# SabaPivot/ProjectionTrainer

Hardware: AMD Instinct MI355X
Metric: Stage-1 images/sec/node (SigLIP-L-384 + Gemma3-1B, 576+128 tok) (higher is better)
Workload: dtype bf16; 1 GPU; cfg2: SigLIP-ViT-L/16-384 frozen fwd + MLP projector fwd/bwd + Gemma3-1B frozen fwd/bwd, 575 vis + 128 text tokens; global_batch=32, per_gpu_batch=32, seq_len=703, parallelism=dp1

## Files before the change

### include/ptk.h

```cpp
#ifndef PTK_H
#define PTK_H

#include <stddef.h>
#include <stdint.h>

#ifdef __cplusplus
extern "C" {
#endif

#define PTK_ABI_VERSION 8

int ptk_abi_version(void);
const char* ptk_last_error(void);


typedef struct {
  int g;
  int skip;
  int64_t gs;
  int64_t off;
} ptk_rowmap;

enum { PTK_ACT_NONE = 0, PTK_ACT_GELU_TANH = 1, PTK_ACT_GELU_ERF = 2, PTK_ACT_GEGLU = 3,
       PTK_ACT_GELU_ERF_BWD = 4, PTK_ACT_GEGLU_BWD = 5 };
enum { PTK_OUT_BF16 = 0, PTK_OUT_F32 = 1, PTK_OUT_F32_BF16ROUND = 2 };

typedef struct {
  const void* A;
  const void* B;
  void* C;
  int M, N, K;
  int64_t lda, ldb, ldc;
  int batch;
  int batch_inner;
  int64_t sA0, sA1, sB0, sB1, sC0, sC1;
  float alpha;
  int act;
  int out;
  const float* bias;
  const float* rowadd;
  int rowadd_period;
  int64_t ld_rowadd;
  const float* resid;
  int64_t ld_resid;
  void* aux;
  void* aux2;
  int64_t ld_aux;
  const void* aux_in;
  const void* aux_in2;
  int64_t ld_aux_in;
  ptk_rowmap amap;
  ptk_rowmap cmap;
  const void* resid16;
  int64_t ld_resid16;
  int bf16_linear;
  void* tail_ws;
  const void* B_kt;
  int A_kt, C_kt, aux_kt, aux_in_kt;
} ptk_gemm_desc;
int ptk_gemm_ktiled_counts(int64_t* out2, int reset);
int ptk_gemm_ktiled_pair(const ptk_gemm_desc* producer, const ptk_gemm_desc* consumer, int ncu, int64_t part_floats,
                         int train);
int ptk_a_ktiled_reload(void);
int ptk_gemm(const ptk_gemm_desc* d, void* stream);
int64_t ptk_kstep_tile_offset(int64_t row, int64_t k, int64_t K);
int ptk_pack_kstep_tiles_bf16(const void* src, void* dst, int N, int K, void* stream);
#define PTK_GEMM_TAIL_COUNTER_BYTES 16384
size_t ptk_gemm_tail_scratch_bytes(void);
int ptk_gemm_tail_split(const ptk_gemm_desc* d);
int ptk_gemm_plan(const ptk_gemm_desc* d, int ncu, int* path, int* tile_rows, int* tail_split);
int ptk_gemm_split_plan(const ptk_gemm_desc* d, int ncu, int64_t part_floats, int* slices, int* kc, int* rem,
                        int* tail_ws);

int ptk_layernorm(const float* x, const float* w, const float* b, void* y, int rows, int cols, float eps,
                  void* stream);
int ptk_rmsnorm(const float* x, const float* w, void* y, float* rstd, int rows, int cols, float eps,
                void* stream);
int ptk_rmsnorm_bwd(const float* x, const float* w, const float* rstd, const float* dn, const float* dacc,
                    float* dx, int rows, int cols, void* stream);
int ptk_qknorm_rope_fwd(const void* qkv, const float* q_norm_w, const float* k_norm_w, const float* cos_t,
                        const float* sin_t, int batch, int seq, int heads, int kv_heads, int head_dim, float eps,
                        void* Q, void* K, void* V, float* rstd_q, float* rstd_k, void* stream);
int ptk_qknorm_rope_bwd(const void* qkv, const float* q_norm_w, const float* k_norm_w, const float* cos_t,
                        const float* sin_t, int batch, int seq, int heads, int kv_heads, int head_dim,
                        const float* rstd_q, const float* rstd_k, const void* dQ, const void* dK, const void* dV,
                        void* dqkv, void* stream);
int ptk_softmax(const float* S, void* P, int nz, int rows, int cols, int64_t ld, int rows_per_batch, int qdiv,
                int zdiv, int causal, int window, const int32_t* key_valid, int key_len, void* stream);
int ptk_cross_entropy(void* logits, int64_t ld, int rows, int vocab, const int64_t* targets, float* row_loss,
                      const float* gscale, void* stream);
int ptk_transpose_bf16(const void* in, int64_t ld_in, void* out, int64_t ld_out, int nz, int64_t s_in,
                       int64_t s_out, int rows, int cols, int rows_pad, void* stream);
int ptk_transpose_rows_bf16(const void* in, int64_t ld_in, int map_g, int64_t map_gs, int64_t map_off, int rows,
                            int cols, void* out, int64_t ld_out, int rows_pad, void* stream);
int ptk_weight_grad_bf16(const void* dy, int64_t lddy, int y_map_g, int64_t y_map_gs, int64_t y_map_off, int Ny,
                         const void* x, int64_t ldx, int x_map_g, int64_t x_map_gs, int64_t x_map_off, int Nx, int rows,
                         void* grad, void* ta, void* tb, float* part, int64_t part_floats, int mode, void* stream);
int ptk_cast_f32_bf16(const float* in, void* out, int64_t n, void* stream);
int ptk_fill_normal_bf16(void* out, int64_t n, uint64_t seed, float std, float mean, void* stream);
int ptk_gemm_timer_enable(int on);
int ptk_gemm_force_small_tiles(int mode);
int ptk_gemm_timer_read(int act_class, double* total_ms, int* count);
#define PTK_GEMM_NPATHS 9
int ptk_gemm_path_counts(int64_t* counts, int reset);

int ptk_stage_timers_enable(int on);
int ptk_stage_begin(const char* name, void* stream);
int ptk_stage_end(void* stream);
int64_t ptk_stage_timers_read(char* buf, size_t cap, int reset);

typedef struct {
  const void* Q; const void* K; const void* V; void* O; float* lse;
  int rows, nkeys, head_dim;
  int64_t ldq, ldk, ldo;
  int batch, batch_inner, zdiv;
  int64_t sQ0, sQ1, sK0, sK1, sO0, sO1;
  ptk_rowmap qmap, omap;
  int qdiv, causal, window;
  const int32_t* key_valid;
  float scale;
} ptk_flash_desc;
int ptk_flash_attn_fwd(const ptk_flash_desc* d, void* stream);

typedef struct {
  const void* Q; const void* K; const void* V; const void* O; const void* dO;
  const float* lse; float* delta;
  void* dQ; void* dK; void* dV;
  int rows, nkeys, head_dim;
  int batch, batch_inner, zdiv;
  int64_t ldo, sO0, sO1;
  ptk_rowmap omap;
  int qdiv, causal, window;
// ... 223 lines not shown
```

### projectiontrainer_amd/_lib.py

```python
from __future__ import annotations

import ctypes as C
import os

_HERE = os.path.dirname(os.path.abspath(__file__))
LIB_PATH = os.path.join(_HERE, "libptk.so")
if os.environ.get("PTK_LIB"):
    LIB_PATH = os.path.join(os.path.dirname(_HERE), os.environ["PTK_LIB"])

c_void_p, c_int, c_int64, c_float, c_size_t, c_uint64 = C.c_void_p, C.c_int, C.c_int64, C.c_float, C.c_size_t, C.c_uint64
c_float_p = C.POINTER(C.c_float)

ACT_NONE, ACT_GELU_TANH, ACT_GELU_ERF, ACT_GEGLU, ACT_GELU_ERF_BWD, ACT_GEGLU_BWD = range(6)
OUT_BF16, OUT_F32, OUT_F32_BF16ROUND = range(3)


class RowMap(C.Structure):
    _fields_ = [("g", c_int), ("skip", c_int), ("gs", c_int64), ("off", c_int64)]


class GemmDesc(C.Structure):
    _fields_ = [("A", c_void_p), ("B", c_void_p), ("C", c_void_p),
                ("M", c_int), ("N", c_int), ("K", c_int),
                ("lda", c_int64), ("ldb", c_int64), ("ldc", c_int64),
# ... 95 lines not shown


class Gemma3LayerGradsC(C.Structure):
    _fields_ = [(n, c_void_p) for n in ("wqkv", "wo", "wgu", "wd", "ln_in", "ln_post_attn", "ln_pre_ff",
                                        "ln_post_ff", "q_norm", "k_norm")]


class Gemma3GradsC(C.Structure):
    _fields_ = [("embed", c_void_p), ("final_norm", c_void_p), ("layers", C.POINTER(Gemma3LayerGradsC))]


class ImageDesc(C.Structure):
    _fields_ = [("src_off", c_int64), ("h", C.c_int32), ("w", C.c_int32), ("c", C.c_int32),
                ("kh", C.c_int32), ("kv", C.c_int32), ("pad_", C.c_int32),
                ("coef_off", c_int64), ("tmp_off", c_int64)]


ABI_VERSION = 8

SIGNATURES = {
    "ptk_abi_version": (c_int, []),
    "ptk_last_error": (C.c_char_p, []),
    "ptk_gemm": (c_int, [C.POINTER(GemmDesc), c_void_p]),
    "ptk_gemm_tail_scratch_bytes": (c_size_t, []),
    "ptk_gemm_tail_split": (c_int, [C.POINTER(GemmDesc)]),
    "ptk_gemm_plan": (c_int, [C.POINTER(GemmDesc), c_int] + [C.POINTER(c_int)] * 3),
    "ptk_gemm_split_plan": (c_int, [C.POINTER(GemmDesc), c_int, c_int64] + [C.POINTER(c_int)] * 4),
    "ptk_layernorm": (c_int, [c_void_p, c_void_p, c_void_p, c_void_p, c_int, c_int, c_float, c_void_p]),
    "ptk_rmsnorm": (c_int, [c_void_p, c_void_p, c_void_p, c_void_p, c_int, c_int, c_float, c_void_p]),
    "ptk_rmsnorm_bwd": (c_int, [c_void_p] * 6 + [c_int, c_int, c_void_p]),
    "ptk_qknorm_rope_fwd": (c_int, [c_void_p] * 5 + [c_int] * 5 + [c_float] + [c_void_p] * 6),
    "ptk_qknorm_rope_bwd": (c_int, [c_void_p] * 5 + [c_int] * 5 + [c_void_p] * 7),
    "ptk_softmax": (c_int, [c_void_p, c_void_p, c_int, c_int, c_int, c_int64, c_int, c_int, c_int, c_int,
                            c_int, c_void_p, c_int, c_void_p]),
    "ptk_cross_entropy": (c_int, [c_void_p, c_int64, c_int, c_int, c_void_p, c_void_p, c_void_p, c_void_p]),
    "ptk_transpose_bf16": (c_int, [c_void_p, c_int64, c_void_p, c_int64, c_int, c_int64, c_int64, c_int,
                                   c_int, c_int, c_void_p]),
    "ptk_transpose_rows_bf16": (c_int, [c_void_p, c_int64, c_int, c_int64, c_int64, c_int, c_int, c_void_p, c_int64,
                                        c_int, c_void_p]),
    "ptk_weight_grad_bf16": (c_int, [c_void_p, c_int64, c_int, c_int64, c_int64, c_int,
                                     c_void_p, c_int64, c_int, c_int64, c_int64, c_int, c_int,
                                     c_void_p, c_void_p, c_void_p, c_void_p, c_int64, c_int, c_void_p]),
    "ptk_cast_f32_bf16": (c_int, [c_void_p, c_void_p, c_int64, c_void_p]),
    "ptk_kstep_tile_offset": (c_int64, [c_int64, c_int64, c_int64]),
    "ptk_pack_kstep_tiles_bf16": (c_int, [c_void_p, c_void_p, c_int, c_int, c_void_p]),
    "ptk_fill_normal_bf16": (c_int, [c_void_p, c_int64, c_uint64, c_float, c_float, c_void_p]),
    "ptk_gemm_timer_enable": (c_int, [c_int]),
    "ptk_gemm_force_small_tiles": (c_int, [c_int]),
    "ptk_gemm_timer_read": (c_int, [c_int, C.POINTER(C.c_double), C.POINTER(c_int)]),
    "ptk_gemm_path_counts": (c_int, [c_void_p, c_int]),
    "ptk_gemm_ktiled_counts": (c_int, [c_void_p, c_int]),
    "ptk_gemm_ktiled_pair": (c_int, [C.POINTER(GemmDesc), C.POINTER(GemmDesc), c_int, c_int64, c_int]),
    "ptk_a_ktiled_reload": (c_int, []),
    "ptk_stage_timers_enable": (c_int, [c_int]),
    "ptk_stage_begin": (c_int, [C.c_char_p, c_void_p]),
    "ptk_stage_end": (c_int, [c_void_p]),
    "ptk_stage_timers_read": (c_int64, [C.c_char_p, c_size_t, c_int]),
    "ptk_flash_attn_fwd": (c_int, [C.POINTER(FlashDesc), c_void_p]),
    "ptk_flash_attn_bwd": (c_int, [C.POINTER(FlashBwdDesc), c_void_p]),
    "ptk_flash_bwd_workspace_bytes": (c_size_t, [C.POINTER(FlashBwdDesc)]),
    "ptk_siglip_workspace_bytes": (c_size_t, [C.POINTER(SiglipConfigC), c_int]),
    "ptk_siglip_fwd": (c_int, [C.POINTER(SiglipConfigC), C.POINTER(SiglipWeightsC), c_int, c_void_p, c_void_p,
                               c_void_p, c_size_t, c_void_p]),
    "ptk_projector_fwd": (c_int, [C.POINTER(ProjectorC), c_int, c_void_p, c_void_p, c_void_p, c_void_p, RowMap,
                                  c_int64, c_int, c_void_p]),
    "ptk_projector_workspace_bytes": (c_size_t, [C.POINTER(ProjectorC), c_int]),
    "ptk_projector_bwd": (c_int, [C.POINTER(ProjectorC), c_int] + [c_void_p] * 8 + [c_void_p, c_size_t, c_void_p]),
    "ptk_gather_vision_grad": (c_int, [c_void_p, c_int, c_int, c_int, c_int, c_void_p, c_void_p]),
    "ptk_gemma3_workspace_bytes": (c_size_t, [C.POINTER(Gemma3ConfigC), c_int, c_int, c_int]),
    "ptk_gemma3_loss_fwd_bwd": (c_int, [C.POINTER(Gemma3ConfigC), C.POINTER(Gemma3WeightsC),
                                        C.POINTER(Gemma3BatchC), c_void_p, c_size_t, c_void_p]),
    "ptk_gemma3_loss_fwd": (c_int, [C.POINTER(Gemma3ConfigC), C.POINTER(Gemma3WeightsC),
                                    C.POINTER(Gemma3BatchC), c_void_p, c_size_t, c_void_p]),
    "ptk_gemma3_train_workspace_bytes": (c_size_t, [C.POINTER(Gemma3ConfigC), c_int, c_int, c_int]),
    "ptk_gemma3_train_fwd_bwd": (c_int, [C.POINTER(Gemma3ConfigC), C.POINTER(Gemma3WeightsC),
                                         C.POINTER(Gemma3BatchC), C.POINTER(Gemma3GradsC), c_void_p, c_size_t,
                                         c_void_p]),
    "ptk_gemma3_generate_workspace_bytes": (c_size_t, [C.POINTER(Gemma3ConfigC), c_int, c_int, c_int]),
    "ptk_gemma3_generate": (c_int, [C.POINTER(Gemma3ConfigC), C.POINTER(Gemma3WeightsC), C.POINTER(Gemma3GenerateC),
                                    c_void_p, c_void_p, c_void_p, c_void_p, c_void_p, c_size_t, c_void_p]),
    "ptk_gemma3_decode_workspace_bytes": (c_size_t, [C.POINTER(Gemma3ConfigC), C.POINTER(Gemma3DecodeC)]),
    "ptk_gemma3_decode_prefill": (c_int, [C.POINTER(Gemma3ConfigC), C.POINTER(Gemma3WeightsC),
                                          C.POINTER(Gemma3DecodeC), c_void_p, c_void_p, c_int64, c_void_p, c_void_p,
                                          c_size_t, c_void_p]),
    "ptk_gemma3_decode_step": (c_int, [C.POINTER(Gemma3ConfigC), C.POINTER(Gemma3WeightsC), C.POINTER(Gemma3DecodeC),
                                       c_int, c_void_p, c_void_p, c_void_p, c_void_p, c_size_t, c_void_p]),
    "ptk_beam_candidates_workspace_bytes": (c_size_t, [c_int, c_int, c_int]),
    "ptk_beam_candidates": (c_int, [c_void_p, c_int64, c_void_p, c_int, c_int, c_int, c_int, c_int, c_float, c_float,
                                    c_int, c_uint64, c_int, c_int, c_void_p, c_void_p, c_void_p, c_void_p, c_size_t,
                                    c_void_p]),
    "ptk_sample_next_token_workspace_bytes": (c_size_t, [c_int]),
    "ptk_sample_next_token": (c_int, [c_void_p, c_int64, c_int, c_int, c_int, c_int, c_float, c_float, c_uint64, c_int,
                                      c_int64, c_int64, c_void_p, c_void_p, c_int64, c_int, c_float, c_void_p,
                                      c_void_p, c_size_t, c_void_p]),
    "ptk_beam_candidates_penalized_workspace_bytes": (c_size_t, [c_int, c_int, c_int]),
    "ptk_beam_candidates_penalized": (c_int, [c_void_p, c_int64, c_void_p, c_int, c_int, c_int, c_int, c_int, c_float,
                                              c_float, c_int, c_uint64, c_int, c_int, c_void_p, c_int64, c_int,
                                              c_float, c_void_p, c_void_p, c_void_p, c_void_p, c_size_t, c_void_p]),
    "ptk_gemma3_generate_penalized_workspace_bytes": (c_size_t, [C.POINTER(Gemma3ConfigC), c_int, c_int, c_int]),
    "ptk_gemma3_generate_penalized": (c_int, [C.POINTER(Gemma3ConfigC), C.POINTER(Gemma3WeightsC),
                                              C.POINTER(Gemma3GenerateC), c_void_p, c_void_p, c_void_p, c_void_p,
                                              c_float, c_void_p, c_size_t, c_void_p]),
    "ptk_gemm_skinny_part_bytes": (c_size_t, [c_int, c_int, c_int]),
    "ptk_gemm_skinny": (c_int, [c_void_p, c_int64, c_void_p, c_int64, c_void_p, c_int64, c_int, c_int, c_int, c_int,
                                c_void_p, c_size_t, c_void_p]),
    "ptk_embed_grad_workspace_bytes": (c_size_t, [c_int, c_int]),
# ... 18 lines not shown
                                    [c_void_p, c_size_t, c_void_p, c_void_p, c_void_p]),
    "ptk_clip_adamw": (c_int, [c_void_p, c_void_p, c_void_p, c_void_p, c_int64, c_float, c_float, c_float,
                               c_float, c_float, c_float, c_float, c_int, c_void_p, c_void_p, c_void_p]),
}

_lib = None


class PtkError(RuntimeError):
    pass


def lib():
    global _lib
    if _lib is None:
        if not os.path.exists(LIB_PATH):
            raise PtkError(f"libptk.so not found at {LIB_PATH}: run `python -c 'import __graft_entry__ as g; g.build()'`")
        L = C.CDLL(LIB_PATH)
        for name, (res, args) in SIGNATURES.items():
            if os.environ.get("PTK_LIB") and not hasattr(L, name):
                continue
            f = getattr(L, name)
            f.restype, f.argtypes = res, args
        if L.ptk_abi_version() != ABI_VERSION:
            raise PtkError("libptk ABI version mismatch")
        _lib = L
    return _lib


def check(rc: int, what: str = ""):
    if rc != 0:
        raise PtkError(f"{what}: {lib().ptk_last_error().decode()}")


def ptr(t) -> int | None:
    return None if t is None else t.data_ptr()


GEMM_PATHS = ("nt128", "big", "big2", "w4", "nt128b", "p8sk", "p8", "tn", "unused8")


def gemm_path_counts(reset=False):
    buf = (C.c_int64 * (8 * len(GEMM_PATHS)))()
    check(lib().ptk_gemm_path_counts(buf, int(reset)), "gemm_path_counts")
    return {(GEMM_PATHS[i // 8], i % 8): int(v) for i, v in enumerate(buf) if v}


def gemm_ktiled_counts(reset=False):
    buf = (C.c_int64 * 2)()
    check(lib().ptk_gemm_ktiled_counts(buf, int(reset)), "gemm_ktiled_counts")
    return int(buf[0]), int(buf[1])


_stages_on = os.environ.get("PTK_STAGE_TIMERS", "0") not in ("", "0")


def stage_timers_enable(on=True):
    global _stages_on
    _stages_on = bool(on)
    check(lib().ptk_stage_timers_enable(int(bool(on))), "stage_timers_enable")


class stage:

    def __init__(self, name, device=None):
        self.name, self.device, self.on = name, device, False

    def __enter__(self):
        self.on = _stages_on
        if self.on:
            self.st = stream_ptr(self.device)
            check(lib().ptk_stage_begin(self.name.encode(), self.st), "stage_begin")
        return self

    def __exit__(self, *exc):
        if self.on:
            check(lib().ptk_stage_end(self.st), "stage_end")
        return False


def stage_timers_read(reset=False):
    n = lib().ptk_stage_timers_read(None, 0, 0)
    if n < 0:
        check(-1, "stage_timers_read")
    buf = C.create_string_buffer(int(n) + 64)
    n = lib().ptk_stage_timers_read(buf, len(buf), int(reset))
    if n < 0:
        check(-1, "stage_timers_read")
    out = {}
    for line in buf.value.decode().splitlines():
        name, ms, cnt = line.split("\t")
        out[name] = (float(ms), int(cnt))
    return out


def stream_ptr(device=None) -> int:
    import torch
    return torch.cuda.current_stream(device).cuda_stream
```

### projectiontrainer_amd/csrc/capi.cpp

```cpp
#include <stdarg.h>
#include <stdio.h>

#include "../../include/ptk.h"
#include "ptk_internal.h"

namespace ptk {

static thread_local char g_err[512] = "";

int set_error(const char* fmt, ...) {
  va_list ap;
  va_start(ap, fmt);
  vsnprintf(g_err, sizeof(g_err), fmt, ap);
  va_end(ap);
  return -1;
}

RowMap to_map(ptk_rowmap m) { return RowMap{m.g, m.skip, (long)m.gs, (long)m.off}; }

GemmArgs to_args(const ptk_gemm_desc* d) {
  GemmArgs a;
  a.A = (const bf16_t*)d->A; a.B = (const bf16_t*)d->B; a.C = d->C;
  a.M = d->M; a.N = d->N; a.K = d->K;
  a.lda = d->lda; a.ldb = d->ldb; a.ldc = d->ldc;
// ... 34 lines not shown

int ptk_abi_version(void) { return PTK_ABI_VERSION; }
const char* ptk_last_error(void) { return g_err; }

int ptk_gemm(const ptk_gemm_desc* d, void* stream) {
  if (!d) return set_error("ptk_gemm: null desc");
  if (d->act == PTK_ACT_GEGLU && (d->N % 32)) return set_error("ptk_gemm: GEGLU needs N %% 32 == 0");
  return launch_gemm(to_args(d), d->act, d->out, d->batch > 0 ? d->batch : 1, ST);
}

size_t ptk_gemm_tail_scratch_bytes(void) { return p8_tail_scratch_bytes(); }
int ptk_gemm_tail_split(const ptk_gemm_desc* d) {
  if (!d) return set_error("ptk_gemm_tail_split: null desc");
  return p8_tail_plan(to_args(d), d->act, d->out, gemm_plan_env()).gsplit;
}
static GemmPlanEnv test_plan_env(int ncu) {
  GemmPlanEnv e = gemm_plan_env();
  e.ncu = ncu;
  e.tail_scope = nullptr;
  return e;
}
int ptk_gemm_plan(const ptk_gemm_desc* d, int ncu, int* path, int* tile_rows, int* tail_split) {
  if (!d || ncu <= 0) return set_error("ptk_gemm_plan: null desc or ncu <= 0");
  const GemmPlan p = gemm_plan(to_args(d), d->act, d->out, d->batch > 0 ? d->batch : 1, test_plan_env(ncu));
  if (path) *path = p.path;
  if (tile_rows) *tile_rows = p.tm;
  if (tail_split) *tail_split = p.tail.gsplit;
  return 0;
}
int ptk_gemm_split_plan(const ptk_gemm_desc* d, int ncu, int64_t part_floats, int* slices, int* kc, int* rem,
                        int* tail_ws) {
  if (!d || ncu <= 0) return set_error("ptk_gemm_split_plan: null desc or ncu <= 0");
  const GemmSplitPlan s = gemm_split_plan(to_args(d), d->out, (long)part_floats, test_plan_env(ncu));
  if (slices) *slices = s.slices;
  if (kc) *kc = s.kc;
  if (rem) *rem = s.rem;
  if (tail_ws) *tail_ws = s.tail_ws ? 1 : 0;
  return 0;
}

size_t ptk_gemm_skinny_part_bytes(int M, int N, int K) { return skinny_part_bytes(M, N, K); }
int ptk_gemm_skinny(const void* A, int64_t lda, const void* B, int64_t ldb, void* C, int64_t ldc, int M, int N, int K,
                    int act, void* part, size_t part_bytes, void* stream) {
  if (!A || !B || !C) return set_error("ptk_gemm_skinny: NULL operand");
  return launch_gemm_skinny((const bf16_t*)A, (long)lda, (const bf16_t*)B, (long)ldb, (bf16_t*)C, (long)ldc, M, N, K,
                            act, (float*)part, part_bytes, (hipStream_t)stream);
}

int ptk_layernorm(const float* x, const float* w, const float* b, void* y, int rows, int cols, float eps,
                  void* stream) {
  return launch_layernorm(x, w, b, (bf16_t*)y, rows, cols, eps, ST);
}

int ptk_rmsnorm(const float* x, const float* w, void* y, float* rstd, int rows, int cols, float eps, void* stream) {
  return launch_rmsnorm_fwd(x, cols, RowMap{0, 0, 0, 0}, w, (bf16_t*)y, rstd, rows, cols, eps, ST);
}

int ptk_rmsnorm_bwd(const float* x, const float* w, const float* rstd, const float* dn, const float* dacc, float* dx,
                    int rows, int cols, void* stream) {
  return launch_rmsnorm_bwd_f32(x, w, rstd, dn, dacc, dx, rows, cols, ST);
}

int ptk_qknorm_rope_fwd(const void* qkv, const float* q_norm_w, const float* k_norm_w, const float* cos_t,
                        const float* sin_t, int batch, int seq, int heads, int kv_heads, int head_dim, float eps,
                        void* Q, void* K, void* V, float* rstd_q, float* rstd_k, void* stream) {
  const AttnShape sh{batch, seq, heads, kv_heads, head_dim};
  return launch_qknorm_rope_fwd((const bf16_t*)qkv, q_norm_w, k_norm_w, cos_t, sin_t, sh, eps, (bf16_t*)Q,
                                (bf16_t*)K, (bf16_t*)V, rstd_q, rstd_k, ST);
}
int ptk_qknorm_rope_bwd(const void* qkv, const float* q_norm_w, const float* k_norm_w, const float* cos_t,
                        const float* sin_t, int batch, int seq, int heads, int kv_heads, int head_dim,
                        const float* rstd_q, const float* rstd_k, const void* dQ, const void* dK, const void* dV,
                        void* dqkv, void* stream) {
  const AttnShape sh{batch, seq, heads, kv_heads, head_dim};
  return launch_qknorm_rope_bwd((const bf16_t*)qkv, q_norm_w, k_norm_w, cos_t, sin_t, sh, rstd_q, rstd_k,
                                (const bf16_t*)dQ, (const bf16_t*)dK, (const bf16_t*)dV, (bf16_t*)dqkv, ST);
}
int ptk_softmax(const float* S, void* P, int nz, int rows, int cols, int64_t ld, int rows_per_batch, int qdiv,
                int zdiv, int causal, int window, const int32_t* key_valid, int key_len, void* stream) {
  MaskSpec m{rows_per_batch > 0 ? rows_per_batch : rows, qdiv > 0 ? qdiv : 1, zdiv > 0 ? zdiv : 1, causal, window,
             key_valid, key_len};
  return launch_softmax_fwd(S, (bf16_t*)P, nz, rows, cols, ld, m, ST);
}

int ptk_cross_entropy(void* logits, int64_t ld, int rows, int vocab, const int64_t* targets, float* row_loss,
                      const float* gscale, void* stream) {
  return launch_ce_fwd_bwd((bf16_t*)logits, ld, rows, vocab, targets, row_loss, gscale, ST);
}

int ptk_transpose_bf16(const void* in, int64_t ld_in, void* out, int64_t ld_out, int nz, int64_t s_in, int64_t s_out,
                       int rows, int cols, int rows_pad, void* stream) {
  return launch_transpose((const bf16_t*)in, ld_in, s_in, 0, 1, (bf16_t*)out, ld_out, s_out, 0, nz, rows, cols,
                          rows_pad, ST);
}

int ptk_transpose_rows_bf16(const void* in, int64_t ld_in, int map_g, int64_t map_gs, int64_t map_off, int rows,
                            int cols, void* out, int64_t ld_out, int rows_pad, void* stream) {
  const RowMap m{map_g, 0, map_gs, map_off};
  return launch_transpose_rows((const bf16_t*)in, ld_in, m, rows, cols, (bf16_t*)out, ld_out, rows_pad, ST);
}

int64_t ptk_kstep_tile_offset(int64_t row, int64_t k, int64_t K) { return kstep_tile_offset(row, k, K); }
int ptk_pack_kstep_tiles_bf16(const void* src, void* dst, int N, int K, void* stream) {
  return launch_pack_kstep_tiles((const bf16_t*)src, (bf16_t*)dst, N, K, ST);
}
int ptk_cast_f32_bf16(const float* in, void* out, int64_t n, void* stream) {
  return launch_cast_f32_bf16(in, (bf16_t*)out, n, ST);
}

int ptk_gemm_force_small_tiles(int mode) {
  if (mode != 0 && mode != 1 && mode != 2 && mode != 4 && mode != 8 && mode != 32 && mode != 512 && mode != 1024 &&
      mode != 4096)
    return set_error("gemm tile mode %d not in {0, 1, 2, 4, 8, 32, 512, 1024, 4096}", mode);
  force_small_tiles(mode);
  return 0;
}
int ptk_gemm_timer_enable(int on) {
  timer_enable(on);
  return 0;
}
int ptk_gemm_timer_read(int act_class, double* total_ms, int* count) { return timer_read(act_class, total_ms, count); }
int ptk_gemm_path_counts(int64_t* counts, int reset) { return path_counts(counts, reset); }
int ptk_gemm_ktiled_counts(int64_t* out2, int reset) { return ktiled_counts(out2, reset); }
int ptk_gemm_ktiled_pair(const ptk_gemm_desc* producer, const ptk_gemm_desc* consumer, int ncu, int64_t part_floats,
                         int train) {
  if (!producer || !consumer || ncu <= 0 || producer->batch > 1 || consumer->batch > 1) return 0;
  return !train && gemm_ktiled_pair(to_args(producer), producer->act, to_args(consumer), (long)part_floats,
                                    test_plan_env(ncu), a_ktiled_mode() != 0, true) ? 1 : 0;
}

int ptk_fill_normal_bf16(void* out, int64_t n, uint64_t seed, float std, float mean, void* stream) {
  return launch_fill_normal_bf16((bf16_t*)out, n, seed, std, mean, ST);
}

int ptk_flash_attn_fwd(const ptk_flash_desc* d, void* stream) {
  if (!d) return set_error("flash: null desc");
  FlashArgs a;
  a.Q = (const bf16_t*)d->Q; a.K = (const bf16_t*)d->K; a.V = (const bf16_t*)d->V; a.O = (bf16_t*)d->O;
  a.lse = d->lse; a.rows = d->rows; a.nkeys = d->nkeys; a.D = d->head_dim;
  a.ldq = d->ldq; a.ldk = d->ldk; a.ldo = d->ldo;
  a.zin = d->batch_inner > 0 ? d->batch_inner : 1; a.zdiv = d->zdiv > 0 ? d->zdiv : 1;
  a.sQ0 = d->sQ0; a.sQ1 = d->sQ1; a.sK0 = d->sK0; a.sK1 = d->sK1; a.sO0 = d->sO0; a.sO1 = d->sO1;
  a.qmap = to_map(d->qmap); a.omap = to_map(d->omap);
  a.qdiv = d->qdiv > 0 ? d->qdiv : 1; a.causal = d->causal; a.window = d->window;
  a.key_valid = d->key_valid; a.scale = d->scale;
  return launch_attn_fwd(a, d->batch > 0 ? d->batch : 1, ST);
}

static FlashBwdArgs to_bwd_args(const ptk_flash_bwd_desc* d) {
  FlashBwdArgs a;
  a.Q = (const bf16_t*)d->Q; a.K = (const bf16_t*)d->K; a.V = (const bf16_t*)d->V; a.O = (const bf16_t*)d->O;
  a.dO = (const bf16_t*)d->dO; a.lse = d->lse; a.delta = d->delta;
  a.dQ = (bf16_t*)d->dQ; a.dK = (bf16_t*)d->dK; a.dV = (bf16_t*)d->dV;
  a.rows = d->rows; a.nkeys = d->nkeys; a.D = d->head_dim;
  a.zin = d->batch_inner > 0 ? d->batch_inner : 1; a.zdiv = d->zdiv > 0 ? d->zdiv : 1;
  a.ldo = d->ldo; a.sO0 = d->sO0; a.sO1 = d->sO1; a.omap = to_map(d->omap);
  a.qdiv = d->qdiv > 0 ? d->qdiv : 1; a.causal = d->causal; a.window = d->window;
  a.key_valid = d->key_valid; a.scale = d->scale;
  a.dkv_part = (float*)d->workspace;
  a.dkv_part_bytes = d->workspace && d->workspace_bytes > 0 ? (size_t)d->workspace_bytes : 0;
  return a;
}

size_t ptk_flash_bwd_workspace_bytes(const ptk_flash_bwd_desc* d) {
  if (!d) return 0;
  return attn_bwd_workspace_bytes(to_bwd_args(d), d->batch > 0 ? d->batch : 1);
}

int ptk_flash_attn_bwd(const ptk_flash_bwd_desc* d, void* stream) {
  if (!d) return set_error("flash_bwd: null desc");
  return launch_attn_bwd(to_bwd_args(d), d->batch > 0 ? d->batch : 1, ST);
}

int ptk_projector_fwd(const ptk_projector* p, int rows, const void* x, void* a, void* h, float* out,
                      ptk_rowmap out_map, int64_t ld_out, int round_bf16, void* stream) {
  const int Dv = p->vision_dim, I = p->inter_dim, Dl = p->llm_dim;
  TailScratchScope tail(p->tail_ws, ST);
  if (tail.status) return -1;
  StageScope stage("projector.fwd", ST);
  GemmArgs g1;
  g1.A = (const bf16_t*)x; g1.B = (const bf16_t*)p->w1; g1.C = h;
  g1.M = rows; g1.N = I; g1.K = Dv; g1.lda = Dv; g1.ldb = Dv; g1.ldc = I;
// ... 101 lines not shown
```

### projectiontrainer_amd/csrc/gemm.hip

```cpp
#include <stdlib.h>

#include "common.h"
#include "ptk_internal.h"
#include "gemm_epi.h"

#include <algorithm>
#include <vector>

namespace ptk {

constexpr int BM = 128, BN = 128, BK = 64, GROUP_M = 8;
constexpr int STAGE_BYTES = (BM + BN) * BK * 2;
static_assert(4 * 64 * 68 * 4 >= 2 * STAGE_BYTES, "epilogue staging must cover the pipeline buffers");

typedef const __attribute__((address_space(1))) void* gptr_t;
typedef __attribute__((address_space(3))) void* lptr_t;

#ifdef PTK_NO_SRC_SWZ
#define PTK_SRC_SWZ(c, r) (c)
#else
#define PTK_SRC_SWZ(c, r) ((c) ^ (((r) >> 1) & 7))
#endif

#ifndef PTK_GLDS_AUX
// ... 594 lines not shown
  for (int i = 0; i < 8; ++i)
#pragma unroll
    for (int j = 0; j < 4; ++j) acc[i][j] = (f32x4_t){0.f, 0.f, 0.f, 0.f};
  big2_kloop(p, smem, bm, bn, 0, p.K / BK, acc, threadIdx.x);
  big_epilogue<ACT, OUT>(p, smem, bm, bn, acc, threadIdx.x);
}

static bool g_timing = false;
static int g_timing_mask = 0;
static int g_force_tiles = 0;
void force_small_tiles(int mode) { g_force_tiles = mode; }
static std::vector<hipEvent_t> g_ev[8];
static size_t g_ev_used[8];

void timer_enable(int on) {
  g_timing = on != 0;
  g_timing_mask = on == 1 ? 0xff : (on & 0xff);
  if (g_timing)
    for (int c = 0; c < 8; ++c) g_ev_used[c] = 0;
}
static hipEvent_t next_event(int cls) {
  auto& v = g_ev[cls];
  if (g_ev_used[cls] == v.size()) {
    hipEvent_t e;
    if (hipEventCreate(&e) != hipSuccess) return nullptr;
    v.push_back(e);
  }
  return v[g_ev_used[cls]++];
}
int timer_read(int cls, double* total_ms, int* count) {
  *total_ms = 0;
  *count = 0;
  if (cls < 0 || cls >= 8) return set_error("timer: class out of range");
  for (size_t i = 0; i + 1 < g_ev_used[cls]; i += 2) {
    float ms = 0;
    if (hipEventSynchronize(g_ev[cls][i + 1]) != hipSuccess) return set_error("timer: sync failed");
    if (hipEventElapsedTime(&ms, g_ev[cls][i], g_ev[cls][i + 1]) != hipSuccess) return set_error("timer: elapsed");
    *total_ms += ms;
    *count += 1;
  }
  return 0;
}

static long g_path_count[GEMM_NPATH][8];
int path_counts(int64_t* out, int reset) {
  for (int p = 0; p < GEMM_NPATH; ++p)
    for (int c = 0; c < 8; ++c) {
      if (out) out[p * 8 + c] = g_path_count[p][c];
      if (reset) g_path_count[p][c] = 0;
    }
  return 0;
}

static long g_kt_count[2];
int ktiled_counts(int64_t* out2, int reset) {
  for (int i = 0; i < 2; ++i) {
    if (out2) out2[i] = g_kt_count[i];
    if (reset) g_kt_count[i] = 0;
  }
  return 0;
}

struct GemmLaunchScope {
  hipStream_t st;
  hipEvent_t e0 = nullptr, e1 = nullptr;
  GemmLaunchScope(int path, int act, hipStream_t s) : st(s) {
    ++g_path_count[path][act & 7];
    if (g_timing && ((g_timing_mask >> act) & 1)) { e0 = next_event(act); e1 = next_event(act); }
    if (e0) (void)hipEventRecord(e0, st);
  }
  ~GemmLaunchScope() { if (e1) (void)hipEventRecord(e1, st); }
};

GemmPlanEnv gemm_plan_env() {
  GemmPlanEnv e;
  e.ncu = device_cus();
  e.force_tiles = g_force_tiles;
  e.p8_all = PTK_AB("PTK_P8", 0) == 1;
  e.tm_short = PTK_AB("PTK_TM224", 1) != 0;
  e.lean_epi = lean_epilogue_enabled();
  e.streamk = streamk_enabled();
  e.tail_scope = tail_scope();
  return e;
}

int launch_gemm(const GemmArgs& a, int act, int out, int batch, hipStream_t st, const GemmPlan* planned) {
  if (a.M <= 0 || a.N <= 0 || batch <= 0) return 0;
  if (a.K <= 0 || a.K % BK) return set_error("gemm: K=%d must be a positive multiple of 64", a.K);
  if ((a.lda % 8) || (a.ldb % 8)) return set_error("gemm: lda/ldb must be multiples of 8 (16-B rows)");
  if (((uintptr_t)a.A | (uintptr_t)a.B) & 15) return set_error("gemm: A/B must be 16-B aligned");
  if (a.zin <= 0) return set_error("gemm: zin must be >= 1");
  const long ntile = (long)((a.M + BM - 1) / BM) * ((a.N + BN - 1) / BN);
  if (ntile > 0x7fffffffL) return set_error("gemm: too many tiles");
  if (!gemm_act_out(act, out, [](auto, auto) {})) return set_error("gemm: unsupported (act=%d, out=%d)", act, out);
  const GemmPlan plan = planned ? *planned : gemm_plan(a, act, out, batch, gemm_plan_env());
  if (a.a_kt && !a_ktiled_ok(a, plan, act, out, batch, lean_epilogue_enabled()))
    return set_error("gemm: this launch cannot read a k-step-tiled A");
  if (!c_ktiled_ok(a, plan, act, out, batch, lean_epilogue_enabled()))
    return set_error("gemm: this launch cannot write k-step-tiled outputs");
  GemmLaunchScope scope(plan.path, act, st);
  g_kt_count[0] += a.a_kt != 0;
  g_kt_count[1] += a.c_kt != 0;
  const dim3 grid_big((unsigned)((long)((a.M + BIG - 1) / BIG) * ((a.N + BIG - 1) / BIG)), 1, 1);
  switch (plan.path) {
    case GEMM_PATH_P8:
    case GEMM_PATH_P8SK:
    case GEMM_PATH_W4: {
      GemmArgs b = a;
      if (!b_ktiled_ok(a, plan, act, batch)) b.B_kt = nullptr;
      if (plan.path == GEMM_PATH_W4) return launch_gemm_w4(b, act, out, st, 0);
      return launch_gemm_p8(b, act, out, st, plan.tail, plan.tm);
    }
    case GEMM_PATH_BIG2:
      gemm_act_out(act, out, [&](auto A, auto O) {
        hipLaunchKernelGGL((gemm_big2_kernel<A(), O()>), grid_big, dim3(512), 0, st, a);
      });
      break;
    case GEMM_PATH_BIG:
      gemm_act_out(act, out, [&](auto A, auto O) {
        hipLaunchKernelGGL((gemm_big_kernel<A(), O()>), grid_big, dim3(512), 0, st, a);
      });
      break;
    default:
      gemm_act_out(act, out, [&](auto A, auto O) {
        hipLaunchKernelGGL((gemm_nt_kernel<A(), O()>), dim3((unsigned)ntile, 1, (unsigned)batch), dim3(256), 0, st, a);
      });
      break;
  }
  return hipGetLastError() == hipSuccess ? 0 : set_error("gemm launch failed");
}

int gemm_p8_kslices(const GemmArgs& a, int slices, hipStream_t st) {
  if (a.M <= 0 || a.N <= 0) return 0;
  GemmLaunchScope scope(GEMM_PATH_P8, ACT_NONE, st);
  return launch_gemm_p8_kslices(a, slices, st);
}

int gemm_tn(const GemmArgs& a, int out, int slices, void* slab, hipStream_t st, long k_rows) {
  if (a.M <= 0 || a.N <= 0) return 0;
  GemmLaunchScope scope(GEMM_PATH_TN, ACT_NONE, st);
  return launch_gemm_tn(a, out, slices, slab, st, k_rows);
}

}

#ifdef PTK_STAMPS
extern "C" int ptk_debug_epi_mode(int m) {
  return hipMemcpyToSymbol(HIP_SYMBOL(ptk::g_epi_mode), &m, sizeof(int), 0, hipMemcpyHostToDevice) == hipSuccess ? 0 : -1;
}
extern "C" int ptk_debug_stamps_read(void* host, size_t bytes) {
  return hipMemcpyFromSymbol(host, HIP_SYMBOL(ptk::g_stamps), bytes, 0, hipMemcpyDeviceToHost) == hipSuccess ? 0 : -1;
}
#endif
```

### projectiontrainer_amd/csrc/gemm_plan.cpp

```cpp
#include <algorithm>

#include "ptk_internal.h"

namespace ptk {

bool w4_supported(const GemmArgs& a, int act, int out) {
  if (a.N % 8 || a.K % W4_KT) return false;
  if (a.alpha != 1.f) return false;
  if (a.row_stats) return false;
  if (a.resid16 && (out != OUT_BF16 || a.ld_resid16 % 8)) return false;
  if ((a.ldc % 8) || (a.resid && a.ld_resid % 4) || (a.rowadd && a.ld_rowadd % 4)) return false;
  if ((a.aux || a.aux2) && a.ld_aux % 8) return false;
  if ((a.aux_in || a.aux_in2) && a.ld_aux_in % 8) return false;
  if (((uintptr_t)a.C | (uintptr_t)a.bias | (uintptr_t)a.resid | (uintptr_t)a.resid16 | (uintptr_t)a.rowadd | (uintptr_t)a.aux |
       (uintptr_t)a.aux2 | (uintptr_t)a.aux_in | (uintptr_t)a.aux_in2) & 15)
    return false;
  if (act == ACT_GEGLU && (a.N % 32)) return false;
  if (act == ACT_GEGLU_BWD && (!a.aux_in || !a.aux_in2 || (a.N % 16) || (a.ldc % 8))) return false;
  if (act == ACT_GELU_ERF_BWD && !a.aux_in) return false;
  if (out != OUT_BF16 && (act != ACT_NONE)) return false;
  if (a.amap.g != 0) return false;
  const double abytes = (double)(a.M + a.amap.off) * a.lda * 2, bbytes = (double)a.N * a.ldb * 2;
  return abytes < 2147483000.0 && bbytes < 2147483000.0;
}
// ... 133 lines not shown
         (act == ACT_NONE && out == OUT_BF16 && a.N >= 1536 && a.K <= 2048 && fill >= 0.65 &&
          lean_epilogue_candidate(a, e.lean_epi));
}

bool big_shape(const GemmArgs& a) {
  return a.M >= 1024 && a.N >= 512 && (a.K >= 6144 || (a.N >= 6144 && a.K >= 1152));
}
bool staggered_big(const GemmArgs& a, const GemmPlanEnv& e) {
  return e.force_tiles == 4 || (e.force_tiles == 0 && big_shape(a) && a.K >= 4096);
}
bool big(const GemmArgs& a, const GemmPlanEnv& e) {
  return e.force_tiles != 1 && (e.force_tiles == 2 || big_shape(a));
}

}

GemmPlan gemm_plan(const GemmArgs& a, int act, int out, int batch, const GemmPlanEnv& e) {
  GemmPlan p;
  if (batch != 1) {
    p.path = GEMM_PATH_NTB;
    return p;
  }
  if (p8_supported(a, act, out)) {
    const P8Tail tl = tail(a, act, out, e);
    const int tm = tl.units ? 256 : short_tile(a, act, out, e);
    const bool single = single_round(a, act, out, e);
    if (e.force_tiles == 32 || single || tl.units || tm != 256 || p8_over_w4(a, act, out, e)) {
      p.path = tl.units ? GEMM_PATH_P8SK : GEMM_PATH_P8;
      p.tm = tm;
      p.tail = tl;
      p.single_round = single;
      return p;
    }
  }
  if ((e.force_tiles == 8 || w4_shape(a, act, out, e)) && w4_supported(a, act, out)) p.path = GEMM_PATH_W4;
  else if (staggered_big(a, e)) p.path = GEMM_PATH_BIG2;
  else if (big(a, e)) p.path = GEMM_PATH_BIG;
  return p;
}

long kstep_tile_offset(long row, long k, long K) {
  const long rr = row & 15, chunk = (k >> 3) & 3;
  const long unit = 4 * rr + (chunk ^ ((rr >> 1) & 2));
  return ((row >> 4) * (K / 32) + (k >> 5)) * 1024 + unit * 16 + (k & 7) * 2;
}

bool b_ktiled_ok(const GemmArgs& a, const GemmPlan& plan, int act, int batch) {
  if (!a.B_kt || batch != 1 || !bkt_act(act)) return false;
  if (plan.path != GEMM_PATH_W4 && plan.path != GEMM_PATH_P8 && plan.path != GEMM_PATH_P8SK) return false;
  return a.ldb == a.K && a.K % 32 == 0 && a.N % 16 == 0 && !((uintptr_t)a.B_kt & 15);
}

bool a_ktiled_ok(const GemmArgs& a, const GemmPlan& plan, int act, int out, int batch, bool lean_epi) {
  if (batch != 1 || act != ACT_NONE || out != OUT_BF16 || plan.path != GEMM_PATH_P8 || plan.tail.units) return false;
  if (a.M % 16 || a.K % 32 || a.lda != a.K || a.amap.g != 0 || a.amap.off < 0 || a.amap.off % 16) return false;
  (void)lean_epi;
  return b_ktiled_ok(a, plan, act, batch);
}

bool c_ktiled_ok(const GemmArgs& a, const GemmPlan& plan, int act, int out, int batch, bool lean_epi) {
  if (!a.c_kt) return !a.aux_kt && !a.aux_in_kt;
  if (batch != 1 || out != OUT_BF16 || plan.path != GEMM_PATH_W4 || a.M % 16 || !b_ktiled_ok(a, plan, act, batch))
    return false;
  if (a.cmap.g != 0 || a.cmap.off < 0 || a.cmap.off % 16 || ((uintptr_t)a.C & 15)) return false;
  if (act == ACT_GEGLU) {
    if (a.N % 64 || a.ldc != a.N / 2 || a.aux_in_kt) return false;
    return !a.aux_kt || (a.aux && a.aux2 && a.ld_aux == a.N / 2 && !(((uintptr_t)a.aux | (uintptr_t)a.aux2) & 15));
  }
  uint32_t cb = 0;
  if (act != ACT_GEGLU_BWD || a.aux_kt || !lean_epilogue_ok(a, act, out, cb, lean_epi)) return false;
  return a.ldc == 2L * a.N && (!a.aux_in_kt || a.ld_aux_in == a.N);
}

bool gemm_ktiled_pair(const GemmArgs& prod, int pact, const GemmArgs& cons, long part_floats, const GemmPlanEnv& env,
                      bool enabled, bool factors) {
  if (!enabled || (pact != ACT_GEGLU && pact != ACT_GEGLU_BWD)) return false;
  GemmArgs p = prod, c = cons;
  p.c_kt = 1;
  if (factors) (pact == ACT_GEGLU ? p.aux_kt : p.aux_in_kt) = 1;
  c.a_kt = 1;
  if (!c_ktiled_ok(p, gemm_plan(prod, pact, OUT_BF16, 1, env), pact, OUT_BF16, 1, env.lean_epi)) return false;
  if (cons.A != (const bf16_t*)prod.C || cons.M != prod.M || cons.K != (pact == ACT_GEGLU ? prod.N / 2 : 2 * prod.N) ||
      cons.amap.off != prod.cmap.off)
    return false;
  const GemmSplitPlan sp = gemm_split_plan(cons, OUT_BF16, part_floats, env);
  if (sp.kc != 0 || sp.tail_ws) return false;
  const GemmPlan cp = env.force_tiles == 0 ? sp.direct : gemm_plan(cons, ACT_NONE, OUT_BF16, 1, env);
  return a_ktiled_ok(c, cp, ACT_NONE, OUT_BF16, 1, env.lean_epi);
}

GemmSplitPlan gemm_split_plan(const GemmArgs& a, int out, long part_floats, const GemmPlanEnv& env) {
  GemmSplitPlan sp;
  GemmPlanEnv e = env;
  e.force_tiles = 0;
  sp.direct = gemm_plan(a, ACT_NONE, out, 1, e);
  const GemmPlan& direct = sp.direct;
  if (direct.path == GEMM_PATH_P8SK) return sp;
  if (e.streamk && a.K >= 4096 && (size_t)part_floats * sizeof(float) >= P8_CNT_BYTES + p8_slab_bytes(e.ncu)) {
    GemmArgs b = a;
    b.tail_ws = reinterpret_cast<void*>((uintptr_t)256);
    const GemmPlan lent = gemm_plan(b, ACT_NONE, out, 1, e);
    if (lent.path == GEMM_PATH_P8SK) {
      sp.tail_ws = true;
      sp.direct = lent;
      return sp;
    }
  }
  if (direct.single_round) return sp;
  const long nbig = tiles256(a);
  int S = 1, kmin = 1024;
  if (a.K >= 4096 && nbig <= 64) S = 4;
  else if (a.K >= 4096 && nbig <= 300) S = 2;
  const long n128 = (long)((a.M + 127) / 128) * ((a.N + 127) / 128), cus = e.ncu;
  if (n128 * 2 <= cus) {
    kmin = 256;
    while (n128 * S * 2 <= 2 * cus && a.K / (S * 2) >= kmin) S *= 2;
  }
  while (S > 1 && ((long)S * a.M * a.N > part_floats || a.K / S < kmin || a.N % 4 || a.ldc % 4)) S /= 2;
  const bool plain = !a.rowadd && !a.resid && !a.aux && !a.aux_in && a.amap.g == 0 && a.amap.off == 0 &&
                     a.cmap.g == 0 && a.cmap.off == 0 && a.bias == nullptr && a.alpha == 1.f;
  if (S == 1 || !plain) return sp;
  sp.kc = (a.K / S + 63) / 64 * 64;
  sp.slices = a.K / sp.kc;
  sp.rem = a.K - sp.slices * sp.kc;
  return sp;
}

bool tn_supported(const GemmArgs& a, int out, int slices, bool lean_epi) {
  if (slices < 1 || a.K % (W4_KT * slices) || a.K / slices < 2 * W4_KT) return false;
  if (a.N % 64 || a.lda % 8 || a.ldb % 8 || a.lda < a.M || a.ldb < a.N) return false;
  if (((uintptr_t)a.A | (uintptr_t)a.B | (uintptr_t)a.C) & 15) return false;
  if (a.amap.g || a.amap.off || a.bias || a.rowadd || a.resid || a.aux || a.aux_in || a.row_stats || a.alpha != 1.f)
    return false;
  const double ab = (double)a.K * a.lda * 2, bb = (double)a.K * a.ldb * 2;
  if (ab >= 4293918720.0 || bb >= 4293918720.0) return false;
  if (out == OUT_BF16) {
    uint32_t cb = 0;
    return slices == 1 && lean_epilogue_candidate(a, lean_epi) && lean_epilogue_ok(a, ACT_NONE, OUT_BF16, cb, lean_epi);
  }
  if (out != OUT_F32 || a.ldc % 4 || a.ldc < a.N || a.cmap.g || a.cmap.off || a.resid16 || a.bf16_linear) return false;
  return (double)slices * a.M * a.ldc * 4 < 2147483000.0;
// ... 34 lines not shown
```

### projectiontrainer_amd/csrc/gemm_w4.hip

```cpp
#include "common.h"
#include "ptk_internal.h"
#include "gemm_epi.h"
#include "gemm_persist.h"

#include <algorithm>
#include <cstdlib>
#include <type_traits>

#ifndef PTK_W4_RDS
#define PTK_W4_RDS 0
#endif
#ifndef PTK_W4_DMS
#define PTK_W4_DMS 0
#endif
#ifndef PTK_P8_PRIO
#define PTK_P8_PRIO 1
#endif
#ifndef PTK_P8_MPRIO
#define PTK_P8_MPRIO 0
#endif

namespace ptk {

template <int ACT, int OUT, bool LEAN = false, bool BKT = false, int KTO = 0>
__global__ void __launch_bounds__(256, 1) gemm_w4_kernel(GemmArgs p, uint32_t a_bytes, uint32_t b_bytes,
                                                         uint32_t c_bytes) {
  __shared__ __attribute__((aligned(16))) char smem[W4_NSLOT * W4_SLOT];
  const int lane = threadIdx.x & 63;
  const int wave = __builtin_amdgcn_readfirstlane(threadIdx.x >> 6);
  const int wr = wave >> 1, wc = wave & 1;
  const int nbm = (p.M + W4 - 1) / W4, nbn = (p.N + W4 - 1) / W4;
  const int ntile = nbm * nbn;
  const int G = gridDim.x;
  int loc;
  {
    const int b = blockIdx.x, q = G >> 3, rr = G & 7, x = b & 7;
    loc = (x < rr ? x * (q + 1) : rr * (q + 1) + (x - rr) * q) + (b >> 3);
  }
  if (loc >= ntile) return;
  const int nt = p.K / W4_KT;
  const int nks = 2 * nt;
  const int total_ks = ((ntile - loc + G - 1) / G) * nks;

  constexpr bool bkt = BKT;
  constexpr uint32_t bks = BKT ? 1024u : (uint32_t)(W4_KS * 2);
  const u32x4_t rsa = w4_rsrc(p.A, a_bytes), rsb = w4_rsrc(bkt ? p.B_kt : p.B, b_bytes);

  uint32_t offa[4], offb[4];
#pragma unroll
  for (int j = 0; j < 4; ++j) {
    const int lr = wave * 64 + 16 * j + (lane >> 2);
    const int lc = (lane & 3) ^ ((lane >> 3) & 2);
    offa[j] = (uint32_t)lr * (uint32_t)p.lda * 2u + lc * 16;
    offb[j] = bkt ? (uint32_t)(wave * 4 + j) * (uint32_t)p.K * 32u + lane * 16
                  : (uint32_t)lr * (uint32_t)p.ldb * 2u + lc * 16;
  }
  const uint32_t lds_base = __builtin_amdgcn_readfirstlane(lds_addr(smem));
  const uint32_t lds_dma = lds_base + wave * 64 * 64;
  int dt = loc, dks = 0, dcount = 0;
  uint32_t dsa = 0, dsb = 0;
  auto dma_tile = [&](int t) {
    int bm, bn;
    w4_tile_coords(t, nbm, nbn, bm, bn);
    dsa = __builtin_amdgcn_readfirstlane((uint32_t)(bm * W4 + (int)p.amap.off) * (uint32_t)p.lda * 2u);
    dsb = __builtin_amdgcn_readfirstlane((uint32_t)(bn * W4) * (uint32_t)p.ldb * 2u);
  };
  auto dma_advance = [&]() {
    if (++dcount < total_ks) {
      if (++dks == nks) {
        dks = 0;
        dt += G;
        dma_tile(dt);
      }
    }
  };
  auto slot_next = [](uint32_t s) { s += W4_SLOT; return s == W4_NSLOT * W4_SLOT ? 0u : s; };

  const int frag_off = (lane & 15) * 64 + (((lane >> 4) ^ ((lane >> 1) & 2)) << 4);
  const uint32_t frag_a = lds_addr(smem) + wr * 128 * 64 + frag_off;
  const uint32_t frag_b = lds_addr(smem) + W4_SOPB + wc * 128 * 64 + frag_off;
  bf16x8_t fa0[8], fb0[8], fa1[8], fb1[8];
  f32x4_t acc[8][8];

#define W4_GROUP(FA, FB, Q, FIRST)                                                  \
  do {                                                                              \
    _Pragma("unroll") for (int jj = 0; jj < 4; ++jj) {                              \
      if (FIRST) W4_MFMA0(acc[(Q) >> 1][4 * ((Q) & 1) + jj], FB[4 * ((Q) & 1) + jj], FA[(Q) >> 1]); \
      else W4_MFMA(acc[(Q) >> 1][4 * ((Q) & 1) + jj], FB[4 * ((Q) & 1) + jj], FA[(Q) >> 1]);       \
    }                                                                               \
  } while (0)
#define W4_READ(FA, FB, BA, BB, Q)                                                  \
  do {                                                                              \
    if ((Q) < 8) W4_DSREAD(FA[(Q) & 7], BA, ((Q) & 7) * 1024);                      \
    else W4_DSREAD(FB[(Q) & 7], BB, ((Q) & 7) * 1024);                              \
  } while (0)
#define W4_PIN(FA, FB)                                                                              \
  do {                                                                                              \
    asm volatile("s_waitcnt lgkmcnt(0)" ::: "memory");                                              \
    asm volatile("" : "+v"(FA[0]), "+v"(FA[1]), "+v"(FA[2]), "+v"(FA[3]), "+v"(FA[4]), "+v"(FA[5]),  \
                 "+v"(FA[6]), "+v"(FA[7]));                                                         \
    asm volatile("" : "+v"(FB[0]), "+v"(FB[1]), "+v"(FB[2]), "+v"(FB[3]), "+v"(FB[4]), "+v"(FB[5]),  \
                 "+v"(FB[6]), "+v"(FB[7]));                                                         \
  } while (0)

  auto kstep = [&](auto first_c, const bf16x8_t (&FA)[8], const bf16x8_t (&FB)[8], bf16x8_t (&NA)[8],
                   bf16x8_t (&NB)[8], uint32_t rs, uint32_t ws) {
    constexpr bool first = decltype(first_c)::value;
    const uint32_t ba = frag_a + rs, bb = frag_b + rs;
    const uint32_t da = lds_dma + ws, db = da + W4_SOPB;
    const uint32_t sa = dsa + dks * (W4_KS * 2), sb = dsb + dks * bks;
#pragma unroll
    for (int q = 0; q < 16; ++q) {
#if PTK_W4_RDS == 1
      if (q < 8) {
        W4_READ(NA, NB, ba, bb, 2 * q);
        W4_READ(NA, NB, ba, bb, 2 * q + 1);
      }
#else
      if (q < 8) {
        W4_READ(NA, NB, ba, bb, q);
      } else if (q < 12) {
        W4_READ(NA, NB, ba, bb, 8 + 2 * (q - 8));
        W4_READ(NA, NB, ba, bb, 9 + 2 * (q - 8));
      }
#endif
#if PTK_W4_DMS == 1
      if (q >= 8) {
        const int pc = q - 8;
#elif PTK_W4_DMS == 2
      if (q < 8) {
        const int pc = q;
#elif PTK_W4_DMS == 3
      if (q & 1) {
        const int pc = q >> 1;
#else
      if (!(q & 1)) {
        const int pc = q >> 1;
#endif
        if (pc & 1) W4_DMA(rsb, offb[pc >> 1], sb, db + (pc >> 1) * 1024);
        else W4_DMA(rsa, offa[pc >> 1], sa, da + (pc >> 1) * 1024);
      }
      W4_GROUP(FA, FB, q, first);
    }
  };

  dma_tile(dt);
#pragma unroll
  for (int b = 0; b < 4; ++b) {
    const uint32_t da = lds_dma + b * W4_SLOT, db = da + W4_SOPB;
    const uint32_t sa = dsa + dks * (W4_KS * 2), sb = dsb + dks * bks;
#pragma unroll
    for (int j = 0; j < 4; ++j) {
      W4_DMA(rsa, offa[j], sa, da + j * 1024);
      W4_DMA(rsb, offb[j], sb, db + j * 1024);
    }
    dma_advance();
  }
  asm volatile("s_waitcnt vmcnt(8)" ::: "memory");
  __builtin_amdgcn_s_barrier();
#pragma unroll
  for (int q = 0; q < 16; ++q) W4_READ(fa0, fb0, frag_a, frag_b, q);
  W4_PIN(fa0, fb0);
  __builtin_amdgcn_s_barrier();

  uint32_t rs = W4_SLOT, ws = 4 * W4_SLOT;
  int t = loc, kt = 0;
#ifdef PTK_P8_STAMPS
  unsigned int stv_[4] = {0u, 0u, 0u, 0u};
  const int em_ = g_p8_epi_mode;
#endif
  for (int g = 0; g < total_ks; g += 2) {
    if (kt == 0) P8_STAMP(0, (t - loc) / G);
    if (kt == 0) kstep(std::true_type{}, fa0, fb0, fa1, fb1, rs, ws);
    else kstep(std::false_type{}, fa0, fb0, fa1, fb1, rs, ws);
    W4_PIN(fa1, fb1);
    dma_advance();
    rs = slot_next(rs);
    ws = slot_next(ws);
    kstep(std::false_type{}, fa1, fb1, fa0, fb0, rs, ws);
    W4_PIN(fa0, fb0);
    dma_advance();
    rs = slot_next(rs);
    ws = slot_next(ws);
    asm volatile("s_waitcnt vmcnt(8)" ::: "memory");
    __builtin_amdgcn_s_barrier();
    if (kt == 0) P8_STAMP(1, (t - loc) / G);
    if (kt == nt - 1) {
      P8_STAMP(2, (t - loc) / G);
      asm volatile("s_nop 7\n\ts_nop 7" ::: "memory");
      int bm, bn;
      w4_tile_coords(t, nbm, nbn, bm, bn);
#ifdef PTK_P8_STAMPS
      if (em_ != 1)
#endif
      {
        const long row0 = (long)bm * W4 + wr * 128, col0 = (long)bn * W4 + wc * 128;
        if constexpr (LEAN && ACT == ACT_GEGLU_BWD)
          w4_epilogue_lean_glu<ACT, 8, KTO>(kernarg_args(), acc, row0, col0, lane, c_bytes);
        else if constexpr (LEAN) w4_epilogue_lean<ACT, 8>(kernarg_args(), acc, row0, col0, lane, c_bytes);
        else w4_epilogue<ACT, OUT, 8, 8, KTO>(kernarg_args(), acc, row0, col0, lane);
      }
      P8_STAMP(3, (t - loc) / G);
      t += G;
      kt = 0;
    } else {
      ++kt;
    }
  }
  asm volatile("s_waitcnt vmcnt(0)" ::: "memory");
#ifdef PTK_P8_STAMPS
  if (wave == 0 && blockIdx.x < 1024)
#pragma unroll
    for (int k = 0; k < 4; ++k) g_p8_stamps[blockIdx.x][k][lane] = stv_[k];
#endif
#undef W4_GROUP
#undef W4_READ
#undef W4_PIN
}

bool lean_epilogue_enabled() { return PTK_AB("PTK_LEAN_EPI", 1) != 0; }

template <int ACT, int OUT, bool LEAN>
static void w4_launch(const GemmArgs& a, long grid, hipStream_t st, uint32_t ab, uint32_t bb, uint32_t cb) {
  if constexpr ((ACT == ACT_GEGLU && !LEAN) || (ACT == ACT_GEGLU_BWD && LEAN)) {
    if (a.c_kt && a.B_kt) {
      if (a.aux_kt || a.aux_in_kt)
        hipLaunchKernelGGL((gemm_w4_kernel<ACT, OUT, LEAN, true, 3>), dim3((unsigned)grid), dim3(256), 0, st, a, ab, bb, cb);
      else
        hipLaunchKernelGGL((gemm_w4_kernel<ACT, OUT, LEAN, true, 1>), dim3((unsigned)grid), dim3(256), 0, st, a, ab, bb, cb);
      return;
    }
  }
  if constexpr (bkt_act(ACT)) {
    if (a.B_kt) {
      hipLaunchKernelGGL((gemm_w4_kernel<ACT, OUT, LEAN, true>), dim3((unsigned)grid), dim3(256), 0, st, a, ab, bb, cb);
      return;
    }
  }
  hipLaunchKernelGGL((gemm_w4_kernel<ACT, OUT, LEAN, false>), dim3((unsigned)grid), dim3(256), 0, st, a, ab, bb, cb);
}

int launch_gemm_w4(const GemmArgs& a, int act, int out, hipStream_t st, int max_grid) {
  const long ntile = (long)((a.M + W4 - 1) / W4) * ((a.N + W4 - 1) / W4);
  long grid = std::min<long>(ntile, max_grid > 0 ? max_grid : device_cus());
#ifdef PTK_P8_STAMPS
  if (const char* e = getenv("PTK_GEMM_GRID")) grid = std::min<long>(grid, atol(e));
#endif
  const long arows = a.M + a.amap.off;
  const uint32_t ab = (uint32_t)std::min<double>((double)arows * a.lda * 2, 2147483000.0);
  const uint32_t bb = (uint32_t)std::min<double>((double)a.N * a.ldb * 2, 2147483000.0);
  uint32_t cb = 0;
  const bool lean = lean_epilogue_ok(a, act, out, cb, lean_epilogue_enabled());
  if (a.c_kt || a.aux_kt || a.aux_in_kt) {
    if (!a.c_kt || !a.B_kt || !((act == ACT_GEGLU && !a.aux_in_kt) || (act == ACT_GEGLU_BWD && lean && !a.aux_kt)))
      return set_error("gemm_w4: no k-step-tiled-output variant for this launch");
  }
  if (lean) {
#define PTK_W4L_CASE(ACT_) \
    if (act == ACT_)       \
      w4_launch<ACT_, OUT_BF16, true>(a, grid, st, ab, bb, cb);
    PTK_W4L_CASE(ACT_NONE)
    PTK_W4L_CASE(ACT_GELU_TANH)
    PTK_W4L_CASE(ACT_GEGLU_BWD)
#undef PTK_W4L_CASE
    return hipGetLastError() == hipSuccess ? 0 : set_error("gemm_w4 launch failed");
  }
  if (!gemm_act_out(act, out, [&](auto A, auto O) {
        w4_launch<A(), O(), false>(a, grid, st, ab, bb, 0u);
      }))
    return set_error("gemm_w4: unsupported (act=%d, out=%d)", act, out);
  return hipGetLastError() == hipSuccess ? 0 : set_error("gemm_w4 launch failed");
}


namespace {
constexpr int P8_PIECES = 4;

}



#ifdef PTK_P8_CREAD
#define P8_DSREAD(DST, ADDR, OFF) \
  (DST) = *reinterpret_cast<const __attribute__((address_space(3))) bf16x8_t*>((uintptr_t)((ADDR) + (OFF)))
#define P8_LGKM(N) do { } while (0)
#define P8_BARRIER() do { __builtin_amdgcn_s_barrier(); asm volatile("" ::: "memory"); } while (0)
#else
#define P8_BARRIER() __builtin_amdgcn_s_barrier()
#define P8_DSREAD(DST, ADDR, OFF) W4_DSREAD(DST, ADDR, OFF)
#define P8_LGKM(N) asm volatile("s_waitcnt lgkmcnt(" #N ")" ::: "memory")
#endif
template <int ACT, int OUT, bool SK, bool LEAN = false, int TM = 256, bool BKT = false, bool AKT = false>
__global__ void __launch_bounds__(512, 1) gemm_p8_kernel(GemmArgs p, uint32_t a_bytes, uint32_t b_bytes, P8Tail tl,
                                                         uint32_t c_bytes) {
  static_assert(TM == 256 || ((TM == 224 || TM == 192 || TM == 160) && !SK), "shorter tiles: whole tiles only");
  static_assert(!AKT || !SK, "a tiled A: whole tiles only");
  constexpr int RB = TM / 32;
  __shared__ __attribute__((aligned(16))) char smem[W4_NSLOT * W4_SLOT];
  const int lane = threadIdx.x & 63;
  const int wave = __builtin_amdgcn_readfirstlane(threadIdx.x >> 6);
  const int hf = wave >> 2, wq = wave & 3, wr = wq >> 1, wc = wq & 1;
  const bool a_dma = TM == 256 || wave < RB;
  const int nbm = (p.M + TM - 1) / TM, nbn = (p.N + W4 - 1) / W4;
  const int ntile = nbm * nbn;
  const int G = gridDim.x;
// ... 325 lines not shown
  if (out == OUT_BF16) hipLaunchKernelGGL((p8_fixup_kernel<ACT_NONE, OUT_BF16>), grid, dim3(512), 0, st, a, tl, nu);
  else if (out == OUT_F32) hipLaunchKernelGGL((p8_fixup_kernel<ACT_NONE, OUT_F32>), grid, dim3(512), 0, st, a, tl, nu);
  else hipLaunchKernelGGL((p8_fixup_kernel<ACT_NONE, OUT_F32_BFR>), grid, dim3(512), 0, st, a, tl, nu);
  return hipGetLastError() == hipSuccess ? 0 : set_error("p8 fixup launch failed");
}

size_t p8_tail_scratch_bytes() { return P8_CNT_BYTES + p8_slab_bytes(device_cus()); }

static bool streamk_models() { return PTK_AB("PTK_STREAMK", 1) != 0; }
bool streamk_enabled() { return streamk_models(); }
static thread_local void* g_tail_scope = nullptr;
void* tail_scope() { return g_tail_scope; }
TailScratchScope::TailScratchScope(void* ws, hipStream_t st) : prev(g_tail_scope) {
  if (!streamk_models()) ws = nullptr;
  g_tail_scope = ws;
  (void)st;
}
TailScratchScope::~TailScratchScope() { g_tail_scope = prev; }

size_t p8_tail_scratch_bytes_models() { return streamk_models() ? p8_tail_scratch_bytes() : 0; }

int launch_gemm_p8_kslices(const GemmArgs& a, int slices, hipStream_t st) {
  if (a.a_kt || a.c_kt) return set_error("gemm_p8_kslices: K slices take no k-step-tiled activation");
  if (slices < 1 || a.M % W4 || a.K < 128 || a.K % W4_KT || a.cmap.g || a.cmap.off || a.amap.g || a.amap.off ||
      a.bias || a.rowadd || a.resid || a.resid16 || a.aux || a.row_stats)
    return set_error("gemm_p8_kslices: unsupported operands");
  if ((double)a.M * a.lda * 2 + (double)slices * a.K * 2 >= 4293918720.0 ||
      (double)a.N * a.ldb * 2 + (double)slices * a.K * 2 >= 4293918720.0)
    return set_error("gemm_p8_kslices: operands past 4 GiB");
  GemmArgs g = a;
  g.M = a.M * slices;
  g.B_kt = nullptr;
  P8Tail tl;
  tl.zslices = slices;
  const long ntile = (long)(g.M / W4) * ((g.N + W4 - 1) / W4);
  const long grid = std::min<long>(ntile, device_cus());
  const uint32_t ab = (uint32_t)std::min<double>((double)a.M * a.lda * 2, 4294967040.0);
  const uint32_t bb = (uint32_t)std::min<double>((double)a.N * a.ldb * 2, 4294967040.0);
  hipLaunchKernelGGL((gemm_p8_kernel<ACT_NONE, OUT_F32, false>), dim3((unsigned)grid), dim3(512), 0, st, g, ab, bb, tl,
                     0u);
  return hipGetLastError() == hipSuccess ? 0 : set_error("gemm_p8_kslices launch failed");
}

template <int ACT, int OUT, bool SK, bool LEAN, int TM>
static void p8_launch(const GemmArgs& a, long grid, hipStream_t st, uint32_t ab, uint32_t bb, const P8Tail& tl,
                      uint32_t cb) {
  if constexpr (ACT == ACT_NONE && OUT == OUT_BF16 && !SK) {
    if (a.a_kt && a.B_kt) {
      hipLaunchKernelGGL((gemm_p8_kernel<ACT, OUT, SK, LEAN, TM, true, true>), dim3((unsigned)grid), dim3(512), 0, st, a,
                         ab, bb, tl, cb);
      return;
    }
  }
  if constexpr (bkt_act(ACT)) {
    if (a.B_kt) {
      hipLaunchKernelGGL((gemm_p8_kernel<ACT, OUT, SK, LEAN, TM, true>), dim3((unsigned)grid), dim3(512), 0, st, a, ab,
                         bb, tl, cb);
      return;
    }
  }
  hipLaunchKernelGGL((gemm_p8_kernel<ACT, OUT, SK, LEAN, TM, false>), dim3((unsigned)grid), dim3(512), 0, st, a, ab, bb,
                     tl, cb);
}

template <int TM>
static int launch_p8_short(const GemmArgs& a, int act, int out, hipStream_t st, long grid, bool lean_epi) {
  const uint32_t ab = (uint32_t)std::min<double>((double)(a.M + a.amap.off) * a.lda * 2, 2147483000.0);
  const uint32_t bb = (uint32_t)std::min<double>((double)a.N * a.ldb * 2, 2147483000.0);
  const P8Tail tl{};
  uint32_t cb = 0;
  if (lean_epilogue_ok(a, act, out, cb, lean_epi)) {
    if (act == ACT_NONE)
      p8_launch<ACT_NONE, OUT_BF16, false, true, TM>(a, grid, st, ab, bb, tl, cb);
    else
      p8_launch<ACT_GELU_TANH, OUT_BF16, false, true, TM>(a, grid, st, ab, bb, tl, cb);
  } else if (act == ACT_GELU_TANH) {
    p8_launch<ACT_GELU_TANH, OUT_BF16, false, false, TM>(a, grid, st, ab, bb, tl, 0u);
  } else if (out == OUT_BF16) {
    p8_launch<ACT_NONE, OUT_BF16, false, false, TM>(a, grid, st, ab, bb, tl, 0u);
  } else if (out == OUT_F32) {
    p8_launch<ACT_NONE, OUT_F32, false, false, TM>(a, grid, st, ab, bb, tl, 0u);
  } else {
    p8_launch<ACT_NONE, OUT_F32_BFR, false, false, TM>(a, grid, st, ab, bb, tl, 0u);
  }
  return hipGetLastError() == hipSuccess ? 0 : set_error("gemm_p8 launch failed");
}

int launch_gemm_p8(const GemmArgs& a, int act, int out, hipStream_t st, const P8Tail& tl, int tm) {
  const long ncu = device_cus();
  const bool lean_epi = lean_epilogue_enabled();
  if (a.a_kt) {
    if (act != ACT_NONE || out != OUT_BF16 || tl.units || !a.B_kt)
      return set_error("gemm_p8: no k-step-tiled-A variant for this launch");
  }
  if (tm != 256 && !tl.units) {
    if (!(act == ACT_NONE || (act == ACT_GELU_TANH && out == OUT_BF16)))
      return set_error("gemm_p8: %d-row tiles take the plain / GELU-tanh epilogues only", tm);
    if (tm != 224 && tm != 192 && tm != 160) return set_error("gemm_p8: tile height %d (256, 224, 192, 160)", tm);
    const long ntm = (long)((a.M + tm - 1) / tm) * ((a.N + W4 - 1) / W4);
    const long grid = std::min<long>(ntm, ncu);
    if (tm == 224) return launch_p8_short<224>(a, act, out, st, grid, lean_epi);
    if (tm == 192) return launch_p8_short<192>(a, act, out, st, grid, lean_epi);
    return launch_p8_short<160>(a, act, out, st, grid, lean_epi);
  }
  const long ntile = (long)((a.M + W4 - 1) / W4) * ((a.N + W4 - 1) / W4);
  long grid = tl.units ? ncu : std::min<long>(ntile, ncu);
#ifdef PTK_P8_STAMPS
  if (const char* e = getenv("PTK_GEMM_GRID")) grid = std::min<long>(grid, atol(e));
#endif
  const long arows = a.M + a.amap.off;
  const uint32_t ab = (uint32_t)std::min<double>((double)arows * a.lda * 2, 2147483000.0);
  const uint32_t bb = (uint32_t)std::min<double>((double)a.N * a.ldb * 2, 2147483000.0);
  uint32_t cb = 0;
  if (tl.units) {
    if (act != ACT_NONE) return set_error("gemm_p8: the stream-K tail takes ACT_NONE only (act=%d)", act);
    if (lean_epilogue_ok(a, act, out, cb, lean_epi)) {
      p8_launch<ACT_NONE, OUT_BF16, true, true, 256>(a, grid, st, ab, bb, tl, cb);
    } else if (!gemm_act_out(act, out, [&](auto A, auto O) {
                 if constexpr (A() == ACT_NONE)
                   p8_launch<ACT_NONE, O(), true, false, 256>(a, grid, st, ab, bb, tl, 0u);
               })) {
      return set_error("gemm_p8: unsupported (act=%d, out=%d)", act, out);
    }
    if (hipGetLastError() != hipSuccess) return set_error("gemm_p8 launch failed");
    return launch_p8_fixup(a, act, out, tl, st);
  }
  if (lean_epilogue_ok(a, act, out, cb, lean_epi)) {
#define PTK_P8L_CASE(ACT_)                                                                                   \
    if (act == ACT_)                                                                                         \
      p8_launch<ACT_, OUT_BF16, false, true, 256>(a, grid, st, ab, bb, tl, cb);
    PTK_P8L_CASE(ACT_NONE)
    PTK_P8L_CASE(ACT_GELU_TANH)
    PTK_P8L_CASE(ACT_GEGLU_BWD)
#undef PTK_P8L_CASE
    return hipGetLastError() == hipSuccess ? 0 : set_error("gemm_p8 launch failed");
  }
  if (!gemm_act_out(act, out, [&](auto A, auto O) {
        p8_launch<A(), O(), false, false, 256>(a, grid, st, ab, bb, tl, 0u);
      }))
    return set_error("gemm_p8: unsupported (act=%d, out=%d)", act, out);
  return hipGetLastError() == hipSuccess ? 0 : set_error("gemm_p8 launch failed");
}

}
```

### projectiontrainer_amd/csrc/models.cpp

```cpp
#include <cstdlib>
#include <algorithm>
#include <math.h>
#include <string.h>

#include <vector>

#include "../../include/ptk.h"
#include "ptk_internal.h"

using namespace ptk;

namespace {

struct Bump {
  char* base;
  size_t off = 0;
  explicit Bump(void* b) : base((char*)b) {}
  template <class T>
  T* take(size_t n) {
    off = (off + 255) & ~(size_t)255;
    T* p = base ? reinterpret_cast<T*>(base + off) : nullptr;
    off += n * sizeof(T);
    return p;
  }
};

float bfround_host(float f) {
  uint32_t u;
  memcpy(&u, &f, 4);
  u += 0x7fffu + ((u >> 16) & 1u);
  u &= 0xffff0000u;
  memcpy(&f, &u, 4);
  return f;
}

constexpr int LM_SPLITK = 8;
constexpr int LM_KSLICES = 16;

#define CK(x) \
  do {        \
    if ((x)) return -1; \
  } while (0)
#define CKH(x)                                                                       \
  do {                                                                               \
    hipError_t e_ = (x);                                                             \
    if (e_ != hipSuccess) return set_error("%s: %s", #x, hipGetErrorString(e_));    \
  } while (0)

static bool geglu_split() {
  const int v = PTK_AB("PTK_GEGLU_SPLIT", 0) == 1;
  return v != 0;
}
static bool norm_wg_fused() { return PTK_AB("PTK_NORM_WG", 1) != 0; }

static int residual_norm_bwd_grads(const float* x2, const float* w_pre, const float* rstd_pre, const bf16_t* dn,
                                   float* dR, const bf16_t* t, const float* w_post, const float* rstd_t, bf16_t* dt,
                                   int M, int H, bf16_t* g_pre, bf16_t* g_post, float* wpart, hipStream_t st) {
  const RowMap ident{0, 0, 0, 0};
  if (g_pre && norm_wg_fused()) {
    const int nb = residual_norm_bwd_wg_blocks(M);
    float* pq = wpart + rms_wgrad_finish_floats(nb, H);
    CK(launch_residual_norm_bwd_wg(x2, w_pre, rstd_pre, dn, dR, t, w_post, rstd_t, dt, M, H, wpart, pq, st));
    CK(launch_rms_wgrad_finish(wpart, nb, H, g_pre, st));
    return launch_rms_wgrad_finish(pq, nb, H, g_post, st);
  }
  if (g_pre) CK(launch_rms_wgrad_bdy(x2, H, ident, rstd_pre, dn, H, M, H, g_pre, wpart, st));
  CK(launch_residual_norm_bwd_bdn(x2, w_pre, rstd_pre, dn, dR, t, w_post, rstd_t, dt, M, H, st));
  if (g_pre) CK(launch_rms_wgrad_bx(t, H, ident, rstd_t, dR, H, 1, M, H, g_post, wpart, st));
  return 0;
}
static bool dkv_reduce_split() {
  static const int v = [] { const char* e = getenv("PTK_DKV_REDUCE_SPLIT"); return e && e[0] == '1' ? 1 : 0; }();
  return v != 0;
}

static bool lm_stats_only() {
#ifdef PTK_DIAG
  static const int v = [] { const char* e = getenv("PTK_LM_STATS_ONLY"); return e && e[0] == '1' ? 1 : 0; }();
  return v != 0;
#else
  return false;
#endif
}

static bool ce_two_pass() {
  static const int v = [] { const char* e = getenv("PTK_CE_TWO_PASS"); return e && e[0] == '1' ? 1 : 0; }();
  return v != 0;
}

static int g_a_ktiled = -1;
}
namespace ptk {
int a_ktiled_mode() {
  if (g_a_ktiled < 0) {
    const char* e = getenv("PTK_A_KTILED");
    g_a_ktiled = e && e[0] == '0' ? 0 : (e && e[0] == '2' ? 2 : 1);
  }
  return g_a_ktiled;
}
}
extern "C" int ptk_a_ktiled_reload(void) {
  g_a_ktiled = -1;
  return a_ktiled_mode();
}
namespace {

GemmArgs gemm(const void* A, long lda, const void* B, long ldb, void* C, long ldc, int M, int N, int K,
              const void* B_kt = nullptr) {
  GemmArgs g;
  g.B_kt = (const bf16_t*)B_kt;
  g.A = (const bf16_t*)A; g.B = (const bf16_t*)B; g.C = C;
  g.lda = lda; g.ldb = ldb; g.ldc = ldc;
  g.M = M; g.N = N; g.K = K;
  return g;
}

struct SiglipWs {
  bf16_t *patches, *h, *a, *qkv, *o, *mlp;
  void* tail;
};

SiglipWs siglip_layout(Bump& bp, const ptk_siglip_config* c, int B) {
  const long D = c->hidden, I = c->intermediate, P = c->patch_size, Nn = (c->image_size / P) * (c->image_size / P);
  const long Np = (Nn + 63) / 64 * 64, M = B * Nn, H = c->heads, hd = D / H, Kp = (long)c->channels * P * P;
  SiglipWs w;
  w.patches = bp.take<bf16_t>(M * Kp);
  w.h = bp.take<bf16_t>(M * D);
  w.a = bp.take<bf16_t>(M * D);
  w.qkv = bp.take<bf16_t>(M * 3 * D);
  w.o = bp.take<bf16_t>(M * D);
  w.mlp = bp.take<bf16_t>(M * I);
  w.tail = bp.take<char>(p8_tail_scratch_bytes_models());
  return w;
}

struct GemmaLayerSave {
  float *x2, *rstd_in, *rstd_ao, *rstd_pre, *rstd_dn, *rstd_q, *rstd_k;
  bf16_t *qkv, *Q, *K, *V, *O, *ao, *glu_a, *glu_b, *dn;
  float* lse;
  bf16_t *xn_in = nullptr, *xn_ff = nullptr, *h = nullptr;
};
struct GemmaWs {
  std::vector<float*> x;
  std::vector<GemmaLayerSave> L;
  bf16_t *P, *xn, *O, *h, *Vt, *Kt, *Qt, *dqkv, *dgu, *dao, *dO, *dS, *dST, *PT, *dOT, *dQ, *dK, *dV, *xf, *logits;
  bf16_t* dtmp;
  float *S, *rstd_f, *row_loss, *dxf, *dxf_part, *count, *gscale, *delta;
  float* ce_stats = nullptr;
  float* dkv_part;
  size_t dkv_part_bytes;
  int32_t* key_valid;
  bf16_t *TA = nullptr, *TB = nullptr, *TL = nullptr, *TX = nullptr;
  float* wpart = nullptr;
  void* eg_keys = nullptr;
  float* skpart = nullptr;
  long sk_floats = 0;
// ... 168 lines not shown
  g.bf16_linear = 1;
  g.resid16 = (const bf16_t*)grad;
  g.ld_resid16 = Nx;
  return gemm_split(g, OUT_BF16, skpart, sk_floats, st);
}

}

extern "C" {

int ptk_weight_grad_bf16(const void* dy, int64_t lddy, int y_map_g, int64_t y_map_gs, int64_t y_map_off, int Ny,
                         const void* x, int64_t ldx, int x_map_g, int64_t x_map_gs, int64_t x_map_off, int Nx, int rows,
                         void* grad, void* ta, void* tb, float* part, int64_t part_floats, int mode, void* stream) {
  if (mode < 0 || mode > 2) return set_error("weight_grad: mode %d (0 auto, 1 transposes, 2 TN)", mode);
  if (Ny <= 0 || Nx <= 0 || rows <= 0) return 0;
  const RowMap ym{y_map_g, 0, y_map_gs, y_map_off}, xm{x_map_g, 0, x_map_gs, x_map_off};
  const bool tn_ok = mode != 1 && ym.g == 0 && ym.off == 0 && xm.g == 0 && xm.off == 0;
  if (!tn_ok && (!ta || !tb)) return set_error("weight_grad: the transpose path needs ta / tb scratch");
  return weight_grad((const bf16_t*)dy, lddy, ym, Ny, (const bf16_t*)x, ldx, xm, Nx, rows, (bf16_t*)ta, (bf16_t*)tb,
                     grad, part, part_floats, (hipStream_t)stream, mode == 0 ? -1 : (mode == 1 ? 0 : 2));
}

size_t ptk_siglip_workspace_bytes(const ptk_siglip_config* c, int batch) {
  Bump bp(nullptr);
  siglip_layout(bp, c, batch);
  return bp.off + 256;
}

int ptk_siglip_fwd(const ptk_siglip_config* c, const ptk_siglip_weights* wt, int B, const void* pixels, void* out,
                   void* ws, size_t ws_bytes, void* stream) {
  hipStream_t st = (hipStream_t)stream;
  if (ws_bytes < ptk_siglip_workspace_bytes(c, B)) return set_error("siglip_fwd: workspace too small");
  if (c->hidden % c->heads) return set_error("siglip_fwd: hidden %% heads");
  const int D = c->hidden, I = c->intermediate, P = c->patch_size, Hh = c->heads, hd = D / Hh;
  const int Nn = (c->image_size / P) * (c->image_size / P), Np = (Nn + 63) / 64 * 64, M = B * Nn;
  const int Kp = c->channels * P * P;
  if (Kp % 64 || hd % 64) return set_error("siglip_fwd: patch dim %d and head dim %d must be multiples of 64", Kp, hd);
  Bump bp(ws);
  SiglipWs w = siglip_layout(bp, c, B);
  TailScratchScope tail(w.tail, st);
  CK(tail.status);
  StageScope stage_all("siglip.fwd", st);
  StageSeq sq(st);
  sq.next("siglip.embed");

  CK(launch_im2col((const bf16_t*)pixels, w.patches, B, c->channels, c->image_size, c->image_size, P, st));
  {
    GemmArgs g = gemm(w.patches, Kp, wt->patch_w, Kp, w.h, D, M, D, Kp);
    g.bias = wt->patch_b;
    g.bf16_linear = 1;
    g.rowadd = wt->pos; g.rowadd_period = Nn; g.ld_rowadd = D;
    CK(launch_gemm(g, ACT_NONE, OUT_BF16, 1, st));
  }
  for (int l = 0; l < c->layers; ++l) {
    const ptk_siglip_layer& L = wt->layers[l];
    sq.next("siglip.attn");
    CK(launch_layernorm_bf16(w.h, L.ln1_w, L.ln1_b, w.a, M, D, c->eps, st));
    {
      GemmArgs g = gemm(w.a, D, L.wqkv, D, w.qkv, 3 * D, M, 3 * D, D, L.wqkv_kt);
      g.bias = L.bqkv;
      CK(launch_gemm(g, ACT_NONE, OUT_BF16, 1, st));
    }
    {
      FlashArgs fa;
      fa.Q = w.qkv; fa.K = w.qkv + D; fa.V = w.qkv + 2 * D; fa.O = w.o;
      fa.rows = Nn; fa.nkeys = Nn; fa.D = hd;
      fa.ldq = fa.ldk = 3 * D; fa.ldo = D;
      fa.zin = Hh; fa.zdiv = Hh;
      fa.sQ0 = fa.sK0 = (long)Nn * 3 * D; fa.sQ1 = fa.sK1 = hd;
      fa.sO0 = (long)Nn * D; fa.sO1 = hd;
      fa.scale = 1.0f / sqrtf((float)hd);
      StageScope sf("siglip.flash", st);
      CK(launch_attn_fwd(fa, B * Hh, st));
    }
    {
      GemmArgs g = gemm(w.o, D, L.wo, D, w.h, D, M, D, D, L.wo_kt);
      g.bias = L.bo; g.bf16_linear = 1; g.resid16 = w.h; g.ld_resid16 = D;
      CK(launch_gemm(g, ACT_NONE, OUT_BF16, 1, st));
    }
    sq.next("siglip.mlp");
    CK(launch_layernorm_bf16(w.h, L.ln2_w, L.ln2_b, w.a, M, D, c->eps, st));
    {
      GemmArgs g = gemm(w.a, D, L.w1, D, w.mlp, I, M, I, D, L.w1_kt);
      g.bias = L.b1;
      CK(launch_gemm(g, ACT_GELU_TANH, OUT_BF16, 1, st));
    }
    {
      GemmArgs g = gemm(w.mlp, I, L.w2, I, w.h, D, M, D, I, L.w2_kt);
      g.bias = L.b2; g.bf16_linear = 1; g.resid16 = w.h; g.ld_resid16 = D;
      CK(launch_gemm(g, ACT_NONE, OUT_BF16, 1, st));
    }
  }
  sq.next("siglip.post_norm");
  CK(launch_layernorm_bf16(w.h, wt->post_w, wt->post_b, (bf16_t*)out, M, D, c->eps, st));
  return 0;
}

size_t ptk_gemma3_workspace_bytes(const ptk_gemma3_config* c, int batch, int text_len, int seq_pad) {
  Bump bp(nullptr);
  gemma_layout(bp, c, batch, text_len, seq_pad);
  return bp.off + 256;
}

size_t ptk_gemma3_train_workspace_bytes(const ptk_gemma3_config* c, int batch, int text_len, int seq_pad) {
  Bump bp(nullptr);
  gemma_layout(bp, c, batch, text_len, seq_pad, true);
  return bp.off + 256;
}

}

namespace {

int gemma_run(const ptk_gemma3_config* c, const ptk_gemma3_weights* wt, const ptk_gemma3_batch* bt,
              const ptk_gemma3_grads* gr, void* ws, size_t ws_bytes, hipStream_t st, bool fwd_only = false) {
  const bool train = gr != nullptr;
  const int B = bt->batch, T = bt->text_len, Nv = bt->num_vision, Sp = bt->seq_pad, S = Nv + T;
  const int lo = bt->label_offset;
  if (Sp % 64 || S > Sp) return set_error("gemma3: seq_pad %d must be a multiple of 64 and >= %d", Sp, S);
  if (Sp > wt->rope_max_pos) return set_error("gemma3: seq_pad %d exceeds rope table (%d)", Sp, wt->rope_max_pos);
  if (c->heads % c->kv_heads) return set_error("gemma3: heads %% kv_heads");
  if (Nv < 1) return set_error("gemma3: num_vision must be >= 1");
  if (lo < 0 || lo >= T) return set_error("gemma3: label_offset %d outside [0, text_len %d)", lo, T);
  const size_t need = train ? ptk_gemma3_train_workspace_bytes(c, B, T, Sp) : ptk_gemma3_workspace_bytes(c, B, T, Sp);
  if (ws_bytes < need) return set_error("gemma3: workspace too small");
  if (c->vocab % 64 || c->vocab < 64 * LM_SPLITK) return set_error("gemma3: vocab must be a multiple of 64 and >= %d", 64 * LM_SPLITK);
  if (train && (!gr->layers || !gr->embed || !gr->final_norm)) return set_error("gemma3 train: grads missing");
  const int H = c->hidden, I = c->inter, D = c->head_dim, Hq = c->heads, Hkv = c->kv_heads, G = Hq / Hkv;
  const int M = B * Sp, Dq = Hq * D, Dqkv = (Hq + 2 * Hkv) * D, Tl = T - lo, R = B * Tl, V = c->vocab;
  const int Z = B * Hkv, SG = Sp * G, nl = c->layers;
  const float eps = c->eps, scale = 1.0f / sqrtf(c->query_pre_attn_scalar);
  Bump bp(ws);
  GemmaWs w = gemma_layout(bp, c, B, T, Sp, train);
  TailScratchScope tail(w.tail, st);
  CK(tail.status);
  AttnShape ash{B, Sp, Hq, Hkv, D};
  const RowMap ident{0, 0, 0, 0};
  const int Rp = (R + 63) / 64 * 64;
  StageSeq sq(st);
  sq.next("gemma.embed");

  const float escale = bfround_host(sqrtf((float)H));
  CK(launch_build_llm_inputs((const bf16_t*)wt->embed, bt->token_ids, B, T, Nv, S, Sp, H, escale, c->pad_token_id,
                             bt->x, w.key_valid, st));
  w.x[0] = bt->x;
  CK(launch_rmsnorm_fwd(w.x[0], H, ident, wt->layers[0].ln_in, train ? w.L[0].xn_in : w.xn, w.L[0].rstd_in, M, H,
                        eps, st));

  const RowMap lossmap{Tl, 0, Sp, Nv - 1 + lo};

  auto mlp_fwd = [&](int l, GemmArgs& g, GemmArgs& d) {
    const ptk_gemma3_layer& L = wt->layers[l];
    g = gemm(train ? w.L[l].xn_ff : w.xn, H, L.wgu, H, train ? w.L[l].h : w.h, I, M, 2 * I, H, L.wgu_kt);
    g.aux = w.L[l].glu_a; g.aux2 = w.L[l].glu_b; g.ld_aux = I;
    d = gemm(g.C, I, L.wd, I, w.L[l].dn, H, M, H, I, L.wd_kt);
  };
  auto mlp_bwd = [&](int l, GemmArgs& g, GemmArgs& d) {
    const ptk_gemma3_layer& L = wt->layers[l];
    g = gemm(w.dao, H, L.wd_t, H, w.dgu, 2 * I, M, I, H, L.wd_t_kt);
    g.aux_in = w.L[l].glu_a; g.aux_in2 = w.L[l].glu_b; g.ld_aux_in = I;
    d = gemm(w.dgu, 2 * I, L.wgu_t, 2 * I, w.dtmp, H, M, H, 2 * I, L.wgu_t_kt);
  };
  bool h_kt = false, dgu_kt = false, fac_kt = false;
  if (!train && nl > 1 && !geglu_split() && a_ktiled_mode()) {
    const GemmPlanEnv env = gemm_plan_env();
    h_kt = true;
    dgu_kt = !fwd_only;
    fac_kt = dgu_kt && a_ktiled_mode() != 2;
    for (int l = 0; l + 1 < nl; ++l) {
      GemmArgs gf, df, gb, db;
      mlp_fwd(l, gf, df);
      mlp_bwd(l, gb, db);
      h_kt = h_kt && gemm_ktiled_pair(gf, ACT_GEGLU, df, w.sk_floats, env, true, false);
      dgu_kt = dgu_kt && gemm_ktiled_pair(gb, ACT_GEGLU_BWD, db, w.sk_floats, env, true, false);
      fac_kt = fac_kt && gemm_ktiled_pair(gf, ACT_GEGLU, df, w.sk_floats, env, true, true) &&
               gemm_ktiled_pair(gb, ACT_GEGLU_BWD, db, w.sk_floats, env, true, true);
    }
  }

  for (int l = 0; l < nl; ++l) {
    const ptk_gemma3_layer& L = wt->layers[l];
    GemmaLayerSave& sv = w.L[l];
    const bool sliding = (l + 1) % c->sliding_pattern != 0;
    const float* cs = sliding ? wt->rope_cos_local : wt->rope_cos_global;
    const float* sn = sliding ? wt->rope_sin_local : wt->rope_sin_global;
    bf16_t* xin = train ? sv.xn_in : w.xn;
    bf16_t* xff = train ? sv.xn_ff : w.xn;
    bf16_t* hh = train ? sv.h : w.h;
    sq.next("gemma.fwd.attn");
    CK(gemm_split(gemm(xin, H, L.wqkv, H, sv.qkv, Dqkv, M, Dqkv, H, L.wqkv_kt), OUT_BF16, w.skpart, w.sk_floats, st));
    CK(launch_qknorm_rope_fwd(sv.qkv, L.q_norm, L.k_norm, cs, sn, ash, eps, sv.Q, sv.K, sv.V, sv.rstd_q, sv.rstd_k,
                              st));
    {
      FlashArgs fa;
      fa.Q = sv.Q; fa.K = sv.K; fa.V = sv.V; fa.O = sv.O; fa.lse = sv.lse;
      fa.rows = SG; fa.nkeys = Sp; fa.D = D;
      fa.ldq = D; fa.ldk = D; fa.ldo = D;
      fa.zin = Hkv; fa.zdiv = Hkv;
      fa.sQ0 = (long)Hkv * SG * D; fa.sQ1 = (long)SG * D;
      fa.sK0 = (long)Hkv * Sp * D; fa.sK1 = (long)Sp * D;
      fa.sO0 = (long)Sp * Hq * D; fa.sO1 = (long)G * D;
      fa.omap = RowMap{G, 0, Hq, 0};
      fa.qdiv = G; fa.causal = 1; fa.window = sliding ? c->sliding_window : 0;
      fa.key_valid = w.key_valid;
      fa.scale = scale;
      StageScope sf("gemma.fwd.flash", st);
      CK(launch_attn_fwd(fa, Z, st));
    }
    CK(gemm_split(gemm(sv.O, Dq, L.wo, Dq, sv.ao, H, M, H, Dq, L.wo_kt), OUT_BF16, w.skpart, w.sk_floats, st));
    CK(launch_residual_norm_fwd(sv.ao, w.x[l], L.ln_post_attn, L.ln_pre_ff, sv.x2, xff, sv.rstd_ao, sv.rstd_pre, M,
                                H, eps, st));
    sq.next("gemma.fwd.mlp");
    if (l + 1 < nl) {
      GemmArgs g, d;
      mlp_fwd(l, g, d);
      g.c_kt = d.a_kt = h_kt;
      g.aux_kt = fac_kt;
      CK(launch_gemm(g, ACT_GEGLU, OUT_BF16, 1, st));
      CK(gemm_split(d, OUT_BF16, w.skpart, w.sk_floats, st));
    } else {
      GemmArgs g = gemm(xff, H, L.wgu, H, hh, I, R, 2 * I, H, L.wgu_kt);
      g.amap = lossmap;
      g.aux = sv.glu_a; g.aux2 = sv.glu_b; g.ld_aux = I;
      CK(launch_gemm(g, ACT_GEGLU, OUT_BF16, 1, st));
      CK(launch_zero(sv.dn, (size_t)M * H * sizeof(bf16_t), st));
      GemmArgs g2 = gemm(hh, I, L.wd, I, sv.dn, H, R, H, I, L.wd_kt);
      g2.cmap = lossmap;
      CK(launch_gemm(g2, ACT_NONE, OUT_BF16, 1, st));
    }
    const float* wnext = (l + 1 < nl) ? wt->layers[l + 1].ln_in : nullptr;
    float* rnext = (l + 1 < nl) ? w.L[l + 1].rstd_in : nullptr;
    bf16_t* xnext = (train && l + 1 < nl) ? w.L[l + 1].xn_in : w.xn;
    CK(launch_residual_norm_fwd(sv.dn, sv.x2, L.ln_post_ff, wnext, w.x[l + 1], xnext, sv.rstd_dn, rnext, M, H, eps,
                                st));
  }

  sq.next("gemma.lm_head_ce");
  CK(launch_rmsnorm_fwd(w.x[nl], H, lossmap, wt->final_norm, w.xf, w.rstd_f, R, H, eps, st));
  {
    GemmArgs g = gemm(w.xf, H, wt->embed, H, w.logits, V, R, V, H);
    if (w.ce_stats && !ce_two_pass()) {
      g.row_stats = w.ce_stats;
      g.ld_stats = (V / 64) * 2;
      g.stats_only = lm_stats_only() ? 1 : 0;
    }
    CK(launch_gemm(g, ACT_NONE, OUT_BF16, 1, st));
    CK(launch_count_valid(bt->labels, R, bt->loss_scale, w.gscale, w.count, st));
    if (g.row_stats)
      CK(launch_ce_stats_fwd_bwd(w.logits, V, R, V, w.ce_stats, g.ld_stats, bt->labels, w.row_loss, w.gscale, st));
    else
      CK(launch_ce_fwd_bwd(w.logits, V, R, V, bt->labels, w.row_loss, w.gscale, st));
  }
  CK(launch_loss_reduce(w.row_loss, R, w.count, bt->loss, st));
  if (fwd_only) return 0;
  sq.next("gemma.lm_head_bwd");
  if (train) CK(weight_grad(w.logits, V, ident, V, w.xf, H, ident, H, R, w.TL, w.TX, gr->embed, w.skpart, w.sk_floats, st));
  const bool ks_fits = (double)R * V * 2 + (double)LM_KSLICES * (V / LM_KSLICES) * 2 < 4293918720.0;
  if (R % 256 == 0 && V % (64 * LM_KSLICES) == 0 && ks_fits) {
    GemmArgs g = gemm(w.logits, V, wt->embed_t, V, w.dxf_part, H, R, H, V / LM_KSLICES);
    CK(gemm_p8_kslices(g, LM_KSLICES, st));
    CK(launch_sum_partials(w.dxf_part, LM_KSLICES, (long)R * H, w.dxf, st));
  } else {
    const int kc = V / (64 * LM_SPLITK) * 64, rem = V - LM_SPLITK * kc;
    GemmArgs g = gemm(w.logits, V, wt->embed_t, V, w.dxf_part, H, R, H, kc);
    g.sA0 = kc; g.sB0 = kc; g.sC0 = (long)R * H;
    CK(launch_gemm(g, ACT_NONE, OUT_F32, LM_SPLITK, st));
    if (rem) {
      const long o = (long)LM_SPLITK * kc;
      CK(launch_gemm(gemm(w.logits + o, V, (const bf16_t*)wt->embed_t + o, V, w.dxf_part + (long)LM_SPLITK * R * H, H, R, H, rem),
                     ACT_NONE, OUT_F32, 1, st));
    }
    CK(launch_sum_partials(w.dxf_part, LM_SPLITK + (rem ? 1 : 0), (long)R * H, w.dxf, st));
  }
  float* dR = bt->dx;
  CK(launch_zero(dR, (size_t)M * H * 4, st));
  CK(launch_rmsnorm_bwd_scatter(w.x[nl], lossmap, wt->final_norm, w.rstd_f, w.dxf, dR, R, H, st));
  if (train)
    CK(launch_rms_wgrad(w.x[nl], H, lossmap, w.rstd_f, w.dxf, H, 1, R, H, (bf16_t*)gr->final_norm, w.wpart, st));

  for (int l = nl - 1; l >= 0; --l) {
    const ptk_gemma3_layer& L = wt->layers[l];
    const ptk_gemma3_layer_grads* GL = train ? &gr->layers[l] : nullptr;
    GemmaLayerSave& sv = w.L[l];
    const bool sliding = (l + 1) % c->sliding_pattern != 0;
    const float* cs = sliding ? wt->rope_cos_local : wt->rope_cos_global;
    const float* sn = sliding ? wt->rope_sin_local : wt->rope_sin_global;
    const bool last = l == nl - 1;
    sq.next("gemma.bwd.mlp");
    if (last) {
      CK(launch_post_norm_bwd(dR, sv.dn, L.ln_post_ff, sv.rstd_dn, w.dao, M, H, st));
      if (train)
        CK(launch_rms_wgrad_bx(sv.dn, H, ident, sv.rstd_dn, dR, H, 1, M, H, (bf16_t*)GL->ln_post_ff, w.wpart, st));
    }
    if (train)
      CK(last ? weight_grad(w.dao, H, lossmap, H, sv.h, I, ident, I, R, w.TA, w.TB, GL->wd, w.skpart, w.sk_floats, st)
              : weight_grad(w.dao, H, ident, H, sv.h, I, ident, I, M, w.TA, w.TB, GL->wd, w.skpart, w.sk_floats, st));
    if (!last) {
      if (geglu_split()) {
        CK(launch_gemm(gemm(w.dao, H, L.wd_t, H, w.h, I, M, I, H, L.wd_t_kt), ACT_NONE, OUT_BF16, 1, st));
        CK(launch_geglu_bwd(w.h, sv.glu_a, sv.glu_b, w.dgu, M, I, st));
      } else {
        GemmArgs g, d;
        mlp_bwd(l, g, d);
        g.c_kt = dgu_kt;
        g.aux_in_kt = fac_kt;
        CK(launch_gemm(g, ACT_GEGLU_BWD, OUT_BF16, 1, st));
      }
      if (train) CK(weight_grad(w.dgu, 2 * I, ident, 2 * I, sv.xn_ff, H, ident, H, M, w.TA, w.TB, GL->wgu, w.skpart, w.sk_floats, st));
      {
        GemmArgs g, d;
        mlp_bwd(l, g, d);
        d.a_kt = dgu_kt;
        CK(gemm_split(d, OUT_BF16, w.skpart, w.sk_floats, st));
      }
    } else {
      GemmArgs g = gemm(w.dao, H, L.wd_t, H, w.h, I, R, I, H, L.wd_t_kt);
      g.amap = lossmap;
      CK(launch_gemm(g, ACT_NONE, OUT_BF16, 1, st));
      CK(launch_geglu_bwd(w.h, sv.glu_a, sv.glu_b, w.dgu, R, I, st));
      if (train) CK(weight_grad(w.dgu, 2 * I, ident, 2 * I, sv.xn_ff, H, lossmap, H, R, w.TA, w.TB, GL->wgu, w.skpart, w.sk_floats, st));
      CK(launch_zero(w.dtmp, (size_t)M * H * sizeof(bf16_t), st));
      GemmArgs g2 = gemm(w.dgu, 2 * I, L.wgu_t, 2 * I, w.dtmp, H, R, H, 2 * I, L.wgu_t_kt);
      g2.cmap = lossmap;
      CK(launch_gemm(g2, ACT_NONE, OUT_BF16, 1, st));
    }
    sq.next("gemma.bwd.attn");
    CK(residual_norm_bwd_grads(sv.x2, L.ln_pre_ff, sv.rstd_pre, w.dtmp, dR, sv.ao, L.ln_post_attn, sv.rstd_ao, w.dao,
                               M, H, train ? (bf16_t*)GL->ln_pre_ff : nullptr,
                               train ? (bf16_t*)GL->ln_post_attn : nullptr, w.wpart, st));
    if (train)
      CK(weight_grad(w.dao, H, ident, H, sv.O, Dq, ident, Dq, M, w.TA, w.TB, GL->wo, w.skpart, w.sk_floats, st));
    {
      GemmArgs g = gemm(w.dao, H, L.wo_t, H, w.dO, (long)G * D, M, G * D, H, L.wo_t_kt);
      g.sB0 = (long)G * D * H; g.sC0 = (long)Sp * G * D;
      g.cmap = RowMap{Sp, 0, (long)Hkv * Sp, 0};
      CK(launch_gemm(g, ACT_NONE, OUT_BF16, Hkv, st));
    }
    FlashBwdArgs dkv_plan;
    dkv_plan.dkv_deferred = 0;
    {
      FlashBwdArgs fb;
      fb.Q = sv.Q; fb.K = sv.K; fb.V = sv.V; fb.O = sv.O; fb.dO = w.dO; fb.lse = sv.lse; fb.delta = w.delta;
      fb.dQ = w.dQ; fb.dK = w.dK; fb.dV = w.dV;
      fb.rows = SG; fb.nkeys = Sp; fb.D = D;
      fb.zin = Hkv; fb.zdiv = Hkv;
      fb.ldo = D; fb.sO0 = (long)Sp * Hq * D; fb.sO1 = (long)G * D;
      fb.omap = RowMap{G, 0, Hq, 0};
      fb.qdiv = G; fb.causal = 1; fb.window = sliding ? c->sliding_window : 0;
      fb.key_valid = w.key_valid;
      fb.scale = scale;
      fb.dkv_part = w.dkv_part; fb.dkv_part_bytes = w.dkv_part_bytes;
      StageScope sf("gemma.bwd.flash", st);
      CK(launch_attn_bwd(fb, Z, st, (dkv_reduce_split() || train) ? nullptr : &dkv_plan));
    }
    CK(launch_qknorm_rope_bwd(sv.qkv, L.q_norm, L.k_norm, cs, sn, ash, sv.rstd_q, sv.rstd_k, w.dQ, w.dK, w.dV, w.dqkv,
                              st, &dkv_plan));
    if (train) {
      CK(launch_qknorm_wgrad(sv.qkv, cs, sn, ash, sv.rstd_q, sv.rstd_k, w.dQ, w.dK, (bf16_t*)GL->q_norm,
                             (bf16_t*)GL->k_norm, w.wpart, st));
      CK(weight_grad(w.dqkv, Dqkv, ident, Dqkv, sv.xn_in, H, ident, H, M, w.TA, w.TB, GL->wqkv, w.skpart, w.sk_floats, st));
    }
    CK(gemm_split(gemm(w.dqkv, Dqkv, L.wqkv_t, Dqkv, w.dtmp, H, M, H, Dqkv, L.wqkv_t_kt), OUT_BF16, w.skpart, w.sk_floats, st));
    if (l > 0) {
      const ptk_gemma3_layer& Lp = wt->layers[l - 1];
      const GemmaLayerSave& sp = w.L[l - 1];
      CK(residual_norm_bwd_grads(w.x[l], L.ln_in, sv.rstd_in, w.dtmp, dR, sp.dn, Lp.ln_post_ff, sp.rstd_dn, w.dao,
                                 M, H, train ? (bf16_t*)GL->ln_in : nullptr,
                                 train ? (bf16_t*)gr->layers[l - 1].ln_post_ff : nullptr, w.wpart, st));
    } else {
      if (train)
        CK(launch_rms_wgrad_bdy(w.x[l], H, ident, sv.rstd_in, w.dtmp, H, M, H, (bf16_t*)GL->ln_in, w.wpart, st));
      CK(launch_rmsnorm_bwd_bdn(w.x[l], L.ln_in, sv.rstd_in, w.dtmp, dR, dR, M, H, st));
    }
  }
  if (train) sq.next("gemma.embed_grad");
  if (train) CK(launch_embed_grad(bt->token_ids, B, T, Nv, Sp, H, escale, dR, (bf16_t*)gr->embed, w.eg_keys, st));
  return 0;
}

}

namespace {

struct GenPass {
  float *xa, *xb, *x2, *rs1, *rs2, *rq, *rk;
  bf16_t *xn, *qkv, *Q, *K, *V, *O, *ao, *h, *dn;
  int32_t* kv;
  float* skp = nullptr;
  size_t skp_bytes = 0;
};
size_t gen_skinny_bytes(const ptk_gemma3_config* c, long rows) {
  if (rows > 256) return 0;
  rows = std::min<long>(rows, 64);
  const int H = c->hidden, I = c->inter, D = c->head_dim, Dq = c->heads * D, Dqkv = (c->heads + 2 * c->kv_heads) * D;
  const int M = (int)rows;
  const int shapes[5][2] = {{Dqkv, H}, {H, Dq}, {2 * I, H}, {H, I}, {c->vocab, H}};
  size_t b = 0;
  for (const auto& nk : shapes) b = std::max(b, skinny_part_bytes(M, nk[0], nk[1]));
  return b;
}
int gen_gemm(const GenPass& g, const bf16_t* A, long lda, const void* B, long ldb, bf16_t* C, long ldc, int M, int N,
             int K, int act, hipStream_t st) {
  if (g.skp_bytes > 0 && skinny_supported(std::min(M, 64), N, K, lda, ldb, ldc, act)) {
    for (int r0 = 0; r0 < M; r0 += 64)
      CK(launch_gemm_skinny(A + (long)r0 * lda, lda, (const bf16_t*)B, ldb, C + (long)r0 * ldc, ldc, std::min(64, M - r0),
                            N, K, act, g.skp, g.skp_bytes, st));
    return 0;
  }
  return launch_gemm(gemm(A, lda, B, ldb, C, ldc, M, N, K), act, OUT_BF16, 1, st);
}
struct GenWs {
  GenPass pre, dec;
  std::vector<bf16_t*> kc, vc;
  bf16_t *xf, *logits;
  float* rstd_f;
  int32_t* finished;
  int64_t *next, *feed;
  void* tail;
};
GenPass gen_pass(Bump& bp, const ptk_gemma3_config* c, long M) {
  const long H = c->hidden, I = c->inter, D = c->head_dim, Hq = c->heads, Hkv = c->kv_heads;
// ... 495 lines not shown
```

### projectiontrainer_amd/csrc/norm.hip

```cpp
#include "common.h"
#include "ptk_internal.h"

namespace ptk {

constexpr int MAXV = 12;

PTK_DEV float4 ld4(const float* p) { return *reinterpret_cast<const float4*>(p); }
PTK_DEV void st4(float* p, float4 v) { *reinterpret_cast<float4*>(p) = v; }
PTK_DEV float4 ld4bf(const bf16_t* p) {
  u16x4_t u = *reinterpret_cast<const u16x4_t*>(p);
  return make_float4(bf2f(u[0]), bf2f(u[1]), bf2f(u[2]), bf2f(u[3]));
}
PTK_DEV void st4bf(bf16_t* p, float4 v) {
  u16x4_t u;
  u[0] = f2bf(v.x); u[1] = f2bf(v.y); u[2] = f2bf(v.z); u[3] = f2bf(v.w);
  *reinterpret_cast<u16x4_t*>(p) = u;
}
PTK_DEV float dot4(float4 a, float4 b) { return a.x * b.x + a.y * b.y + a.z * b.z + a.w * b.w; }
PTK_DEV float4 bfr4(float4 v) { return make_float4(bfround(v.x), bfround(v.y), bfround(v.z), bfround(v.w)); }
PTK_DEV float4 onep(float4 w) { return make_float4(1.f + w.x, 1.f + w.y, 1.f + w.z, 1.f + w.w); }
PTK_DEV float4 mul4(float4 a, float4 b) { return make_float4(a.x * b.x, a.y * b.y, a.z * b.z, a.w * b.w); }
PTK_DEV float4 add4(float4 a, float4 b) { return make_float4(a.x + b.x, a.y + b.y, a.z + b.z, a.w + b.w); }
PTK_DEV float4 scl4(float4 a, float s) { return make_float4(a.x * s, a.y * s, a.z * s, a.w * s); }

#define ROW_SETUP                                          \
  const int lane = threadIdx.x & 63;                       \
  const long row = (long)blockIdx.x * 4 + (threadIdx.x >> 6); \
  if (row >= rows) return;

#define FOR_V for (int v = 0; v < NV; ++v) if (v < NV - 1 || lane * 4 + v * 256 < cols)
#define COL (lane * 4 + v * 256)

PTK_DEV float4 ldx4(const float* p) { return ld4(p); }
PTK_DEV float4 ldx4(const bf16_t* p) { return ld4bf(p); }

template <typename T, int NV>
PTK_DEV void layernorm_body(const T* __restrict__ x, const float* __restrict__ w, const float* __restrict__ b,
                            bf16_t* __restrict__ y, long rows, int cols, float eps) {
  ROW_SETUP
  float4 r[NV];
  float s = 0.f;
#pragma unroll
  FOR_V { r[v] = ldx4(x + row * cols + COL); s += r[v].x + r[v].y + r[v].z + r[v].w; }
  const float mean = warp_sum(s) / cols;
  float q = 0.f;
#pragma unroll
  FOR_V {
    float4 d = make_float4(r[v].x - mean, r[v].y - mean, r[v].z - mean, r[v].w - mean);
    r[v] = d;
    q += dot4(d, d);
  }
  const float rstd = rsqrtf(warp_sum(q) / cols + eps);
#pragma unroll
  FOR_V { st4bf(y + row * cols + COL, add4(mul4(scl4(r[v], rstd), ld4(w + COL)), ld4(b + COL))); }
}

template <int NV>
__global__ void __launch_bounds__(256) layernorm_f32(const float* __restrict__ x, const float* __restrict__ w,
                                                     const float* __restrict__ b, bf16_t* __restrict__ y, long rows,
                                                     int cols, float eps) {
  layernorm_body<float, NV>(x, w, b, y, rows, cols, eps);
}
template <int NV>
__global__ void __launch_bounds__(256) layernorm_b16(const bf16_t* __restrict__ x, const float* __restrict__ w,
                                                     const float* __restrict__ b, bf16_t* __restrict__ y, long rows,
                                                     int cols, float eps) {
  layernorm_body<bf16_t, NV>(x, w, b, y, rows, cols, eps);
}

template <int NV>
__global__ void __launch_bounds__(256) rmsnorm_fwd_kernel(const float* __restrict__ x, long ldx, RowMap xmap,
                                                          const float* __restrict__ w, bf16_t* __restrict__ y,
                                                          float* __restrict__ rstd_out, long rows, int cols,
                                                          float eps) {
  ROW_SETUP
  const float* xr = x + map_row(xmap, row) * ldx;
  float4 r[NV];
  float q = 0.f;
#pragma unroll
  FOR_V { r[v] = ld4(xr + COL); q += dot4(r[v], r[v]); }
  const float rs = rsqrtf(warp_sum(q) / cols + eps);
  if (lane == 0 && rstd_out) rstd_out[row] = rs;
#pragma unroll
  FOR_V { st4bf(y + row * cols + COL, mul4(scl4(r[v], rs), onep(ld4(w + COL)))); }
}

template <int NV>
__global__ void __launch_bounds__(256) residual_norm_fwd_kernel(
    const bf16_t* __restrict__ t, const float* __restrict__ xi, const float* __restrict__ w_post,
    const float* __restrict__ w_next, float* __restrict__ xo, bf16_t* __restrict__ n,
    float* __restrict__ rstd_t, float* __restrict__ rstd_x, long rows, int cols, float eps) {
  ROW_SETUP
  float4 r[NV];
  float q = 0.f;
#pragma unroll
  FOR_V { r[v] = ld4bf(t + row * cols + COL); q += dot4(r[v], r[v]); }
  const float rs = rsqrtf(warp_sum(q) / cols + eps);
  if (lane == 0) rstd_t[row] = rs;
  float q2 = 0.f;
#pragma unroll
  FOR_V {
    float4 yv = bfr4(mul4(scl4(r[v], rs), onep(ld4(w_post + COL))));
    float4 xv = add4(ld4(xi + row * cols + COL), yv);
    st4(xo + row * cols + COL, xv);
    r[v] = xv;
    q2 += dot4(xv, xv);
  }
  if (!w_next) return;
  const float rs2 = rsqrtf(warp_sum(q2) / cols + eps);
  if (lane == 0) rstd_x[row] = rs2;
#pragma unroll
  FOR_V { st4bf(n + row * cols + COL, mul4(scl4(r[v], rs2), onep(ld4(w_next + COL)))); }
}

#define RMS_BWD_BODY(XV, DNV, RS, OUTEXPR)                                   \
  {                                                                           \
    float sdot = 0.f;                                                         \
    _Pragma("unroll") FOR_V { sdot += dot4(mul4(DNV[v], onep(ld4(w + COL))), XV[v]); } \
    sdot = warp_sum(sdot);                                                    \
    const float c3 = RS * RS * RS * sdot / cols;                              \
    _Pragma("unroll") FOR_V {                                                 \
      float4 dxv = add4(scl4(mul4(DNV[v], onep(ld4(w + COL))), RS), scl4(XV[v], -c3)); \
      OUTEXPR;                                                                \
    }                                                                         \
  }

template <typename TD, int NV>
PTK_DEV void rmsnorm_bwd_body(const float* __restrict__ x, const float* __restrict__ w, const float* __restrict__ rstd,
                              const TD* __restrict__ dn, const float* dacc, float* dx, long rows, int cols) {
  ROW_SETUP
  float4 xv[NV], dv[NV];
#pragma unroll
  FOR_V { xv[v] = ld4(x + row * cols + COL); dv[v] = ldx4(dn + row * cols + COL); }
  const float rs = rstd[row];
  RMS_BWD_BODY(xv, dv, rs, {
    float4 o = dacc ? add4(ld4(dacc + row * cols + COL), dxv) : dxv;
    st4(dx + row * cols + COL, o);
  })
}
template <int NV>
__global__ void __launch_bounds__(256) rmsnorm_bwd_f32_kernel(const float* __restrict__ x, const float* __restrict__ w,
                                                              const float* __restrict__ rstd, const float* __restrict__ dn,
                                                              const float* dacc, float* dx, long rows, int cols) {
  rmsnorm_bwd_body<float, NV>(x, w, rstd, dn, dacc, dx, rows, cols);
}
template <int NV>
__global__ void __launch_bounds__(256) rmsnorm_bwd_bdn_kernel(const float* __restrict__ x, const float* __restrict__ w,
                                                              const float* __restrict__ rstd, const bf16_t* __restrict__ dn,
                                                              const float* dacc, float* dx, long rows, int cols) {
  rmsnorm_bwd_body<bf16_t, NV>(x, w, rstd, dn, dacc, dx, rows, cols);
}

template <int NV>
__global__ void __launch_bounds__(256) rmsnorm_bwd_scatter_kernel(const float* __restrict__ x, RowMap xmap,
                                                                  const float* __restrict__ w,
                                                                  const float* __restrict__ rstd,
                                                                  const float* __restrict__ dn, float* dR,
                                                                  long rows, int cols) {
  ROW_SETUP
  const long xr = map_row(xmap, row);
  float4 xv[NV], dv[NV];
#pragma unroll
  FOR_V { xv[v] = ld4(x + xr * cols + COL); dv[v] = ld4(dn + row * cols + COL); }
  const float rs = rstd[row];
  RMS_BWD_BODY(xv, dv, rs, { st4(dR + xr * cols + COL, add4(ld4(dR + xr * cols + COL), dxv)); })
}

template <int NV>
PTK_DEV void post_norm_bwd_row(const float* dR, const bf16_t* t, const float* w, float rs, bf16_t* dt, int lane,
                               int cols) {
  float4 xv[NV], dv[NV];
#pragma unroll
  FOR_V { xv[v] = ld4bf(t + COL); dv[v] = bfr4(ld4(dR + COL)); }
  RMS_BWD_BODY(xv, dv, rs, { st4bf(dt + COL, dxv); })
}

template <typename TD, int NV>
PTK_DEV void residual_norm_bwd_body(
    const float* __restrict__ x2, const float* __restrict__ w_pre, const float* __restrict__ rstd_pre,
    const TD* __restrict__ dn, float* __restrict__ dR, const bf16_t* __restrict__ t,
    const float* __restrict__ w_post, const float* __restrict__ rstd_t, bf16_t* __restrict__ dt, long rows,
    int cols) {
  ROW_SETUP
  float4 nd[NV];
  {
    const float* w = w_pre;
    float4 xv[NV], dv[NV];
#pragma unroll
    FOR_V { xv[v] = ld4(x2 + row * cols + COL); dv[v] = ldx4(dn + row * cols + COL); }
    const float rs = rstd_pre[row];
    RMS_BWD_BODY(xv, dv, rs, {
      nd[v] = add4(ld4(dR + row * cols + COL), dxv);
      st4(dR + row * cols + COL, nd[v]);
    })
  }
  {
    const float* w = w_post;
    const float rs = rstd_t[row];
    float4 xv[NV], dv[NV];
#pragma unroll
    FOR_V { xv[v] = ld4bf(t + row * cols + COL); dv[v] = bfr4(nd[v]); }
    RMS_BWD_BODY(xv, dv, rs, { st4bf(dt + row * cols + COL, dxv); })
  }
}
template <int NV>
__global__ void __launch_bounds__(256) residual_norm_bwd_kernel(
    const float* __restrict__ x2, const float* __restrict__ w_pre, const float* __restrict__ rstd_pre,
    const float* __restrict__ dn, float* __restrict__ dR, const bf16_t* __restrict__ t,
    const float* __restrict__ w_post, const float* __restrict__ rstd_t, bf16_t* __restrict__ dt, long rows,
    int cols) {
  residual_norm_bwd_body<float, NV>(x2, w_pre, rstd_pre, dn, dR, t, w_post, rstd_t, dt, rows, cols);
}
template <int NV>
__global__ void __launch_bounds__(256) residual_norm_bwd_bdn_kernel(
    const float* __restrict__ x2, const float* __restrict__ w_pre, const float* __restrict__ rstd_pre,
    const bf16_t* __restrict__ dn, float* __restrict__ dR, const bf16_t* __restrict__ t,
    const float* __restrict__ w_post, const float* __restrict__ rstd_t, bf16_t* __restrict__ dt, long rows,
    int cols) {
  residual_norm_bwd_body<bf16_t, NV>(x2, w_pre, rstd_pre, dn, dR, t, w_post, rstd_t, dt, rows, cols);
}

#ifndef PTK_NWG_WAVES
#define PTK_NWG_WAVES 4
#endif
constexpr int NWG = PTK_NWG_WAVES;
template <int NV>
__global__ void __launch_bounds__(64 * NWG) residual_norm_bwd_wg_kernel(
    const float* __restrict__ x2, const float* __restrict__ w_pre, const float* __restrict__ rstd_pre,
    const bf16_t* __restrict__ dn, float* __restrict__ dR, const bf16_t* __restrict__ t,
    const float* __restrict__ w_post, const float* __restrict__ rstd_t, bf16_t* __restrict__ dt, long rows,
    int cols, float* __restrict__ part_pre, float* __restrict__ part_post) {
  __shared__ float4 red[NWG][NV][64];
  const int lane = threadIdx.x & 63, wv = threadIdx.x >> 6;
  const long row = (long)blockIdx.x * NWG + wv;
  const bool ok = row < rows;
#define NWG_SUM(PART)                                                                    \
  __syncthreads();                                                                       \
  if (wv == 0) {                                                                         \
    float* part = PART + (long)blockIdx.x * cols;                                        \
    _Pragma("unroll") FOR_V {                                                            \
      float4 a = red[0][v][lane];                                                        \
      _Pragma("unroll") for (int g = 1; g < NWG; ++g) a = add4(a, red[g][v][lane]);      \
      st4(part + COL, a);                                                                \
    }                                                                                    \
  }                                                                                      \
  __syncthreads();
  float4 nd[NV];
  if (ok) {
    const float* w = w_pre;
    float4 xv[NV], dv[NV];
#pragma unroll
    FOR_V { xv[v] = ld4(x2 + row * cols + COL); dv[v] = ld4bf(dn + row * cols + COL); }
    const float rs = rstd_pre[row];
#pragma unroll
    FOR_V { red[wv][v][lane] = scl4(mul4(dv[v], xv[v]), rs); }
    RMS_BWD_BODY(xv, dv, rs, {
      nd[v] = add4(ld4(dR + row * cols + COL), dxv);
      st4(dR + row * cols + COL, nd[v]);
    })
  } else {
#pragma unroll
    for (int v = 0; v < NV; ++v) red[wv][v][lane] = make_float4(0.f, 0.f, 0.f, 0.f);
  }
  NWG_SUM(part_pre)
  if (ok) {
    const float* w = w_post;
    const float rs = rstd_t[row];
    float4 xv[NV], dv[NV];
#pragma unroll
    FOR_V { xv[v] = ld4bf(t + row * cols + COL); dv[v] = bfr4(nd[v]); }
#pragma unroll
    FOR_V { red[wv][v][lane] = scl4(mul4(dv[v], xv[v]), rs); }
    RMS_BWD_BODY(xv, dv, rs, { st4bf(dt + row * cols + COL, dxv); })
  } else {
#pragma unroll
    for (int v = 0; v < NV; ++v) red[wv][v][lane] = make_float4(0.f, 0.f, 0.f, 0.f);
  }
  NWG_SUM(part_post)
#undef NWG_SUM
}

template <int NV>
__global__ void __launch_bounds__(256) post_norm_bwd_kernel(const float* __restrict__ dR, const bf16_t* __restrict__ t,
                                                            const float* __restrict__ w, const float* __restrict__ rstd_t,
                                                            bf16_t* __restrict__ dt, long rows, int cols) {
  ROW_SETUP
  post_norm_bwd_row<NV>(dR + row * cols, t + row * cols, w, rstd_t[row], dt + row * cols, lane, cols);
}

#define NORM_DISPATCH(KERNEL, ...)                                                                  \
  do {                                                                                              \
    switch ((cols + 255) / 256) {                                                                   \
      case 1: hipLaunchKernelGGL(KERNEL<1>, NORM_GRID, __VA_ARGS__); break;                         \
      case 2: hipLaunchKernelGGL(KERNEL<2>, NORM_GRID, __VA_ARGS__); break;                         \
      case 3: hipLaunchKernelGGL(KERNEL<3>, NORM_GRID, __VA_ARGS__); break;                         \
      case 4: hipLaunchKernelGGL(KERNEL<4>, NORM_GRID, __VA_ARGS__); break;                         \
      case 5: hipLaunchKernelGGL(KERNEL<5>, NORM_GRID, __VA_ARGS__); break;                         \
      case 6: hipLaunchKernelGGL(KERNEL<6>, NORM_GRID, __VA_ARGS__); break;                         \
      case 7: hipLaunchKernelGGL(KERNEL<7>, NORM_GRID, __VA_ARGS__); break;                         \
      case 8: hipLaunchKernelGGL(KERNEL<8>, NORM_GRID, __VA_ARGS__); break;                         \
      case 9: hipLaunchKernelGGL(KERNEL<9>, NORM_GRID, __VA_ARGS__); break;                         \
      case 10: hipLaunchKernelGGL(KERNEL<10>, NORM_GRID, __VA_ARGS__); break;                       \
      case 11: hipLaunchKernelGGL(KERNEL<11>, NORM_GRID, __VA_ARGS__); break;                       \
      default: hipLaunchKernelGGL(KERNEL<MAXV>, NORM_GRID, __VA_ARGS__); break;                     \
    }                                                                                               \
  } while (0)

static int check_cols(int cols) {
  if (cols <= 0 || cols % 4 || cols > 256 * MAXV) return set_error("norm: cols=%d unsupported", cols);
  return 0;
}
#define NORM_GRID dim3((unsigned)((rows + 3) / 4)), dim3(256), 0, st
#define RET_LAUNCH(name) return hipGetLastError() == hipSuccess ? 0 : set_error(name " launch failed")

int launch_layernorm(const float* x, const float* w, const float* b, bf16_t* y, int rows, int cols, float eps,
                     hipStream_t st) {
  if (check_cols(cols)) return -1;
  if (rows <= 0) return 0;
  NORM_DISPATCH(layernorm_f32, x, w, b, y, (long)rows, cols, eps);
  RET_LAUNCH("layernorm");
}
int launch_layernorm_bf16(const bf16_t* x, const float* w, const float* b, bf16_t* y, int rows, int cols, float eps,
                          hipStream_t st) {
  if (check_cols(cols)) return -1;
  if (rows <= 0) return 0;
  NORM_DISPATCH(layernorm_b16, x, w, b, y, (long)rows, cols, eps);
  RET_LAUNCH("layernorm_bf16");
}
int launch_rmsnorm_fwd(const float* x, long ldx, RowMap xmap, const float* w, bf16_t* y, float* rstd, int rows,
                       int cols, float eps, hipStream_t st) {
  if (check_cols(cols)) return -1;
  if (rows <= 0) return 0;
  NORM_DISPATCH(rmsnorm_fwd_kernel, x, ldx, xmap, w, y, rstd, (long)rows, cols, eps);
  RET_LAUNCH("rmsnorm_fwd");
}
int launch_residual_norm_fwd(const bf16_t* t, const float* xi, const float* w_post, const float* w_next, float* xo,
                             bf16_t* n, float* rstd_t, float* rstd_x, int rows, int cols, float eps,
                             hipStream_t st) {
  if (check_cols(cols)) return -1;
  if (rows <= 0) return 0;
  NORM_DISPATCH(residual_norm_fwd_kernel, t, xi, w_post, w_next, xo, n, rstd_t, rstd_x,
                     (long)rows, cols, eps);
  RET_LAUNCH("residual_norm_fwd");
}
int launch_rmsnorm_bwd_f32(const float* x, const float* w, const float* rstd, const float* dn, const float* dacc,
                           float* dx, int rows, int cols, hipStream_t st) {
  if (check_cols(cols)) return -1;
  if (rows <= 0) return 0;
  NORM_DISPATCH(rmsnorm_bwd_f32_kernel, x, w, rstd, dn, dacc, dx, (long)rows, cols);
  RET_LAUNCH("rmsnorm_bwd");
}
int launch_rmsnorm_bwd_bdn(const float* x, const float* w, const float* rstd, const bf16_t* dn, const float* dacc,
                           float* dx, int rows, int cols, hipStream_t st) {
  if (check_cols(cols)) return -1;
  if (rows <= 0) return 0;
  NORM_DISPATCH(rmsnorm_bwd_bdn_kernel, x, w, rstd, dn, dacc, dx, (long)rows, cols);
  RET_LAUNCH("rmsnorm_bwd_bdn");
}
int launch_residual_norm_bwd_bdn(const float* x2, const float* w_pre, const float* rstd_pre, const bf16_t* dn,
                                 float* dR, const bf16_t* t, const float* w_post, const float* rstd_t, bf16_t* dt,
                                 int rows, int cols, hipStream_t st) {
  if (check_cols(cols)) return -1;
  if (rows <= 0) return 0;
  NORM_DISPATCH(residual_norm_bwd_bdn_kernel, x2, w_pre, rstd_pre, dn, dR, t, w_post, rstd_t, dt, (long)rows, cols);
  RET_LAUNCH("residual_norm_bwd_bdn");
}
int residual_norm_bwd_wg_blocks(int rows) { return (rows + NWG - 1) / NWG; }
int launch_residual_norm_bwd_wg(const float* x2, const float* w_pre, const float* rstd_pre, const bf16_t* dn,
                                float* dR, const bf16_t* t, const float* w_post, const float* rstd_t, bf16_t* dt,
                                int rows, int cols, float* part_pre, float* part_post, hipStream_t st) {
  if (check_cols(cols)) return -1;
  if (rows <= 0) return 0;
#undef NORM_GRID
#define NORM_GRID dim3((unsigned)residual_norm_bwd_wg_blocks(rows)), dim3(64 * NWG), 0, st
  NORM_DISPATCH(residual_norm_bwd_wg_kernel, x2, w_pre, rstd_pre, dn, dR, t, w_post, rstd_t, dt, (long)rows, cols,
                part_pre, part_post);
#undef NORM_GRID
#define NORM_GRID dim3((unsigned)((rows + 3) / 4)), dim3(256), 0, st
  RET_LAUNCH("residual_norm_bwd_wg");
}
int launch_rmsnorm_bwd_scatter(const float* x, RowMap xmap, const float* w, const float* rstd, const float* dn,
                               float* dR, int rows, int cols, hipStream_t st) {
  if (check_cols(cols)) return -1;
  if (rows <= 0) return 0;
  NORM_DISPATCH(rmsnorm_bwd_scatter_kernel, x, xmap, w, rstd, dn, dR, (long)rows, cols);
  RET_LAUNCH("rmsnorm_bwd_scatter");
}
int launch_residual_norm_bwd(const float* x2, const float* w_pre, const float* rstd_pre, const float* dn, float* dR,
                             const bf16_t* t, const float* w_post, const float* rstd_t, bf16_t* dt, int rows,
                             int cols, hipStream_t st) {
  if (check_cols(cols)) return -1;
  if (rows <= 0) return 0;
  NORM_DISPATCH(residual_norm_bwd_kernel, x2, w_pre, rstd_pre, dn, dR, t, w_post, rstd_t, dt,
                     (long)rows, cols);
  RET_LAUNCH("residual_norm_bwd");
}
int launch_post_norm_bwd(const float* dR, const bf16_t* t, const float* w, const float* rstd_t, bf16_t* dt,
                         int rows, int cols, hipStream_t st) {
  if (check_cols(cols)) return -1;
  if (rows <= 0) return 0;
  NORM_DISPATCH(post_norm_bwd_kernel, dR, t, w, rstd_t, dt, (long)rows, cols);
  RET_LAUNCH("post_norm_bwd");
}

}
```

### projectiontrainer_amd/csrc/ptk_internal.h

```cpp
#pragma once
#include <hip/hip_runtime.h>
#include <stddef.h>
#include <stdint.h>

#include <type_traits>

#include "common.h"

namespace ptk {

int set_error(const char* fmt, ...);

#ifdef PTK_AB_ENV
}
#include <cstdlib>
namespace ptk {
inline int ab_env(const char* name, int dflt) { const char* e = getenv(name); return e && *e ? atoi(e) : dflt; }
#define PTK_AB(NAME, DFLT) ([] { static const int v_ = ::ptk::ab_env(NAME, DFLT); return v_; }())
#else
#define PTK_AB(NAME, DFLT) (DFLT)
#endif

enum Act { ACT_NONE = 0, ACT_GELU_TANH = 1, ACT_GELU_ERF = 2, ACT_GEGLU = 3,
           ACT_GELU_ERF_BWD = 4, ACT_GEGLU_BWD = 5 };
enum Out { OUT_BF16 = 0, OUT_F32 = 1, OUT_F32_BFR = 2 };

struct GemmArgs {
  const bf16_t* A = nullptr;
  const bf16_t* B = nullptr;
  void* C = nullptr;
  int M = 0, N = 0, K = 0;
  long lda = 0, ldb = 0, ldc = 0;
  int zin = 1;
  long sA0 = 0, sA1 = 0, sB0 = 0, sB1 = 0, sC0 = 0, sC1 = 0;
  float alpha = 1.f;
  const float* bias = nullptr;
  const float* rowadd = nullptr;
  int rowadd_period = 1;
  long ld_rowadd = 0;
  const float* resid = nullptr;
  long ld_resid = 0;
  const bf16_t* resid16 = nullptr;
  long ld_resid16 = 0;
  int bf16_linear = 0;
  bf16_t* aux = nullptr;
  bf16_t* aux2 = nullptr;
  long ld_aux = 0;
  const bf16_t* aux_in = nullptr;
  const bf16_t* aux_in2 = nullptr;
  long ld_aux_in = 0;
  RowMap amap{0, 0, 0, 0};
  RowMap cmap{0, 0, 0, 0};
  float* row_stats = nullptr;
  long ld_stats = 0;
  int stats_only = 0;
  void* tail_ws = nullptr;
  const bf16_t* B_kt = nullptr;
  int a_kt = 0, c_kt = 0, aux_kt = 0, aux_in_kt = 0;
};

enum GemmPath { GEMM_PATH_NT = 0, GEMM_PATH_BIG = 1, GEMM_PATH_BIG2 = 2, GEMM_PATH_W4 = 3, GEMM_PATH_NTB = 4,
                GEMM_PATH_P8SK = 5, GEMM_PATH_P8 = 6, GEMM_PATH_TN = 7, GEMM_NPATH = 9 };
int path_counts(int64_t* out, int reset);
int ktiled_counts(int64_t* out2, int reset);
int device_cus();

template <class F>
inline bool gemm_act_out(int act, int out, F&& f) {
#define PTK_ACT_OUT(ACT_, OUT_)                                                          \
  if (act == ACT_ && out == OUT_) {                                                      \
    f(std::integral_constant<int, ACT_>{}, std::integral_constant<int, OUT_>{});         \
    return true;                                                                         \
  }
  PTK_ACT_OUT(ACT_NONE, OUT_BF16)
  PTK_ACT_OUT(ACT_NONE, OUT_F32)
  PTK_ACT_OUT(ACT_NONE, OUT_F32_BFR)
  PTK_ACT_OUT(ACT_GELU_TANH, OUT_BF16)
  PTK_ACT_OUT(ACT_GELU_ERF, OUT_BF16)
  PTK_ACT_OUT(ACT_GEGLU, OUT_BF16)
  PTK_ACT_OUT(ACT_GELU_ERF_BWD, OUT_BF16)
  PTK_ACT_OUT(ACT_GEGLU_BWD, OUT_BF16)
#undef PTK_ACT_OUT
  return false;
}

constexpr int W4 = 256;
constexpr int W4_KT = 64;
struct P8Tail {
  int dp_tiles = 0;
  int units = 0;
  int gsplit = 0;
  float* slab = nullptr;
  int zslices = 1;
};
constexpr size_t P8_WAVE_FLOATS = 128 * 64;
constexpr size_t P8_CNT_BYTES = 16384;
struct GemmPlanEnv {
  int ncu = 256;
  int force_tiles = 0;
  bool p8_all = false;
  bool tm_short = true;
  bool lean_epi = true;
  bool streamk = true;
  void* tail_scope = nullptr;
};
GemmPlanEnv gemm_plan_env();
struct GemmPlan {
  int path = GEMM_PATH_NT;
  int tm = 256;
  P8Tail tail;
  bool single_round = false;
};
GemmPlan gemm_plan(const GemmArgs& a, int act, int out, int batch, const GemmPlanEnv& env);
constexpr bool bkt_act(int act) { return act != ACT_GELU_ERF && act != ACT_GELU_ERF_BWD; }
long kstep_tile_offset(long row, long k, long K);
bool b_ktiled_ok(const GemmArgs& a, const GemmPlan& plan, int act, int batch);
bool a_ktiled_ok(const GemmArgs& a, const GemmPlan& plan, int act, int out, int batch, bool lean_epi);
bool c_ktiled_ok(const GemmArgs& a, const GemmPlan& plan, int act, int out, int batch, bool lean_epi);
bool gemm_ktiled_pair(const GemmArgs& prod, int pact, const GemmArgs& cons, long part_floats, const GemmPlanEnv& env,
                      bool enabled, bool factors);
int a_ktiled_mode();
int launch_gemm(const GemmArgs& a, int act, int out, int batch, hipStream_t st, const GemmPlan* planned = nullptr);
struct GemmSplitPlan {
  int slices = 1, kc = 0, rem = 0;
  bool tail_ws = false;
  GemmPlan direct;
};
GemmSplitPlan gemm_split_plan(const GemmArgs& a, int out, long part_floats, const GemmPlanEnv& env);
bool w4_supported(const GemmArgs& a, int act, int out);
int launch_gemm_w4(const GemmArgs& a, int act, int out, hipStream_t st, int max_grid);
double w4_round_fill(long M, long N, int ncu);
bool p8_supported(const GemmArgs& a, int act, int out);
int launch_gemm_p8(const GemmArgs& a, int act, int out, hipStream_t st, const P8Tail& tail, int tm = 256);
int p8_tile_height(const GemmArgs& a, int act, int out, int ncu);
int launch_gemm_p8_kslices(const GemmArgs& a, int slices, hipStream_t st);
int gemm_p8_kslices(const GemmArgs& a, int slices, hipStream_t st);
bool lean_epilogue_candidate(const GemmArgs& a, bool lean_epi);
bool lean_epilogue_ok(const GemmArgs& a, int act, int out, uint32_t& c_bytes, bool lean_epi);
bool lean_epilogue_enabled();
bool tn_supported(const GemmArgs& a, int out, int slices, bool lean_epi);
int tn_slices(const GemmArgs& a, long part_floats, const GemmPlanEnv& env);
P8Tail tn_tail_plan(const GemmArgs& a, void* slab, int ncu);
size_t tn_slab_bytes();
int launch_gemm_tn(const GemmArgs& a, int out, int slices, void* slab, hipStream_t st, long k_rows = -1);
int gemm_tn(const GemmArgs& a, int out, int slices, void* slab, hipStream_t st, long k_rows = -1);
int wgrad_tn_enabled();
size_t p8_tail_scratch_bytes();
size_t p8_tail_scratch_bytes_models();
size_t p8_slab_bytes(long G);
bool streamk_enabled();
P8Tail p8_tail_plan_ws(const GemmArgs& a, long ntile, long G, void* slab, long max_t0, long max_t1);
P8Tail p8_tail_plan(const GemmArgs& a, int act, int out, const GemmPlanEnv& env);
void* tail_scope();
struct TailScratchScope {
  void* prev;
  int status = 0;
  TailScratchScope(void* ws, hipStream_t st);
  ~TailScratchScope();
};
bool stage_timers_on();
void stage_begin(const char* name, hipStream_t st);
int stage_end(hipStream_t st);
struct StageScope {
  hipStream_t st;
  bool on;
  StageScope(const char* name, hipStream_t s) : st(s), on(stage_timers_on()) { if (on) stage_begin(name, s); }
  ~StageScope() { if (on) (void)stage_end(st); }
};
struct StageSeq {
  hipStream_t st;
  bool on, open = false;
  explicit StageSeq(hipStream_t s) : st(s), on(stage_timers_on()) {}
  void next(const char* name) {
    if (!on) return;
    if (open) (void)stage_end(st);
    stage_begin(name, st);
    open = true;
  }
  ~StageSeq() { if (on && open) (void)stage_end(st); }
};
void timer_enable(int on);
void force_small_tiles(int mode);
int timer_read(int cls, double* total_ms, int* count);

int launch_layernorm(const float* x, const float* w, const float* b, bf16_t* y, int rows, int cols,
                     float eps, hipStream_t st);
int launch_layernorm_bf16(const bf16_t* x, const float* w, const float* b, bf16_t* y, int rows, int cols,
                          float eps, hipStream_t st);
int launch_rmsnorm_fwd(const float* x, long ldx, RowMap xmap, const float* w, bf16_t* y, float* rstd,
                       int rows, int cols, float eps, hipStream_t st);
int launch_residual_norm_fwd(const bf16_t* t, const float* xi, const float* w_post, const float* w_next,
                             float* xo, bf16_t* n, float* rstd_t, float* rstd_x, int rows, int cols,
                             float eps, hipStream_t st);
int launch_rmsnorm_bwd_f32(const float* x, const float* w, const float* rstd, const float* dn,
                           const float* dacc, float* dx, int rows, int cols, hipStream_t st);
int launch_residual_norm_bwd(const float* x2, const float* w_pre, const float* rstd_pre, const float* dn,
                             float* dR, const bf16_t* t, const float* w_post, const float* rstd_t,
                             bf16_t* dt, int rows, int cols, hipStream_t st);
int launch_post_norm_bwd(const float* dR, const bf16_t* t, const float* w, const float* rstd_t, bf16_t* dt,
                         int rows, int cols, hipStream_t st);
int launch_rmsnorm_bwd_bdn(const float* x, const float* w, const float* rstd, const bf16_t* dn, const float* dacc,
                           float* dx, int rows, int cols, hipStream_t st);
int launch_residual_norm_bwd_bdn(const float* x2, const float* w_pre, const float* rstd_pre, const bf16_t* dn,
                                 float* dR, const bf16_t* t, const float* w_post, const float* rstd_t, bf16_t* dt,
                                 int rows, int cols, hipStream_t st);
int residual_norm_bwd_wg_blocks(int rows);
int launch_residual_norm_bwd_wg(const float* x2, const float* w_pre, const float* rstd_pre, const bf16_t* dn,
                                float* dR, const bf16_t* t, const float* w_post, const float* rstd_t, bf16_t* dt,
                                int rows, int cols, float* part_pre, float* part_post, hipStream_t st);
int launch_rmsnorm_bwd_scatter(const float* x, RowMap xmap, const float* w, const float* rstd,
                               const float* dn, float* dR, int rows, int cols, hipStream_t st);

struct AttnShape {
  int B, S, Hq, Hkv, D;
  const int32_t* pos = nullptr;
};
int launch_qknorm_rope_fwd(const bf16_t* qkv, const float* qw, const float* kw, const float* cos_t,
                           const float* sin_t, AttnShape s, float eps, bf16_t* Q, bf16_t* K, bf16_t* V,
                           float* rstd_q, float* rstd_k, hipStream_t st);
int launch_qknorm_rope_bwd(const bf16_t* qkv, const float* qw, const float* kw, const float* cos_t,
                           const float* sin_t, AttnShape s, const float* rstd_q, const float* rstd_k,
                           const bf16_t* dQ, const bf16_t* dK, const bf16_t* dV, bf16_t* dqkv,
                           hipStream_t st, const struct FlashBwdArgs* dkv = nullptr);
struct MaskSpec {
  int rows_per_batch;
  int qdiv;
  int zdiv;
  int causal;
  int window;
  const int32_t* key_valid;
  int key_len;
};
int launch_softmax_fwd(const float* S, bf16_t* P, int nz, int rows, int cols, long ld, MaskSpec m,
                       hipStream_t st);
int launch_softmax_bwd(const bf16_t* P, const float* dP, bf16_t* dS, int nrows, int cols, long ld,
                       float scale, hipStream_t st);

struct FlashArgs {
  const bf16_t* Q = nullptr;
  const bf16_t* K = nullptr;
  const bf16_t* V = nullptr;
  bf16_t* O = nullptr;
  float* lse = nullptr;
  int rows = 0, nkeys = 0, D = 0;
  long ldq = 0, ldk = 0, ldo = 0;
  int zin = 1, zdiv = 1;
  long sQ0 = 0, sQ1 = 0, sK0 = 0, sK1 = 0, sO0 = 0, sO1 = 0;
  RowMap qmap{0, 0, 0, 0}, omap{0, 0, 0, 0};
  int qdiv = 1, causal = 0, window = 0;
  const int32_t* key_valid = nullptr;
  float scale = 1.f;
  int variant = 0;
};
int launch_attn_fwd(const FlashArgs& a, int nz, hipStream_t st);
struct FlashBwdArgs {
  const bf16_t* Q = nullptr;
  const bf16_t* K = nullptr;
  const bf16_t* V = nullptr;
// ... 157 lines not shown
```

### projectiontrainer_amd/kernels.py

```python
from __future__ import annotations

import os

import torch

from . import _lib as L
from ._lib import check, ptr


def _require_cuda(*ts):
    for t in ts:
        if t is not None and not t.is_cuda:
            raise L.PtkError("libptk ops need HIP device tensors (no CPU fallback)")


def _bits(t):
    return ptr(t)


def gemm(A, B, *, C=None, out_dtype=torch.bfloat16, act=L.ACT_NONE, alpha=1.0, bias=None, rowadd=None,
         resid=None, aux=None, aux2=None, aux_in=None, aux_in2=None, M=None, N=None, K=None,
         lda=None, ldb=None, ldc=None, batch=1, batch_inner=1, strides=(0, 0, 0, 0, 0, 0),
         amap=(0, 0, 0, 0), cmap=(0, 0, 0, 0), out_mode=None, resid16=None, bf16_linear=False, tail_ws=None,
         B_kt=None, A_kt=False, C_kt=False, aux_kt=False, aux_in_kt=False):
    _require_cuda(A, B)
    M = A.shape[-2] if M is None else M
    K = A.shape[-1] if K is None else K
    N = B.shape[-2] if N is None else N
    n_out = N // 2 if act == L.ACT_GEGLU else (2 * N if act == L.ACT_GEGLU_BWD else N)
    if C is None:
        C = torch.empty((M, n_out), dtype=out_dtype, device=A.device)
    if out_mode is None:
        out_mode = L.OUT_BF16 if C.dtype == torch.bfloat16 else L.OUT_F32
    d = L.GemmDesc()
    d.A, d.B, d.C = ptr(A), ptr(B), ptr(C)
    d.M, d.N, d.K = M, N, K
    d.lda = A.stride(-2) if lda is None else lda
    d.ldb = B.stride(-2) if ldb is None else ldb
    d.ldc = C.stride(-2) if ldc is None else ldc
    d.batch, d.batch_inner = batch, batch_inner
    d.sA0, d.sA1, d.sB0, d.sB1, d.sC0, d.sC1 = strides
    d.alpha, d.act, d.out = alpha, act, out_mode
    d.bias = ptr(bias)
    if rowadd is not None:
        d.rowadd, d.rowadd_period, d.ld_rowadd = ptr(rowadd), rowadd.shape[0], rowadd.stride(0)
    if resid is not None:
        d.resid, d.ld_resid = ptr(resid), resid.stride(-2)
    if aux is not None:
        d.aux, d.ld_aux = ptr(aux), aux.stride(-2)
    d.aux2 = ptr(aux2)
    if aux_in is not None:
        d.aux_in, d.ld_aux_in = ptr(aux_in), aux_in.stride(-2)
    d.aux_in2 = ptr(aux_in2)
    d.amap = L.RowMap(*amap)
    d.cmap = L.RowMap(*cmap)
    if resid16 is not None:
        d.resid16, d.ld_resid16 = ptr(resid16), resid16.stride(-2)
    d.bf16_linear = int(bool(bf16_linear))
    d.tail_ws = ptr(tail_ws)
    d.B_kt = ptr(B_kt)
    d.A_kt, d.C_kt, d.aux_kt, d.aux_in_kt = int(bool(A_kt)), int(bool(C_kt)), int(bool(aux_kt)), int(bool(aux_in_kt))
    check(L.lib().ptk_gemm(d, L.stream_ptr(A.device)), "ptk_gemm")
    return C


def layernorm(x, w, b, eps):
    _require_cuda(x)
    y = torch.empty(x.shape, dtype=torch.bfloat16, device=x.device)
    rows, cols = x.numel() // x.shape[-1], x.shape[-1]
    check(L.lib().ptk_layernorm(ptr(x), ptr(w), ptr(b), ptr(y), rows, cols, eps, L.stream_ptr(x.device)), "layernorm")
    return y


def rmsnorm(x, w, eps):
    _require_cuda(x)
    rows, cols = x.numel() // x.shape[-1], x.shape[-1]
    y = torch.empty(x.shape, dtype=torch.bfloat16, device=x.device)
    rstd = torch.empty(rows, dtype=torch.float32, device=x.device)
    check(L.lib().ptk_rmsnorm(ptr(x), ptr(w), ptr(y), ptr(rstd), rows, cols, eps, L.stream_ptr(x.device)), "rmsnorm")
    return y, rstd


def rmsnorm_bwd(x, w, rstd, dn, dacc=None):
    rows, cols = x.numel() // x.shape[-1], x.shape[-1]
    dx = torch.empty_like(x)
    check(L.lib().ptk_rmsnorm_bwd(ptr(x), ptr(w), ptr(rstd), ptr(dn), ptr(dacc), ptr(dx), rows, cols,
                                  L.stream_ptr(x.device)), "rmsnorm_bwd")
    return dx


def qknorm_rope(qkv, q_w, k_w, cos_t, sin_t, *, batch, seq, heads, kv_heads, head_dim, eps):
    _require_cuda(qkv)
    dev, G = qkv.device, heads // kv_heads
    Q = torch.empty(batch, kv_heads, seq, G, head_dim, dtype=torch.bfloat16, device=dev)
    K = torch.empty(batch, kv_heads, seq, head_dim, dtype=torch.bfloat16, device=dev)
    V = torch.empty_like(K)
    rq = torch.empty(batch * seq, heads, dtype=torch.float32, device=dev)
    rk = torch.empty(batch * seq, kv_heads, dtype=torch.float32, device=dev)
    check(L.lib().ptk_qknorm_rope_fwd(ptr(qkv), ptr(q_w), ptr(k_w), ptr(cos_t), ptr(sin_t), batch, seq, heads, kv_heads,
                                      head_dim, eps, ptr(Q), ptr(K), ptr(V), ptr(rq), ptr(rk), L.stream_ptr(dev)),
          "qknorm_rope_fwd")
    return Q, K, V, rq, rk


def qknorm_rope_bwd(qkv, q_w, k_w, cos_t, sin_t, rq, rk, dQ, dK, dV, *, batch, seq, heads, kv_heads, head_dim):
    _require_cuda(qkv)
    dqkv = torch.empty_like(qkv)
    check(L.lib().ptk_qknorm_rope_bwd(ptr(qkv), ptr(q_w), ptr(k_w), ptr(cos_t), ptr(sin_t), batch, seq, heads,
                                      kv_heads, head_dim, ptr(rq), ptr(rk), ptr(dQ), ptr(dK), ptr(dV), ptr(dqkv),
                                      L.stream_ptr(qkv.device)), "qknorm_rope_bwd")
    return dqkv


def softmax(S, *, nz, rows, cols, rows_per_batch=0, qdiv=1, zdiv=1, causal=False, window=0, key_valid=None,
            key_len=None):
    P = torch.empty(S.shape, dtype=torch.bfloat16, device=S.device)
    check(L.lib().ptk_softmax(ptr(S), ptr(P), nz, rows, cols, S.stride(-2), rows_per_batch, qdiv, zdiv, int(causal),
                              window, ptr(key_valid), cols if key_len is None else key_len,
                              L.stream_ptr(S.device)), "softmax")
    return P


def cross_entropy_(logits, targets, gscale):
    R, V = logits.shape
# ... 147 lines not shown
```

Before: 337.4 images/sec.

## Let norm kernels write k-step-tiled rows consumed directly by following GEMMs

Result: no change. 340.4 images/sec (median of 6 runs) (+0.9%).

```diff
diff --git a/include/ptk.h b/include/ptk.h
--- a/include/ptk.h
+++ b/include/ptk.h
@@ -62,6 +62,11 @@
 int ptk_gemm_ktiled_pair(const ptk_gemm_desc* producer, const ptk_gemm_desc* consumer, int ncu, int64_t part_floats,
                          int train);
 int ptk_a_ktiled_reload(void);
+int ptk_gemm_row_ktiled_pair(const ptk_gemm_desc* consumer, int ncu, int64_t part_floats, int via_split, int kind,
+                             int train);
+int ptk_row_ktiled_reload(void);
+int64_t ptk_gemm_row_ktiled_count(int reset);
+int64_t ptk_row_ktile_lane_offset(int64_t row, int lane, int v, int cols);
 int ptk_gemm(const ptk_gemm_desc* d, void* stream);
 int64_t ptk_kstep_tile_offset(int64_t row, int64_t k, int64_t K);
 int ptk_pack_kstep_tiles_bf16(const void* src, void* dst, int N, int K, void* stream);
@@ -78,6 +83,13 @@
                 void* stream);
 int ptk_rmsnorm_bwd(const float* x, const float* w, const float* rstd, const float* dn, const float* dacc,
                     float* dx, int rows, int cols, void* stream);
+int ptk_residual_norm_fwd(const void* t, const float* xi, const float* w_post, const float* w_next, float* xo, void* n,
+                          float* rstd_t, float* rstd_x, int rows, int cols, float eps, int kt, void* stream);
+int ptk_residual_norm_bwd_bdn(const float* x2, const float* w_pre, const float* rstd_pre, const void* dn, float* dR,
+                              const void* t, const float* w_post, const float* rstd_t, void* dt, int rows, int cols,
+                              int kt, void* stream);
+int ptk_layernorm_bf16(const void* x, const float* w, const float* b, void* y, int rows, int cols, float eps, int kt,
+                       void* stream);
 int ptk_qknorm_rope_fwd(const void* qkv, const float* q_norm_w, const float* k_norm_w, const float* cos_t,
                         const float* sin_t, int batch, int seq, int heads, int kv_heads, int head_dim, float eps,
                         void* Q, void* K, void* V, float* rstd_q, float* rstd_k, void* stream);
diff --git a/projectiontrainer_amd/_lib.py b/projectiontrainer_amd/_lib.py
--- a/projectiontrainer_amd/_lib.py
+++ b/projectiontrainer_amd/_lib.py
@@ -171,6 +171,13 @@
     "ptk_gemm_ktiled_counts": (c_int, [c_void_p, c_int]),
     "ptk_gemm_ktiled_pair": (c_int, [C.POINTER(GemmDesc), C.POINTER(GemmDesc), c_int, c_int64, c_int]),
     "ptk_a_ktiled_reload": (c_int, []),
+    "ptk_gemm_row_ktiled_pair": (c_int, [C.POINTER(GemmDesc), c_int, c_int64, c_int, c_int, c_int]),
+    "ptk_row_ktiled_reload": (c_int, []),
+    "ptk_gemm_row_ktiled_count": (c_int64, [c_int]),
+    "ptk_row_ktile_lane_offset": (c_int64, [c_int64, c_int, c_int, c_int]),
+    "ptk_layernorm_bf16": (c_int, [c_void_p, c_void_p, c_void_p, c_void_p, c_int, c_int, c_float, c_int, c_void_p]),
+    "ptk_residual_norm_fwd": (c_int, [c_void_p] * 8 + [c_int, c_int, c_float, c_int, c_void_p]),
+    "ptk_residual_norm_bwd_bdn": (c_int, [c_void_p] * 9 + [c_int, c_int, c_int, c_void_p]),
     "ptk_stage_timers_enable": (c_int, [c_int]),
     "ptk_stage_begin": (c_int, [C.c_char_p, c_void_p]),
     "ptk_stage_end": (c_int, [c_void_p]),
@@ -295,6 +302,10 @@
     return int(buf[0]), int(buf[1])
 
 
+def gemm_row_ktiled_count(reset=False):
+    return int(lib().ptk_gemm_row_ktiled_count(int(reset)))
+
+
 _stages_on = os.environ.get("PTK_STAGE_TIMERS", "0") not in ("", "0")
 
 
diff --git a/projectiontrainer_amd/csrc/capi.cpp b/projectiontrainer_amd/csrc/capi.cpp
--- a/projectiontrainer_amd/csrc/capi.cpp
+++ b/projectiontrainer_amd/csrc/capi.cpp
@@ -110,6 +110,25 @@
   return launch_layernorm(x, w, b, (bf16_t*)y, rows, cols, eps, ST);
 }
 
+int ptk_layernorm_bf16(const void* x, const float* w, const float* b, void* y, int rows, int cols, float eps, int kt,
+                       void* stream) {
+  return launch_layernorm_bf16((const bf16_t*)x, w, b, (bf16_t*)y, rows, cols, eps, ST, kt);
+}
+int ptk_residual_norm_fwd(const void* t, const float* xi, const float* w_post, const float* w_next, float* xo, void* n,
+                          float* rstd_t, float* rstd_x, int rows, int cols, float eps, int kt, void* stream) {
+  return launch_residual_norm_fwd((const bf16_t*)t, xi, w_post, w_next, xo, (bf16_t*)n, rstd_t, rstd_x, rows, cols, eps,
+                                  ST, kt);
+}
+int ptk_residual_norm_bwd_bdn(const float* x2, const float* w_pre, const float* rstd_pre, const void* dn, float* dR,
+                              const void* t, const float* w_post, const float* rstd_t, void* dt, int rows, int cols,
+                              int kt, void* stream) {
+  return launch_residual_norm_bwd_bdn(x2, w_pre, rstd_pre, (const bf16_t*)dn, dR, (const bf16_t*)t, w_post, rstd_t,
+                                      (bf16_t*)dt, rows, cols, ST, kt);
+}
+int64_t ptk_row_ktile_lane_offset(int64_t row, int lane, int v, int cols) {
+  return row_ktile_lane_offset((long)row, lane, v, cols);
+}
+
 int ptk_rmsnorm(const float* x, const float* w, void* y, float* rstd, int rows, int cols, float eps, void* stream) {
   return launch_rmsnorm_fwd(x, cols, RowMap{0, 0, 0, 0}, w, (bf16_t*)y, rstd, rows, cols, eps, ST);
 }
@@ -186,6 +205,15 @@
   return !train && gemm_ktiled_pair(to_args(producer), producer->act, to_args(consumer), (long)part_floats,
                                     test_plan_env(ncu), a_ktiled_mode() != 0, true) ? 1 : 0;
 }
+
+int ptk_gemm_row_ktiled_pair(const ptk_gemm_desc* consumer, int ncu, int64_t part_floats, int via_split, int kind,
+                             int train) {
+  if (!consumer || ncu <= 0) return 0;
+  return !train && row_ktiled_pair(to_args(consumer), consumer->act, consumer->batch > 0 ? consumer->batch : 1,
+                                   via_split != 0, (long)part_floats, test_plan_env(ncu),
+                                   (row_ktiled_mode() & kind) != 0) ? 1 : 0;
+}
+int64_t ptk_gemm_row_ktiled_count(int reset) { return row_ktiled_count(reset); }
 
 int ptk_fill_normal_bf16(void* out, int64_t n, uint64_t seed, float std, float mean, void* stream) {
   return launch_fill_normal_bf16((bf16_t*)out, n, seed, std, mean, ST);
diff --git a/projectiontrainer_amd/csrc/gemm.hip b/projectiontrainer_amd/csrc/gemm.hip
--- a/projectiontrainer_amd/csrc/gemm.hip
+++ b/projectiontrainer_amd/csrc/gemm.hip
@@ -670,7 +670,12 @@
   return 0;
 }
 
-static long g_kt_count[2];
+static long g_kt_count[2], g_row_kt_count;
+int64_t row_ktiled_count(int reset) {
+  const int64_t v = g_row_kt_count;
+  if (reset) g_row_kt_count = 0;
+  return v;
+}
 int ktiled_counts(int64_t* out2, int reset) {
   for (int i = 0; i < 2; ++i) {
     if (out2) out2[i] = g_kt_count[i];
@@ -717,7 +722,8 @@
   if (!c_ktiled_ok(a, plan, act, out, batch, lean_epilogue_enabled()))
     return set_error("gemm: this launch cannot write k-step-tiled outputs");
   GemmLaunchScope scope(plan.path, act, st);
-  g_kt_count[0] += a.a_kt != 0;
+  g_kt_count[0] += a.a_kt != 0 && a.a_kt != A_KT_ROW;
+  g_row_kt_count += a.a_kt == A_KT_ROW;
   g_kt_count[1] += a.c_kt != 0;
   const dim3 grid_big((unsigned)((long)((a.M + BIG - 1) / BIG) * ((a.N + BIG - 1) / BIG)), 1, 1);
   switch (plan.path) {
diff --git a/projectiontrainer_amd/csrc/gemm_plan.cpp b/projectiontrainer_amd/csrc/gemm_plan.cpp
--- a/projectiontrainer_amd/csrc/gemm_plan.cpp
+++ b/projectiontrainer_amd/csrc/gemm_plan.cpp
@@ -209,9 +209,16 @@
 }
 
 bool a_ktiled_ok(const GemmArgs& a, const GemmPlan& plan, int act, int out, int batch, bool lean_epi) {
-  if (batch != 1 || act != ACT_NONE || out != OUT_BF16 || plan.path != GEMM_PATH_P8 || plan.tail.units) return false;
+  if (batch != 1 || out != OUT_BF16) return false;
   if (a.M % 16 || a.K % 32 || a.lda != a.K || a.amap.g != 0 || a.amap.off < 0 || a.amap.off % 16) return false;
-  (void)lean_epi;
+  if (plan.path == GEMM_PATH_W4) {
+    uint32_t cb = 0;
+    if (act != ACT_GEGLU && !(act == ACT_GEGLU_BWD && lean_epilogue_ok(a, act, out, cb, lean_epi))) return false;
+  } else if (plan.path == GEMM_PATH_P8 && !plan.tail.units) {
+    if (act != ACT_NONE && !(act == ACT_GELU_TANH && plan.tm == 192)) return false;
+  } else {
+    return false;
+  }
   return b_ktiled_ok(a, plan, act, batch);
 }
 
@@ -244,6 +251,23 @@
   if (sp.kc != 0 || sp.tail_ws) return false;
   const GemmPlan cp = env.force_tiles == 0 ? sp.direct : gemm_plan(cons, ACT_NONE, OUT_BF16, 1, env);
   return a_ktiled_ok(c, cp, ACT_NONE, OUT_BF16, 1, env.lean_epi);
+}
+
+bool row_ktiled_pair(const GemmArgs& cons, int act, int batch, bool via_split, long part_floats, const GemmPlanEnv& env,
+                     bool enabled) {
+  if (!enabled || batch != 1) return false;
+  GemmArgs c = cons;
+  c.a_kt = A_KT_ROW;
+  GemmPlan plan;
+  if (via_split) {
+    if (act != ACT_NONE) return false;
+    const GemmSplitPlan sp = gemm_split_plan(cons, OUT_BF16, part_floats, env);
+    if (sp.kc != 0 || sp.tail_ws) return false;
+    plan = env.force_tiles == 0 ? sp.direct : gemm_plan(cons, act, OUT_BF16, 1, env);
+  } else {
+    plan = gemm_plan(cons, act, OUT_BF16, 1, env);
+  }
+  return a_ktiled_ok(c, plan, act, OUT_BF16, 1, env.lean_epi);
 }
 
 GemmSplitPlan gemm_split_plan(const GemmArgs& a, int out, long part_floats, const GemmPlanEnv& env) {
diff --git a/projectiontrainer_amd/csrc/gemm_w4.hip b/projectiontrainer_amd/csrc/gemm_w4.hip
--- a/projectiontrainer_amd/csrc/gemm_w4.hip
+++ b/projectiontrainer_amd/csrc/gemm_w4.hip
@@ -22,7 +22,7 @@
 
 namespace ptk {
 
-template <int ACT, int OUT, bool LEAN = false, bool BKT = false, int KTO = 0>
+template <int ACT, int OUT, bool LEAN = false, bool BKT = false, int KTO = 0, bool AKT = false>
 __global__ void __launch_bounds__(256, 1) gemm_w4_kernel(GemmArgs p, uint32_t a_bytes, uint32_t b_bytes,
                                                          uint32_t c_bytes) {
   __shared__ __attribute__((aligned(16))) char smem[W4_NSLOT * W4_SLOT];
@@ -44,6 +44,7 @@
 
   constexpr bool bkt = BKT;
   constexpr uint32_t bks = BKT ? 1024u : (uint32_t)(W4_KS * 2);
+  constexpr uint32_t aks = AKT ? 1024u : (uint32_t)(W4_KS * 2);
   const u32x4_t rsa = w4_rsrc(p.A, a_bytes), rsb = w4_rsrc(bkt ? p.B_kt : p.B, b_bytes);
 
   uint32_t offa[4], offb[4];
@@ -51,7 +52,8 @@
   for (int j = 0; j < 4; ++j) {
     const int lr = wave * 64 + 16 * j + (lane >> 2);
     const int lc = (lane & 3) ^ ((lane >> 3) & 2);
-    offa[j] = (uint32_t)lr * (uint32_t)p.lda * 2u + lc * 16;
+    offa[j] = AKT ? (uint32_t)(wave * 4 + j) * (uint32_t)p.K * 32u + lane * 16
+                  : (uint32_t)lr * (uint32_t)p.lda * 2u + lc * 16;
     offb[j] = bkt ? (uint32_t)(wave * 4 + j) * (uint32_t)p.K * 32u + lane * 16
                   : (uint32_t)lr * (uint32_t)p.ldb * 2u + lc * 16;
   }
@@ -108,7 +110,7 @@
     constexpr bool first = decltype(first_c)::value;
     const uint32_t ba = frag_a + rs, bb = frag_b + rs;
     const uint32_t da = lds_dma + ws, db = da + W4_SOPB;
-    const uint32_t sa = dsa + dks * (W4_KS * 2), sb = dsb + dks * bks;
+    const uint32_t sa = dsa + dks * aks, sb = dsb + dks * bks;
 #pragma unroll
     for (int q = 0; q < 16; ++q) {
 #if PTK_W4_RDS == 1
@@ -148,7 +150,7 @@
 #pragma unroll
   for (int b = 0; b < 4; ++b) {
     const uint32_t da = lds_dma + b * W4_SLOT, db = da + W4_SOPB;
-    const uint32_t sa = dsa + dks * (W4_KS * 2), sb = dsb + dks * bks;
+    const uint32_t sa = dsa + dks * aks, sb = dsb + dks * bks;
 #pragma unroll
     for (int j = 0; j < 4; ++j) {
       W4_DMA(rsa, offa[j], sa, da + j * 1024);
@@ -223,6 +225,16 @@
 template <int ACT, int OUT, bool LEAN>
 static void w4_launch(const GemmArgs& a, long grid, hipStream_t st, uint32_t ab, uint32_t bb, uint32_t cb) {
   if constexpr ((ACT == ACT_GEGLU && !LEAN) || (ACT == ACT_GEGLU_BWD && LEAN)) {
+    if (a.a_kt && a.B_kt) {
+      const dim3 g((unsigned)grid), b(256);
+      if (!a.c_kt)
+        hipLaunchKernelGGL((gemm_w4_kernel<ACT, OUT, LEAN, true, 0, true>), g, b, 0, st, a, ab, bb, cb);
+      else if (a.aux_kt || a.aux_in_kt)
+        hipLaunchKernelGGL((gemm_w4_kernel<ACT, OUT, LEAN, true, 3, true>), g, b, 0, st, a, ab, bb, cb);
+      else
+        hipLaunchKernelGGL((gemm_w4_kernel<ACT, OUT, LEAN, true, 1, true>), g, b, 0, st, a, ab, bb, cb);
+      return;
+    }
     if (a.c_kt && a.B_kt) {
       if (a.aux_kt || a.aux_in_kt)
         hipLaunchKernelGGL((gemm_w4_kernel<ACT, OUT, LEAN, true, 3>), dim3((unsigned)grid), dim3(256), 0, st, a, ab, bb, cb);
@@ -251,6 +263,8 @@
   const uint32_t bb = (uint32_t)std::min<double>((double)a.N * a.ldb * 2, 2147483000.0);
   uint32_t cb = 0;
   const bool lean = lean_epilogue_ok(a, act, out, cb, lean_epilogue_enabled());
+  if (a.a_kt && !(a.B_kt && (act == ACT_GEGLU || (act == ACT_GEGLU_BWD && lean))))
+    return set_error("gemm_w4: no k-step-tiled-A variant for this launch");
   if (a.c_kt || a.aux_kt || a.aux_in_kt) {
     if (!a.c_kt || !a.B_kt || !((act == ACT_GEGLU && !a.aux_in_kt) || (act == ACT_GEGLU_BWD && lean && !a.aux_kt)))
       return set_error("gemm_w4: no k-step-tiled-output variant for this launch");
@@ -682,6 +696,13 @@
       return;
     }
   }
+  if constexpr (ACT == ACT_GELU_TANH && OUT == OUT_BF16 && !SK && TM == 192) {
+    if (a.a_kt && a.B_kt) {
+      hipLaunchKernelGGL((gemm_p8_kernel<ACT, OUT, SK, LEAN, TM, true, true>), dim3((unsigned)grid), dim3(512), 0, st, a,
+                         ab, bb, tl, cb);
+      return;
+    }
+  }
   if constexpr (bkt_act(ACT)) {
     if (a.B_kt) {
       hipLaunchKernelGGL((gemm_p8_kernel<ACT, OUT, SK, LEAN, TM, true>), dim3((unsigned)grid), dim3(512), 0, st, a, ab,
@@ -720,7 +741,8 @@
   const long ncu = device_cus();
   const bool lean_epi = lean_epilogue_enabled();
   if (a.a_kt) {
-    if (act != ACT_NONE || out != OUT_BF16 || tl.units || !a.B_kt)
+    const bool epi = act == ACT_NONE || (act == ACT_GELU_TANH && tm == 192);
+    if (!epi || out != OUT_BF16 || tl.units || !a.B_kt)
       return set_error("gemm_p8: no k-step-tiled-A variant for this launch");
   }
   if (tm != 256 && !tl.units) {
diff --git a/projectiontrainer_amd/csrc/models.cpp b/projectiontrainer_amd/csrc/models.cpp
--- a/projectiontrainer_amd/csrc/models.cpp
+++ b/projectiontrainer_amd/csrc/models.cpp
@@ -55,9 +55,11 @@
 
 static int residual_norm_bwd_grads(const float* x2, const float* w_pre, const float* rstd_pre, const bf16_t* dn,
                                    float* dR, const bf16_t* t, const float* w_post, const float* rstd_t, bf16_t* dt,
-                                   int M, int H, bf16_t* g_pre, bf16_t* g_post, float* wpart, hipStream_t st) {
+                                   int M, int H, bf16_t* g_pre, bf16_t* g_post, float* wpart, hipStream_t st,
+                                   int dt_kt = 0) {
   const RowMap ident{0, 0, 0, 0};
   if (g_pre && norm_wg_fused()) {
+    if (dt_kt) return set_error("residual_norm_bwd: the weight-grad path takes no k-step-tiled dt");
     const int nb = residual_norm_bwd_wg_blocks(M);
     float* pq = wpart + rms_wgrad_finish_floats(nb, H);
     CK(launch_residual_norm_bwd_wg(x2, w_pre, rstd_pre, dn, dR, t, w_post, rstd_t, dt, M, H, wpart, pq, st));
@@ -65,7 +67,8 @@
     return launch_rms_wgrad_finish(pq, nb, H, g_post, st);
   }
   if (g_pre) CK(launch_rms_wgrad_bdy(x2, H, ident, rstd_pre, dn, H, M, H, g_pre, wpart, st));
-  CK(launch_residual_norm_bwd_bdn(x2, w_pre, rstd_pre, dn, dR, t, w_post, rstd_t, dt, M, H, st));
+  if (g_pre && dt_kt) return set_error("residual_norm_bwd: the weight-grad path takes no k-step-tiled dt");
+  CK(launch_residual_norm_bwd_bdn(x2, w_pre, rstd_pre, dn, dR, t, w_post, rstd_t, dt, M, H, st, dt_kt));
   if (g_pre) CK(launch_rms_wgrad_bx(t, H, ident, rstd_t, dR, H, 1, M, H, g_post, wpart, st));
   return 0;
 }
@@ -89,8 +92,17 @@
 }
 
 static int g_a_ktiled = -1;
+constexpr int PTK_ROW_KTILED_ALL = 15, PTK_ROW_KTILED_DEFAULT = 7;
+static int g_row_ktiled = -1;
 }
 namespace ptk {
+int row_ktiled_mode() {
+  if (g_row_ktiled < 0) {
+    const char* e = getenv("PTK_ROW_KTILED");
+    g_row_ktiled = e && e[0] ? (atoi(e) & PTK_ROW_KTILED_ALL) : PTK_ROW_KTILED_DEFAULT;
+  }
+  return g_row_ktiled;
+}
 int a_ktiled_mode() {
   if (g_a_ktiled < 0) {
     const char* e = getenv("PTK_A_KTILED");
@@ -102,6 +114,10 @@
 extern "C" int ptk_a_ktiled_reload(void) {
   g_a_ktiled = -1;
   return a_ktiled_mode();
+}
+extern "C" int ptk_row_ktiled_reload(void) {
+  g_row_ktiled = -1;
+  return row_ktiled_mode();
 }
 namespace {
 
@@ -376,13 +392,33 @@
     g.rowadd = wt->pos; g.rowadd_period = Nn; g.ld_rowadd = D;
     CK(launch_gemm(g, ACT_NONE, OUT_BF16, 1, st));
   }
+  auto qkv_args = [&](int l) {
+    const ptk_siglip_layer& L = wt->layers[l];
+    GemmArgs g = gemm(w.a, D, L.wqkv, D, w.qkv, 3 * D, M, 3 * D, D, L.wqkv_kt);
+    g.bias = L.bqkv;
+    return g;
+  };
+  auto fc1_args = [&](int l) {
+    const ptk_siglip_layer& L = wt->layers[l];
+    GemmArgs g = gemm(w.a, D, L.w1, D, w.mlp, I, M, I, D, L.w1_kt);
+    g.bias = L.b1;
+    return g;
+  };
+  bool ln1_kt = (row_ktiled_mode() & 4) != 0, ln2_kt = ln1_kt;
+  {
+    const GemmPlanEnv env = gemm_plan_env();
+    for (int l = 0; l < c->layers; ++l) {
+      ln1_kt = ln1_kt && row_ktiled_pair(qkv_args(l), ACT_NONE, 1, false, 0, env, true);
+      ln2_kt = ln2_kt && row_ktiled_pair(fc1_args(l), ACT_GELU_TANH, 1, false, 0, env, true);
+    }
+  }
   for (int l = 0; l < c->layers; ++l) {
     const ptk_siglip_layer& L = wt->layers[l];
     sq.next("siglip.attn");
-    CK(launch_layernorm_bf16(w.h, L.ln1_w, L.ln1_b, w.a, M, D, c->eps, st));
+    CK(launch_layernorm_bf16(w.h, L.ln1_w, L.ln1_b, w.a, M, D, c->eps, st, ln1_kt));
     {
-      GemmArgs g = gemm(w.a, D, L.wqkv, D, w.qkv, 3 * D, M, 3 * D, D, L.wqkv_kt);
-      g.bias = L.bqkv;
+      GemmArgs g = qkv_args(l);
+      g.a_kt = ln1_kt ? A_KT_ROW : 0;
       CK(launch_gemm(g, ACT_NONE, OUT_BF16, 1, st));
     }
     {
@@ -403,10 +439,10 @@
       CK(launch_gemm(g, ACT_NONE, OUT_BF16, 1, st));
     }
     sq.next("siglip.mlp");
-    CK(launch_layernorm_bf16(w.h, L.ln2_w, L.ln2_b, w.a, M, D, c->eps, st));
+    CK(launch_layernorm_bf16(w.h, L.ln2_w, L.ln2_b, w.a, M, D, c->eps, st, ln2_kt));
     {
-      GemmArgs g = gemm(w.a, D, L.w1, D, w.mlp, I, M, I, D, L.w1_kt);
-      g.bias = L.b1;
+      GemmArgs g = fc1_args(l);
+      g.a_kt = ln2_kt ? A_KT_ROW : 0;
       CK(launch_gemm(g, ACT_GELU_TANH, OUT_BF16, 1, st));
     }
     {
@@ -502,6 +538,35 @@
     }
   }
 
+  auto qkv_args = [&](int l) {
+    const ptk_gemma3_layer& L = wt->layers[l];
+    return gemm(train ? w.L[l].xn_in : w.xn, H, L.wqkv, H, w.L[l].qkv, Dqkv, M, Dqkv, H, L.wqkv_kt);
+  };
+  auto do_args = [&](int l) {
+    const ptk_gemma3_layer& L = wt->layers[l];
+    GemmArgs g = gemm(w.dao, H, L.wo_t, H, w.dO, (long)G * D, M, G * D, H, L.wo_t_kt);
+    g.sB0 = (long)G * D * H; g.sC0 = (long)Sp * G * D;
+    g.cmap = RowMap{Sp, 0, (long)Hkv * Sp, 0};
+    return g;
+  };
+  bool ff_kt = false, in_kt = false, do_kt = false, dh_kt = false;
+  if (!train && nl > 1) {
+    const GemmPlanEnv env = gemm_plan_env();
+    ff_kt = (row_ktiled_mode() & 1) != 0;
+    in_kt = (row_ktiled_mode() & 8) != 0;
+    do_kt = dh_kt = (row_ktiled_mode() & 2) != 0 && !fwd_only;
+    dh_kt = dh_kt && !geglu_split();
+    for (int l = 0; l < nl; ++l) {
+      GemmArgs gf, df, gb, db;
+      mlp_fwd(l, gf, df);
+      mlp_bwd(l, gb, db);
+      if (l + 1 < nl) ff_kt = ff_kt && row_ktiled_pair(gf, ACT_GEGLU, 1, false, 0, env, true);
+      if (l > 0) in_kt = in_kt && row_ktiled_pair(qkv_args(l), ACT_NONE, 1, true, w.sk_floats, env, true);
+      do_kt = do_kt && row_ktiled_pair(do_args(l), ACT_NONE, Hkv, false, 0, env, true);
+      if (l + 1 < nl) dh_kt = dh_kt && row_ktiled_pair(gb, ACT_GEGLU_BWD, 1, false, 0, env, true);
+    }
+  }
+
   for (int l = 0; l < nl; ++l) {
     const ptk_gemma3_layer& L = wt->layers[l];
     GemmaLayerSave& sv = w.L[l];
@@ -512,7 +577,11 @@
     bf16_t* xff = train ? sv.xn_ff : w.xn;
     bf16_t* hh = train ? sv.h : w.h;
     sq.next("gemma.fwd.attn");
-    CK(gemm_split(gemm(xin, H, L.wqkv, H, sv.qkv, Dqkv, M, Dqkv, H, L.wqkv_kt), OUT_BF16, w.skpart, w.sk_floats, st));
+    {
+      GemmArgs g = qkv_args(l);
+      g.a_kt = in_kt && l > 0 ? A_KT_ROW : 0;
+      CK(gemm_split(g, OUT_BF16, w.skpart, w.sk_floats, st));
+    }
     CK(launch_qknorm_rope_fwd(sv.qkv, L.q_norm, L.k_norm, cs, sn, ash, eps, sv.Q, sv.K, sv.V, sv.rstd_q, sv.rstd_k,
                               st));
     {
@@ -533,13 +602,14 @@
     }
     CK(gemm_split(gemm(sv.O, Dq, L.wo, Dq, sv.ao, H, M, H, Dq, L.wo_kt), OUT_BF16, w.skpart, w.sk_floats, st));
     CK(launch_residual_norm_fwd(sv.ao, w.x[l], L.ln_post_attn, L.ln_pre_ff, sv.x2, xff, sv.rstd_ao, sv.rstd_pre, M,
-                                H, eps, st));
+                                H, eps, st, ff_kt && l + 1 < nl));
     sq.next("gemma.fwd.mlp");
     if (l + 1 < nl) {
       GemmArgs g, d;
       mlp_fwd(l, g, d);
       g.c_kt = d.a_kt = h_kt;
       g.aux_kt = fac_kt;
+      g.a_kt = ff_kt ? A_KT_ROW : 0;
       CK(launch_gemm(g, ACT_GEGLU, OUT_BF16, 1, st));
       CK(gemm_split(d, OUT_BF16, w.skpart, w.sk_floats, st));
     } else {
@@ -556,7 +626,7 @@
     float* rnext = (l + 1 < nl) ? w.L[l + 1].rstd_in : nullptr;
     bf16_t* xnext = (train && l + 1 < nl) ? w.L[l + 1].xn_in : w.xn;
     CK(launch_residual_norm_fwd(sv.dn, sv.x2, L.ln_post_ff, wnext, w.x[l + 1], xnext, sv.rstd_dn, rnext, M, H, eps,
-                                st));
+                                st, in_kt && l + 1 < nl));
   }
 
   sq.next("gemma.lm_head_ce");
@@ -628,6 +698,7 @@
         mlp_bwd(l, g, d);
         g.c_kt = dgu_kt;
         g.aux_in_kt = fac_kt;
+        g.a_kt = dh_kt ? A_KT_ROW : 0;
         CK(launch_gemm(g, ACT_GEGLU_BWD, OUT_BF16, 1, st));
       }
       if (train) CK(weight_grad(w.dgu, 2 * I, ident, 2 * I, sv.xn_ff, H, ident, H, M, w.TA, w.TB, GL->wgu, w.skpart, w.sk_floats, st));
@@ -651,13 +722,12 @@
     sq.next("gemma.bwd.attn");
     CK(residual_norm_bwd_grads(sv.x2, L.ln_pre_ff, sv.rstd_pre, w.dtmp, dR, sv.ao, L.ln_post_attn, sv.rstd_ao, w.dao,
                                M, H, train ? (bf16_t*)GL->ln_pre_ff : nullptr,
-                               train ? (bf16_t*)GL->ln_post_attn : nullptr, w.wpart, st));
+                               train ? (bf16_t*)GL->ln_post_attn : nullptr, w.wpart, st, do_kt));
     if (train)
       CK(weight_grad(w.dao, H, ident, H, sv.O, Dq, ident, Dq, M, w.TA, w.TB, GL->wo, w.skpart, w.sk_floats, st));
     {
-      GemmArgs g = gemm(w.dao, H, L.wo_t, H, w.dO, (long)G * D, M, G * D, H, L.wo_t_kt);
-      g.sB0 = (long)G * D * H; g.sC0 = (long)Sp * G * D;
-      g.cmap = RowMap{Sp, 0, (long)Hkv * Sp, 0};
+      GemmArgs g = do_args(l);
+      g.a_kt = do_kt ? A_KT_ROW : 0;
       CK(launch_gemm(g, ACT_NONE, OUT_BF16, Hkv, st));
     }
     FlashBwdArgs dkv_plan;
@@ -690,7 +760,7 @@
       const GemmaLayerSave& sp = w.L[l - 1];
       CK(residual_norm_bwd_grads(w.x[l], L.ln_in, sv.rstd_in, w.dtmp, dR, sp.dn, Lp.ln_post_ff, sp.rstd_dn, w.dao,
                                  M, H, train ? (bf16_t*)GL->ln_in : nullptr,
-                                 train ? (bf16_t*)gr->layers[l - 1].ln_post_ff : nullptr, w.wpart, st));
+                                 train ? (bf16_t*)gr->layers[l - 1].ln_post_ff : nullptr, w.wpart, st, dh_kt));
     } else {
       if (train)
         CK(launch_rms_wgrad_bdy(w.x[l], H, ident, sv.rstd_in, w.dtmp, H, M, H, (bf16_t*)GL->ln_in, w.wpart, st));
diff --git a/projectiontrainer_amd/csrc/norm.hip b/projectiontrainer_amd/csrc/norm.hip
--- a/projectiontrainer_amd/csrc/norm.hip
+++ b/projectiontrainer_amd/csrc/norm.hip
@@ -31,10 +31,21 @@
 #define FOR_V for (int v = 0; v < NV; ++v) if (v < NV - 1 || lane * 4 + v * 256 < cols)
 #define COL (lane * 4 + v * 256)
 
+__host__ __device__ inline long row_ktile_offset(long row, int col, int cols) {
+  const long rr = row & 15, chunk = (col >> 3) & 3;
+  const long unit = 4 * rr + (chunk ^ ((rr >> 1) & 2));
+  return ((row >> 4) * (cols >> 5) + (col >> 5)) * 1024 + unit * 16 + (col & 7) * 2;
+}
+template <bool KT>
+PTK_DEV bf16_t* out4(bf16_t* base, long row, int col, int cols) {
+  if constexpr (KT) return reinterpret_cast<bf16_t*>(reinterpret_cast<char*>(base) + row_ktile_offset(row, col, cols));
+  else return base + row * cols + col;
+}
+
 PTK_DEV float4 ldx4(const float* p) { return ld4(p); }
 PTK_DEV float4 ldx4(const bf16_t* p) { return ld4bf(p); }
 
-template <typename T, int NV>
+template <typename T, int NV, bool KT = false>
 PTK_DEV void layernorm_body(const T* __restrict__ x, const float* __restrict__ w, const float* __restrict__ b,
                             bf16_t* __restrict__ y, long rows, int cols, float eps) {
   ROW_SETUP
@@ -52,7 +63,7 @@
   }
   const float rstd = rsqrtf(warp_sum(q) / cols + eps);
 #pragma unroll
-  FOR_V { st4bf(y + row * cols + COL, add4(mul4(scl4(r[v], rstd), ld4(w + COL)), ld4(b + COL))); }
+  FOR_V { st4bf(out4<KT>(y, row, COL, cols), add4(mul4(scl4(r[v], rstd), ld4(w + COL)), ld4(b + COL))); }
 }
 
 template <int NV>
@@ -61,11 +72,11 @@
                                                      int cols, float eps) {
   layernorm_body<float, NV>(x, w, b, y, rows, cols, eps);
 }
-template <int NV>
+template <int NV, bool KT = false>
 __global__ void __launch_bounds__(256) layernorm_b16(const bf16_t* __restrict__ x, const float* __restrict__ w,
                                                      const float* __restrict__ b, bf16_t* __restrict__ y, long rows,
                                                      int cols, float eps) {
-  layernorm_body<bf16_t, NV>(x, w, b, y, rows, cols, eps);
+  layernorm_body<bf16_t, NV, KT>(x, w, b, y, rows, cols, eps);
 }
 
 template <int NV>
@@ -85,7 +96,7 @@
   FOR_V { st4bf(y + row * cols + COL, mul4(scl4(r[v], rs), onep(ld4(w + COL)))); }
 }
 
-template <int NV>
+template <int NV, bool KT = false>
 __global__ void __launch_bounds__(256) residual_norm_fwd_kernel(
     const bf16_t* __restrict__ t, const float* __restrict__ xi, const float* __restrict__ w_post,
     const float* __restrict__ w_next, float* __restrict__ xo, bf16_t* __restrict__ n,
@@ -110,7 +121,7 @@
   const float rs2 = rsqrtf(warp_sum(q2) / cols + eps);
   if (lane == 0) rstd_x[row] = rs2;
 #pragma unroll
-  FOR_V { st4bf(n + row * cols + COL, mul4(scl4(r[v], rs2), onep(ld4(w_next + COL)))); }
+  FOR_V { st4bf(out4<KT>(n, row, COL, cols), mul4(scl4(r[v], rs2), onep(ld4(w_next + COL)))); }
 }
 
 #define RMS_BWD_BODY(XV, DNV, RS, OUTEXPR)                                   \
@@ -175,7 +186,7 @@
   RMS_BWD_BODY(xv, dv, rs, { st4bf(dt + COL, dxv); })
 }
 
-template <typename TD, int NV>
+template <typename TD, int NV, bool KT = false>
 PTK_DEV void residual_norm_bwd_body(
     const float* __restrict__ x2, const float* __restrict__ w_pre, const float* __restrict__ rstd_pre,
     const TD* __restrict__ dn, float* __restrict__ dR, const bf16_t* __restrict__ t,
@@ -200,7 +211,7 @@
     float4 xv[NV], dv[NV];
 #pragma unroll
     FOR_V { xv[v] = ld4bf(t + row * cols + COL); dv[v] = bfr4(nd[v]); }
-    RMS_BWD_BODY(xv, dv, rs, { st4bf(dt + row * cols + COL, dxv); })
+    RMS_BWD_BODY(xv, dv, rs, { st4bf(out4<KT>(dt, row, COL, cols), dxv); })
   }
 }
 template <int NV>
@@ -211,13 +222,13 @@
     int cols) {
   residual_norm_bwd_body<float, NV>(x2, w_pre, rstd_pre, dn, dR, t, w_post, rstd_t, dt, rows, cols);
 }
-template <int NV>
+template <int NV, bool KT = false>
 __global__ void __launch_bounds__(256) residual_norm_bwd_bdn_kernel(
     const float* __restrict__ x2, const float* __restrict__ w_pre, const float* __restrict__ rstd_pre,
     const bf16_t* __restrict__ dn, float* __restrict__ dR, const bf16_t* __restrict__ t,
     const float* __restrict__ w_post, const float* __restrict__ rstd_t, bf16_t* __restrict__ dt, long rows,
     int cols) {
-  residual_norm_bwd_body<bf16_t, NV>(x2, w_pre, rstd_pre, dn, dR, t, w_post, rstd_t, dt, rows, cols);
+  residual_norm_bwd_body<bf16_t, NV, KT>(x2, w_pre, rstd_pre, dn, dR, t, w_post, rstd_t, dt, rows, cols);
 }
 
 #ifndef PTK_NWG_WAVES
@@ -288,28 +299,36 @@
   post_norm_bwd_row<NV>(dR + row * cols, t + row * cols, w, rstd_t[row], dt + row * cols, lane, cols);
 }
 
-#define NORM_DISPATCH(KERNEL, ...)                                                                  \
+#define NORM_DISPATCH_X(KERNEL, SUF, ...)                                                           \
   do {                                                                                              \
     switch ((cols + 255) / 256) {                                                                   \
-      case 1: hipLaunchKernelGGL(KERNEL<1>, NORM_GRID, __VA_ARGS__); break;                         \
-      case 2: hipLaunchKernelGGL(KERNEL<2>, NORM_GRID, __VA_ARGS__); break;                         \
-      case 3: hipLaunchKernelGGL(KERNEL<3>, NORM_GRID, __VA_ARGS__); break;                         \
-      case 4: hipLaunchKernelGGL(KERNEL<4>, NORM_GRID, __VA_ARGS__); break;                         \
-      case 5: hipLaunchKernelGGL(KERNEL<5>, NORM_GRID, __VA_ARGS__); break;                         \
-      case 6: hipLaunchKernelGGL(KERNEL<6>, NORM_GRID, __VA_ARGS__); break;                         \
-      case 7: hipLaunchKernelGGL(KERNEL<7>, NORM_GRID, __VA_ARGS__); break;                         \
-      case 8: hipLaunchKernelGGL(KERNEL<8>, NORM_GRID, __VA_ARGS__); break;                         \
-      case 9: hipLaunchKernelGGL(KERNEL<9>, NORM_GRID, __VA_ARGS__); break;                         \
-      case 10: hipLaunchKernelGGL(KERNEL<10>, NORM_GRID, __VA_ARGS__); break;                       \
-      case 11: hipLaunchKernelGGL(KERNEL<11>, NORM_GRID, __VA_ARGS__); break;                       \
-      default: hipLaunchKernelGGL(KERNEL<MAXV>, NORM_GRID, __VA_ARGS__); break;                     \
+      case 1: hipLaunchKernelGGL((KERNEL<1 SUF>), NORM_GRID, __VA_ARGS__); break;                   \
+      case 2: hipLaunchKernelGGL((KERNEL<2 SUF>), NORM_GRID, __VA_ARGS__); break;                   \
+      case 3: hipLaunchKernelGGL((KERNEL<3 SUF>), NORM_GRID, __VA_ARGS__); break;                   \
+      case 4: hipLaunchKernelGGL((KERNEL<4 SUF>), NORM_GRID, __VA_ARGS__); break;                   \
+      case 5: hipLaunchKernelGGL((KERNEL<5 SUF>), NORM_GRID, __VA_ARGS__); break;                   \
+      case 6: hipLaunchKernelGGL((KERNEL<6 SUF>), NORM_GRID, __VA_ARGS__); break;                   \
+      case 7: hipLaunchKernelGGL((KERNEL<7 SUF>), NORM_GRID, __VA_ARGS__); break;                   \
+      case 8: hipLaunchKernelGGL((KERNEL<8 SUF>), NORM_GRID, __VA_ARGS__); break;                   \
+      case 9: hipLaunchKernelGGL((KERNEL<9 SUF>), NORM_GRID, __VA_ARGS__); break;                   \
+      case 10: hipLaunchKernelGGL((KERNEL<10 SUF>), NORM_GRID, __VA_ARGS__); break;                 \
+      case 11: hipLaunchKernelGGL((KERNEL<11 SUF>), NORM_GRID, __VA_ARGS__); break;                 \
+      default: hipLaunchKernelGGL((KERNEL<MAXV SUF>), NORM_GRID, __VA_ARGS__); break;               \
     }                                                                                               \
   } while (0)
+#define NORM_DISPATCH(KERNEL, ...) NORM_DISPATCH_X(KERNEL, , __VA_ARGS__)
+#define NORM_KT , true
 
 static int check_cols(int cols) {
   if (cols <= 0 || cols % 4 || cols > 256 * MAXV) return set_error("norm: cols=%d unsupported", cols);
   return 0;
 }
+static int check_kt(const void* out, int rows, int cols) {
+  if (!out || rows % 16 || cols % 32 || ((uintptr_t)out & 15))
+    return set_error("norm: a k-step-tiled output needs rows %% 16 == 0, cols %% 32 == 0 and a 16-B aligned buffer "
+                     "(rows=%d, cols=%d)", rows, cols);
+  return 0;
+}
 #define NORM_GRID dim3((unsigned)((rows + 3) / 4)), dim3(256), 0, st
 #define RET_LAUNCH(name) return hipGetLastError() == hipSuccess ? 0 : set_error(name " launch failed")
 
@@ -321,10 +340,11 @@
   RET_LAUNCH("layernorm");
 }
 int launch_layernorm_bf16(const bf16_t* x, const float* w, const float* b, bf16_t* y, int rows, int cols, float eps,
-                          hipStream_t st) {
-  if (check_cols(cols)) return -1;
-  if (rows <= 0) return 0;
-  NORM_DISPATCH(layernorm_b16, x, w, b, y, (long)rows, cols, eps);
+                          hipStream_t st, int kt) {
+  if (check_cols(cols) || (kt && check_kt(y, rows, cols))) return -1;
+  if (rows <= 0) return 0;
+  if (kt) NORM_DISPATCH_X(layernorm_b16, NORM_KT, x, w, b, y, (long)rows, cols, eps);
+  else NORM_DISPATCH(layernorm_b16, x, w, b, y, (long)rows, cols, eps);
   RET_LAUNCH("layernorm_bf16");
 }
 int launch_rmsnorm_fwd(const float* x, long ldx, RowMap xmap, const float* w, bf16_t* y, float* rstd, int rows,
@@ -336,10 +356,14 @@
 }
 int launch_residual_norm_fwd(const bf16_t* t, const float* xi, const float* w_post, const float* w_next, float* xo,
                              bf16_t* n, float* rstd_t, float* rstd_x, int rows, int cols, float eps,
-                             hipStream_t st) {
-  if (check_cols(cols)) return -1;
-  if (rows <= 0) return 0;
-  NORM_DISPATCH(residual_norm_fwd_kernel, t, xi, w_post, w_next, xo, n, rstd_t, rstd_x,
+                             hipStream_t st, int kt) {
+  if (check_cols(cols) || (kt && check_kt(w_next ? n : nullptr, rows, cols))) return -1;
+  if (rows <= 0) return 0;
+  if (kt)
+    NORM_DISPATCH_X(residual_norm_fwd_kernel, NORM_KT, t, xi, w_post, w_next, xo, n, rstd_t, rstd_x, (long)rows, cols,
+                    eps);
+  else
+    NORM_DISPATCH(residual_norm_fwd_kernel, t, xi, w_post, w_next, xo, n, rstd_t, rstd_x,
                      (long)rows, cols, eps);
   RET_LAUNCH("residual_norm_fwd");
 }
@@ -359,10 +383,14 @@
 }
 int launch_residual_norm_bwd_bdn(const float* x2, const float* w_pre, const float* rstd_pre, const bf16_t* dn,
                                  float* dR, const bf16_t* t, const float* w_post, const float* rstd_t, bf16_t* dt,
-                                 int rows, int cols, hipStream_t st) {
-  if (check_cols(cols)) return -1;
-  if (rows <= 0) return 0;
-  NORM_DISPATCH(residual_norm_bwd_bdn_kernel, x2, w_pre, rstd_pre, dn, dR, t, w_post, rstd_t, dt, (long)rows, cols);
+                                 int rows, int cols, hipStream_t st, int kt) {
+  if (check_cols(cols) || (kt && check_kt(dt, rows, cols))) return -1;
+  if (rows <= 0) return 0;
+  if (kt)
+    NORM_DISPATCH_X(residual_norm_bwd_bdn_kernel, NORM_KT, x2, w_pre, rstd_pre, dn, dR, t, w_post, rstd_t, dt,
+                    (long)rows, cols);
+  else
+    NORM_DISPATCH(residual_norm_bwd_bdn_kernel, x2, w_pre, rstd_pre, dn, dR, t, w_post, rstd_t, dt, (long)rows, cols);
   RET_LAUNCH("residual_norm_bwd_bdn");
 }
 int residual_norm_bwd_wg_blocks(int rows) { return (rows + NWG - 1) / NWG; }
@@ -403,4 +431,6 @@
   RET_LAUNCH("post_norm_bwd");
 }
 
-}
+long row_ktile_lane_offset(long row, int lane, int v, int cols) { return row_ktile_offset(row, lane * 4 + v * 256, cols); }
+
+}
diff --git a/projectiontrainer_amd/csrc/ptk_internal.h b/projectiontrainer_amd/csrc/ptk_internal.h
--- a/projectiontrainer_amd/csrc/ptk_internal.h
+++ b/projectiontrainer_amd/csrc/ptk_internal.h
@@ -58,11 +58,13 @@
   const bf16_t* B_kt = nullptr;
   int a_kt = 0, c_kt = 0, aux_kt = 0, aux_in_kt = 0;
 };
+constexpr int A_KT_GEMM = 1, A_KT_ROW = 2;
 
 enum GemmPath { GEMM_PATH_NT = 0, GEMM_PATH_BIG = 1, GEMM_PATH_BIG2 = 2, GEMM_PATH_W4 = 3, GEMM_PATH_NTB = 4,
                 GEMM_PATH_P8SK = 5, GEMM_PATH_P8 = 6, GEMM_PATH_TN = 7, GEMM_NPATH = 9 };
 int path_counts(int64_t* out, int reset);
 int ktiled_counts(int64_t* out2, int reset);
+int64_t row_ktiled_count(int reset);
 int device_cus();
 
 template <class F>
@@ -119,6 +121,9 @@
 bool c_ktiled_ok(const GemmArgs& a, const GemmPlan& plan, int act, int out, int batch, bool lean_epi);
 bool gemm_ktiled_pair(const GemmArgs& prod, int pact, const GemmArgs& cons, long part_floats, const GemmPlanEnv& env,
                       bool enabled, bool factors);
+bool row_ktiled_pair(const GemmArgs& cons, int act, int batch, bool via_split, long part_floats, const GemmPlanEnv& env,
+                     bool enabled);
+int row_ktiled_mode();
 int a_ktiled_mode();
 int launch_gemm(const GemmArgs& a, int act, int out, int batch, hipStream_t st, const GemmPlan* planned = nullptr);
 struct GemmSplitPlan {
@@ -186,12 +191,13 @@
 int launch_layernorm(const float* x, const float* w, const float* b, bf16_t* y, int rows, int cols,
                      float eps, hipStream_t st);
 int launch_layernorm_bf16(const bf16_t* x, const float* w, const float* b, bf16_t* y, int rows, int cols,
-                          float eps, hipStream_t st);
+                          float eps, hipStream_t st, int kt = 0);
+long row_ktile_lane_offset(long row, int lane, int v, int cols);
 int launch_rmsnorm_fwd(const float* x, long ldx, RowMap xmap, const float* w, bf16_t* y, float* rstd,
                        int rows, int cols, float eps, hipStream_t st);
 int launch_residual_norm_fwd(const bf16_t* t, const float* xi, const float* w_post, const float* w_next,
                              float* xo, bf16_t* n, float* rstd_t, float* rstd_x, int rows, int cols,
-                             float eps, hipStream_t st);
+                             float eps, hipStream_t st, int kt = 0);
 int launch_rmsnorm_bwd_f32(const float* x, const float* w, const float* rstd, const float* dn,
                            const float* dacc, float* dx, int rows, int cols, hipStream_t st);
 int launch_residual_norm_bwd(const float* x2, const float* w_pre, const float* rstd_pre, const float* dn,
@@ -203,7 +209,7 @@
                            float* dx, int rows, int cols, hipStream_t st);
 int launch_residual_norm_bwd_bdn(const float* x2, const float* w_pre, const float* rstd_pre, const bf16_t* dn,
                                  float* dR, const bf16_t* t, const float* w_post, const float* rstd_t, bf16_t* dt,
-                                 int rows, int cols, hipStream_t st);
+                                 int rows, int cols, hipStream_t st, int kt = 0);
 int residual_norm_bwd_wg_blocks(int rows);
 int launch_residual_norm_bwd_wg(const float* x2, const float* w_pre, const float* rstd_pre, const bf16_t* dn,
                                 float* dR, const bf16_t* t, const float* w_post, const float* rstd_t, bf16_t* dt,
diff --git a/projectiontrainer_amd/kernels.py b/projectiontrainer_amd/kernels.py
--- a/projectiontrainer_amd/kernels.py
+++ b/projectiontrainer_amd/kernels.py
@@ -59,7 +59,7 @@
     d.bf16_linear = int(bool(bf16_linear))
     d.tail_ws = ptr(tail_ws)
     d.B_kt = ptr(B_kt)
-    d.A_kt, d.C_kt, d.aux_kt, d.aux_in_kt = int(bool(A_kt)), int(bool(C_kt)), int(bool(aux_kt)), int(bool(aux_in_kt))
+    d.A_kt, d.C_kt, d.aux_kt, d.aux_in_kt = int(A_kt), int(bool(C_kt)), int(bool(aux_kt)), int(bool(aux_in_kt))
     check(L.lib().ptk_gemm(d, L.stream_ptr(A.device)), "ptk_gemm")
     return C
 
@@ -70,6 +70,37 @@
     rows, cols = x.numel() // x.shape[-1], x.shape[-1]
     check(L.lib().ptk_layernorm(ptr(x), ptr(w), ptr(b), ptr(y), rows, cols, eps, L.stream_ptr(x.device)), "layernorm")
     return y
+
+
+def layernorm_bf16(x, w, b, eps, *, y=None, kt=False):
+    _require_cuda(x)
+    rows, cols = x.shape
+    y = torch.empty_like(x) if y is None else y
+    check(L.lib().ptk_layernorm_bf16(ptr(x), ptr(w), ptr(b), ptr(y), rows, cols, eps, int(kt), L.stream_ptr(x.device)),
+          "layernorm_bf16")
+    return y
+
+
+def residual_norm_fwd(t, xi, w_post, w_next, eps, *, n=None, kt=False):
+    _require_cuda(t, xi)
+    rows, cols = t.shape
+    xo = torch.empty_like(xi)
+    if n is None and w_next is not None:
+        n = torch.empty_like(t)
+    rt, rx = (torch.empty(rows, dtype=torch.float32, device=t.device) for _ in range(2))
+    check(L.lib().ptk_residual_norm_fwd(ptr(t), ptr(xi), ptr(w_post), ptr(w_next), ptr(xo), ptr(n), ptr(rt), ptr(rx),
+                                        rows, cols, eps, int(kt), L.stream_ptr(t.device)), "residual_norm_fwd")
+    return xo, n, rt, rx
+
+
+def residual_norm_bwd_bdn_(x2, w_pre, rstd_pre, dn, dR, t, w_post, rstd_t, *, dt=None, kt=False):
+    _require_cuda(x2, dR)
+    rows, cols = x2.shape
+    dt = torch.empty_like(t) if dt is None else dt
+    check(L.lib().ptk_residual_norm_bwd_bdn(ptr(x2), ptr(w_pre), ptr(rstd_pre), ptr(dn), ptr(dR), ptr(t), ptr(w_post),
+                                            ptr(rstd_t), ptr(dt), rows, cols, int(kt), L.stream_ptr(x2.device)),
+          "residual_norm_bwd_bdn")
+    return dt
 
 
 def rmsnorm(x, w, eps):
```
